# kolinko/effort

Hardware: AMD Instinct MI355X
Metric: effective GB/s + tokens/s vs effort %, Mistral-7B FFN 4096x11008 fp16 (higher is better)
Workload: dtype f16

## Files before the change

effort_amd/_lib.py:

```python
from __future__ import annotations

import ctypes as C
import os
import subprocess

_HERE = os.path.dirname(os.path.abspath(__file__))
LAB_LIB_PATH = os.path.join(_HERE, "libeffort_hip_lab.so")
LIB_PATH = (LAB_LIB_PATH if os.environ.get("EFFORT_HIP_LIB") == "lab" else os.environ.get("EFFORT_HIP_LIB")) or os.path.join(_HERE, "libeffort_hip.so")

ERRORS = {
    -1: "EFFORT_ERR_ARG", -2: "EFFORT_ERR_SHAPE", -3: "EFFORT_ERR_EFFORT", -4: "EFFORT_ERR_HIP",
    -5: "EFFORT_ERR_KIND", -6: "EFFORT_ERR_CONVERT", -7: "EFFORT_ERR_BLAS", -8: "EFFORT_ERR_COMM",
}


class EffortError(RuntimeError):
    def __init__(self, code: int, where: str, detail: str = ""):
        self.code = code
        super().__init__(f"{where}: {ERRORS.get(code, code)} {detail}".strip())


def build(verbose: bool = False) -> str:
    cmd = ["make", "-C", os.path.join(_HERE, "csrc"), "-j8", "all"]
    res = subprocess.run(cmd, capture_output=not verbose, text=True)
    if res.returncode != 0:
        raise RuntimeError("building libeffort_hip.so failed:\n" + (res.stdout or "") + (res.stderr or ""))
    return LIB_PATH


_P = C.c_void_p
_SIGS = {
    "effort_create": (_P, [C.c_int, _P]),
    "effort_destroy": (None, [_P]),
    "effort_set_stream": (C.c_int, [_P, _P]),
    "effort_sync": (C.c_int, [_P]),
    "effort_set_overlap": (C.c_int, [_P, C.c_int]),
    "effort_set_row_reuse": (C.c_int, [_P, C.c_int]),
    "effort_join": (C.c_int, [_P]),
    "effort_last_error": (C.c_char_p, [_P]),
    "effort_version": (C.c_char_p, []),
    "effort_weights_fp16": (_P, [_P, _P, _P, _P, C.c_int, C.c_int, C.c_int, C.c_int]),
    "effort_weights_fp16_pitched": (_P, [_P, _P, C.c_int, _P, _P, C.c_int, C.c_int, C.c_int, C.c_int]),
    "effort_aligned_row_pitch": (C.c_int, [C.c_int]),
    "effort_weights_q4": (_P, [_P, _P, _P, _P, _P, C.c_int64, C.c_int, C.c_int, C.c_int]),
    "effort_weights_free": (None, [_P]),
    "effort_weights_refresh": (C.c_int, [_P]),
    "effort_weights_align_rows": (C.c_int, [_P]),
    "effort_weights_row_pitch": (C.c_int, [_P]),
    "effort_weights_get_bound": (C.c_int, [_P, C.POINTER(C.c_float)]),
    "effort_weights_set_bound": (C.c_int, [_P, C.POINTER(C.c_float)]),
    "effort_weights_column_shard": (_P, [_P, C.c_int, C.c_int]),
    "effort_comm_unique_id": (C.c_int, [_P]),
    "effort_comm_create": (C.c_int, [_P, C.c_int, C.c_int, _P]),
    "effort_comm_destroy": (C.c_int, [_P]),
    "effort_comm_rank": (C.c_int, [_P]),
    "effort_comm_world": (C.c_int, [_P]),
    "effort_allgather_outputs": (C.c_int, [_P, _P, _P, C.c_int]),
    "effort_bucketmul": (C.c_int, [_P, _P, _P, _P, _P, C.c_double]),
    "effort_bucketmul_q4": (C.c_int, [_P, _P, _P, _P, _P, C.c_double]),
    "effort_bucketmul_group": (C.c_int, [_P, C.c_int, _P, _P, _P, _P, _P]),
    "effort_bucketmul_q4_group": (C.c_int, [_P, C.c_int, _P, _P, _P, _P, _P]),
    "effort_bucketmul_group_fused": (C.c_int, [_P, C.c_int, _P, _P, _P, _P, _P, _P, _P, _P]),
    "effort_bucketmul_q4_group_fused": (C.c_int, [_P, C.c_int, _P, _P, _P, _P, _P, _P, _P, _P]),
    "effort_group_dispatch_count": (C.c_int, [_P, C.c_int, C.POINTER(C.c_uint32)]),
    "effort_group_cutoff": (C.c_int, [_P, C.c_int, C.POINTER(C.c_float)]),
    "effort_debug_occupancy": (C.c_int, [_P, C.c_int, C.c_int, C.c_int, C.c_int]),
    "effort_set_persistent": (C.c_int, [_P, C.c_int]),
    "effort_debug_hook_lane": (C.c_int, [_P, C.c_int]),
    "effort_add_rmsnorm_mul": (C.c_int, [_P, _P, _P, _P, _P, C.c_int]),
    "effort_rope_kv": (C.c_int, [_P, _P, _P, _P, _P, _P, _P, _P, C.c_int, C.c_int, C.c_int, C.c_int, C.c_float]),
    "effort_attention": (C.c_int, [_P, _P, _P, _P, _P, _P, C.c_int, C.c_int, C.c_int]),
    "effort_rope_attention": (C.c_int, [_P, _P, _P, _P, _P, _P, _P, _P, C.c_int, C.c_int, C.c_int, C.c_int, C.c_float]),
    "effort_silu_mul": (C.c_int, [_P, _P, _P, _P, C.c_int]),
    "effort_fetch_row": (C.c_int, [_P, _P, _P, _P, C.c_int]),
    "effort_argmax": (C.c_int, [_P, _P, C.c_int, _P, _P, _P, C.c_int]),
    "effort_decode_status": (C.c_int, [_P, C.POINTER(C.c_int)]),
    "effort_sample": (C.c_int, [_P, _P, C.c_int, _P, _P, _P, _P, C.c_int, _P, _P]),
    "effort_topk": (C.c_int, [_P, _P, C.c_int, C.c_int, _P, _P]),
    "effort_sample_bits": (C.c_uint32, [C.c_uint32, C.c_uint32, C.c_uint32, C.c_uint32]),
    "effort_convert_status": (C.c_int, [_P, C.POINTER(C.c_int)]),
    "effort_q4_outlier_count": (C.c_int64, [C.c_int, C.c_int, C.c_double]),
    "effort_convert_q4": (C.c_int, [_P, _P, C.c_int, C.c_int, C.c_double, _P, _P, _P, _P]),
    "effort_top2_softmax": (C.c_int, [_P, _P, C.c_int, _P, _P]),
    "effort_mix2": (C.c_int, [_P, _P, _P, _P, _P, C.c_int]),
    "effort_moe_route": (C.c_int, [_P, _P, _P, _P, C.c_int, C.c_int, _P, _P, _P]),
    "effort_mix2_add": (C.c_int, [_P, _P, _P, _P, _P, C.c_int]),
    "effort_dense_gemv": (C.c_int, [_P, _P, _P, _P, C.c_int, C.c_int]),
    "effort_dense_gemv_expert": (C.c_int, [_P, _P, _P, _P, _P, C.c_int, C.c_int, C.c_int]),
    "effort_dense_gemm_rows": (C.c_int, [_P, _P, _P, _P, C.c_int, C.c_int, C.c_int]),
    "effort_dense_gemm_rows_routed": (C.c_int, [_P, _P, C.c_int, _P, _P, C.c_int, _P, C.c_int, C.c_int, C.c_int]),
    "effort_weights_bucket_dense_ok": (C.c_int, [_P, C.POINTER(C.c_int)]),
    "effort_bucket_gemm_rows": (C.c_int, [_P, _P, C.c_int, _P, _P, C.c_int]),
    "effort_bucket_gemm_rows_routed": (C.c_int, [_P, _P, _P, _P, C.c_int, _P, C.c_int]),
    "effort_moe_route_rows": (C.c_int, [_P, _P, _P, _P, C.c_int, C.c_int, _P, _P, _P, C.c_int]),
    "effort_mix2_add_rows": (C.c_int, [_P, _P, _P, _P, C.c_int, C.c_int]),
    "effort_fetch_rows": (C.c_int, [_P, _P, _P, _P, C.c_int, C.c_int]),
    "effort_add_rmsnorm_mul_rows": (C.c_int, [_P, _P, _P, _P, _P, C.c_int, C.c_int]),
    "effort_rope_kv_rows": (C.c_int, [_P, _P, _P, _P, _P, _P, _P, C.c_int, C.c_int, C.c_int, C.c_int, C.c_int, C.c_int, C.c_float]),
    "effort_attention_rows": (C.c_int, [_P, _P, _P, _P, C.c_int, C.c_int, _P, C.c_int, C.c_int, C.c_int]),
    "effort_attention_block": (C.c_int, [_P, _P, _P, _P, C.c_int, C.c_int, _P, C.c_int, C.c_int, C.c_int]),
    "effort_set_dense_backend": (C.c_int, [_P, C.c_int]),
    "effort_last_dispatch_count": (C.c_int, [_P, C.POINTER(C.c_uint32)]),
    "effort_last_cutoff": (C.c_int, [_P, C.POINTER(C.c_float)]),
    "effort_calc_dispatch": (C.c_int, [_P, _P, _P, _P, C.c_double, _P, _P]),
    "effort_convert_fp16": (C.c_int, [_P, _P, C.c_int, C.c_int, _P, _P, _P]),
    "effort_convert_fp16_pitched": (C.c_int, [_P, _P, C.c_int, C.c_int, _P, C.c_int, _P, _P]),
    "effort_cosine": (C.c_int, [_P, _P, _P, C.c_int, C.POINTER(C.c_float)]),
    "effort_set_split_cutoff": (C.c_int, [_P, C.c_int]),
    "effort_set_tuning": (C.c_int, [_P, C.c_int, C.c_int, C.c_int]),
    "effort_is_lab_build": (C.c_int, []),
    "effort_enable_kernel_timing": (C.c_int, [_P, C.c_int]),
    "effort_debug_stamps": (C.c_int, [_P, C.POINTER(C.c_ulonglong)]),
    "effort_debug_slice_counts": (C.c_int, [_P, C.c_int, C.POINTER(C.c_uint32), C.c_int]),
    "effort_debug_plan": (C.c_int, [C.c_int, C.c_int, C.c_int, C.c_int, _P, _P, _P, _P, _P, _P, C.c_int, C.c_int, C.c_int, C.c_int, _P, _P, _P, _P, _P, _P, _P, _P, _P]),
    "effort_debug_check_bundle": (C.c_int, [C.c_int, C.c_int, C.c_int, C.c_int, C.c_int, C.c_int]),
    "effort_debug_variants": (C.c_int, [C.c_int, _P, C.c_int]),
    "effort_debug_last_variant": (C.c_int, [_P, C.c_int, _P]),
    "effort_debug_lanes": (C.c_int, [C.c_int, C.c_int, _P, C.c_int64, _P]),
    "effort_debug_trace": (C.c_int, [_P, C.POINTER(C.c_ulonglong), C.c_int]),
    "effort_kernel_clock": (C.c_int, [_P, C.POINTER(C.c_double), C.POINTER(C.c_int)]),
    "effort_kernel_timing": (C.c_int, [_P, C.POINTER(C.c_double), C.POINTER(C.c_double), C.POINTER(C.c_double), C.POINTER(C.c_int)]),
}

_lib = None


def lib() -> C.CDLL:
    global _lib
    if _lib is None:
        if not os.path.exists(LIB_PATH):
            raise RuntimeError(
                f"{LIB_PATH} is missing: the HIP extension has not been built "
                "(run `python -c 'import __graft_entry__ as g; g.build()'` or `make -C effort_amd/csrc`). "
                "effort_amd has no CPU fallback.")
        import torch
        l = C.CDLL(LIB_PATH)
        for name, (res, args) in _SIGS.items():
            if (name.startswith("effort_debug_") or name == "effort_is_lab_build") and os.environ.get("EFFORT_HIP_LIB") and not hasattr(l, name):
                continue
            fn = getattr(l, name)
            fn.restype = res
            fn.argtypes = args
        _lib = l
    return _lib


def exported_symbols() -> list[str]:
    return sorted(_SIGS)
```

effort_amd/csrc/bucket_mul.hip:

```cpp
#include <cstring>
#include <type_traits>

#include "cutoff_device.h"

namespace effort {

constexpr int kBatch = 16;
template <int E> __host__ __device__ constexpr int batch_rows() { return E >= 4 ? 8 : kBatch; }
constexpr int kRounds = 16;

#ifndef EFFORT_ABLATE_NOSCATTER
#define EFFORT_ABLATE_NOSCATTER 0
#endif
#ifndef EFFORT_ABLATE_NOLOAD
#define EFFORT_ABLATE_NOLOAD 0
#endif

constexpr int kMinWavesPerEU = 4;

#ifndef EFFORT_ROW_AUX
#define EFFORT_ROW_AUX 2
#endif
constexpr int kRowAux = EFFORT_ROW_AUX;
#define GA_PERSISTENT(ga) (PERSIST ? (ga).persistent : 0u)
#define GA_CUTJOBS(ga) (PERSIST ? (ga).cutJobs : 0u)
#ifndef EFFORT_LAB
#define EFFORT_PRODUCT_ONLY 1
#if defined(EFFORT_CUT_FINE) || defined(EFFORT_LEAN_STAMPS) || EFFORT_ABLATE_NOSCATTER || EFFORT_ABLATE_NOLOAD
#error "lab switches need -DEFFORT_LAB (they belong in libeffort_hip_lab.so / build/variants, never in the shipped library)"
#endif
#endif
#ifdef EFFORT_PRODUCT_ONLY
constexpr bool kProductOnly = true;
#else
constexpr bool kProductOnly = false;
#endif
#ifdef EFFORT_PRODUCT_ONLY
#define GA_TSTAMP(ga) ((unsigned long long*)nullptr)
#define GA_ABLATE(ga) 0u
#define GA_TRACE(ga) 0u
#elif defined(EFFORT_LEAN_STAMPS)
#define GA_TSTAMP(ga) ((ga).tstamp)
#define GA_ABLATE(ga) (PERSIST ? (ga).ablate : 0u)
#define GA_TRACE(ga) 0u
#else
#define GA_TSTAMP(ga) (PERSIST ? (ga).tstamp : nullptr)
#define GA_ABLATE(ga) (PERSIST ? (ga).ablate : 0u)
#define GA_TRACE(ga) (PERSIST ? (ga).trace : 0u)
#endif
#ifdef EFFORT_LEAN_STAMPS
constexpr bool kLeanStamps = true;
#else
constexpr bool kLeanStamps = false;
#endif
constexpr uint32_t kMaxLdsBytes = 160u * 1024u - 1024u;
constexpr int kSc1 = 16;

template <int FMT> struct Fmt;
template <> struct Fmt<kFp16> { static constexpr int kAcc = 16, kSlots = 16; };
template <> struct Fmt<kQ4> { static constexpr int kAcc = 32, kSlots = 64; };

template <int FMT> struct MeanT;
template <> struct MeanT<kFp16> { typedef uint16_t type; };
template <> struct MeanT<kQ4> { typedef float type; };

template <int E> struct Piece;
template <> struct Piece<1> {
    uint32_t w;
    template <int AUX> __device__ __forceinline__ void load(__amdgpu_buffer_rsrc_t r, uint32_t voff, uint32_t soff) { w = __builtin_amdgcn_raw_buffer_load_b16(r, voff, soff, AUX); }
    __device__ __forceinline__ uint32_t word(int) const { return w & 0xFFFFu; }
    __device__ __forceinline__ uint32_t dword(int) const { return w; }
};
template <> struct Piece<2> {
    uint32_t w;
    template <int AUX> __device__ __forceinline__ void load(__amdgpu_buffer_rsrc_t r, uint32_t voff, uint32_t soff) { w = __builtin_amdgcn_raw_buffer_load_b32(r, voff, soff, AUX); }
    __device__ __forceinline__ uint32_t word(int j) const { return (w >> (16 * j)) & 0xFFFFu; }
    __device__ __forceinline__ uint32_t dword(int) const { return w; }
};
template <> struct Piece<4> {
    uint32_t w[2];
    template <int AUX> __device__ __forceinline__ void load(__amdgpu_buffer_rsrc_t r, uint32_t voff, uint32_t soff) {
        auto t = __builtin_amdgcn_raw_buffer_load_b64(r, voff, soff, AUX); w[0] = t[0]; w[1] = t[1];
    }
    __device__ __forceinline__ uint32_t word(int j) const { return (w[j >> 1] >> (16 * (j & 1))) & 0xFFFFu; }
    __device__ __forceinline__ uint32_t dword(int j) const { return w[j >> 1]; }
};
__host__ __device__ inline uint32_t align_up(uint32_t x, uint32_t a) { return (x + a - 1) / a * a; }

constexpr int kOlBatch = 16;
constexpr uint32_t kOlLdsFloats = 16384;
template <int E> __host__ __device__ inline uint32_t ol_outputs_per_item(const MulGeom& g) { return align_up((32u * E * 64u + g.slices - 1u) / g.slices, 64u); }
constexpr uint32_t kOlEarlyFloats = 4096;
constexpr int kOlMerged = 8;
constexpr uint32_t kOlSumFloats = 1024;
template <int E> __host__ __device__ inline uint32_t ol_scratch_bytes(const MulGeom& g) {
    const uint32_t per = ol_outputs_per_item<E>(g);
    return (per > kOlSumFloats ? per : kOlSumFloats) * 4u + (g.inDim <= kOlLdsFloats ? g.inDim * 4u : 0u);
}

template <int FMT, int E, int W>
__host__ __device__ inline LdsPlan plan_lds(const MulGeom* geoms, int nGeoms, bool merge) {
    uint32_t slots = 0, vrows = 0, ol = 0, vEarly = 0;
    for (int i = 0; i < nGeoms; i++) {
        const MulGeom& g = geoms[i];
        if (!g.slices) continue;
        slots = slots > g.slots ? slots : g.slots;
        const uint32_t vr = align_up(g.sliceRows, 64);
        vrows = vrows > vr ? vrows : vr;
        if (FMT != kFp16) {
            const uint32_t x = ol_scratch_bytes<E>(g); ol = ol > x ? ol : x;
            if (merge && W == 8 && g.inDim <= kOlEarlyFloats) vEarly = vEarly > g.inDim * 4u ? vEarly : g.inDim * 4u;
        }
    }
    LdsPlan p;
    uint32_t o = 0;
    p.offM = o; o += align_up(slots, 64) * 4;
    p.offV[0] = o; o += vrows * 4;
    p.offV[1] = FMT == kFp16 ? o : p.offV[0];
    if (FMT == kFp16) o += vrows * 4;
    if (FMT != kFp16 && o < ol) o = align_up(ol, 16);
    p.offA = o; o += (uint32_t)Fmt<FMT>::kSlots * E * 64 * 4;
    p.offL = o; o += align_up(slots * 2, 16);
    const uint32_t tbl = cutoff_table_bytes(64 * W);
    if (o < p.offA + tbl) o = p.offA + tbl;
    p.offC = o; o += 2048;
    p.offO = vEarly ? o : 0u; o += vEarly;
    static_assert(kCutoffLdsBytes <= 1280, "the cutoff scratch must end below the flags of the misc region");
    p.total = o;
    return p;
}
struct ItemRef { uint32_t ci, t, s; };

__device__ __forceinline__ bool locate_item(const GroupKArgs& ga, const uint32_t item, ItemRef& r) {
    uint32_t ci = 0;
    for (uint32_t i = 0; i + 1 < ga.count; i++) if ((item >> 3) >= (uint32_t)ga.wgEnd8[i]) ci = i + 1;
    ci = __builtin_amdgcn_readfirstlane(ci);
    const MulGeom& g = ga.geom[ga.call[ci].geom];
    const uint32_t b = item - (ci ? (uint32_t)ga.wgEnd8[ci - 1] * 8u : 0u), xcd = b & 7u, k = b >> 3;
    r.ci = ci;
    if ((g.slices & 7u) == 0u) {
        r.s = (k / g.tiles) * 8u + ((xcd + ci) & 7u); r.t = k % g.tiles;
        return true;
    }
    const uint32_t per = (uint32_t)ga.wgEnd8[ci] - (ci ? (uint32_t)ga.wgEnd8[ci - 1] : 0u);
    const uint32_t idx = ((xcd + ci) & 7u) * per + k;
    r.s = idx / g.tiles; r.t = idx - r.s * g.tiles;
    return r.s < g.slices;
}

typedef uint32_t u32x4 __attribute__((ext_vector_type(4)));
__device__ __forceinline__ void lds_dma_dword(const u32x4 rsrc, const uint32_t voff, const uint32_t ldsAddr) {
    uint32_t keep;
    asm volatile("s_mov_b32 %0, m0\n\ts_mov_b32 m0, %2\n\ts_nop 0\n\tbuffer_load_dword %1, %3, 0 offen lds\n\ts_mov_b32 m0, %0"
                 : "=&s"(keep) : "v"(voff), "s"(ldsAddr), "s"(rsrc) : "memory");
}
__device__ __forceinline__ u32x4 make_rsrc(const void* base, uint32_t bytes) {
    const uint64_t p = (uint64_t)(size_t)base;
    u32x4 r;
    r[0] = __builtin_amdgcn_readfirstlane((uint32_t)p); r[1] = __builtin_amdgcn_readfirstlane((uint32_t)(p >> 32) & 0xFFFFu);
    r[2] = __builtin_amdgcn_readfirstlane(bytes); r[3] = 0x00020000u;
    return r;
}

template <int FMT, int W, bool COMPACT>
__device__ __forceinline__ void stage_issue(const GroupKArgs& ga, const ItemRef& r, const int tid, char* smem, const LdsPlan& lp, const uint32_t par) {
    constexpr int NT = 64 * W;
    using lds_v = __attribute__((address_space(3))) void;
    const CallDesc& a = ga.call[__builtin_amdgcn_readfirstlane(r.ci)];
    const MulGeom& g = ga.geom[a.geom];
    const uint32_t wave = __builtin_amdgcn_readfirstlane(tid >> 6);
    const uint32_t B = g.sliceRows, j0 = __builtin_amdgcn_readfirstlane(r.s) * B, nb = min(B, g.inDim - j0), lg = g.sliceLog2;
    const uint32_t e = a.expNo ? a.expNo[0] : 0u;
    const uint32_t rowBase = e * g.expertRows;
    const uint32_t rowsPerIn = g.rowsPerIn, inDim = g.inDim, mask = (1u << lg) - 1u;
    const uint32_t nSlots = FMT == kFp16 ? (rowsPerIn << lg) : (nb << 3);
    constexpr bool compact = COMPACT && FMT == kFp16;
    const u32x4 rs = make_rsrc(a.stats, (uint32_t)((size_t)g.numExperts * g.expertRows * (compact ? 2u : 8u)));
    const u32x4 rv = make_rsrc(a.v, inDim * 4u);
    const uint32_t ldsM = __builtin_amdgcn_readfirstlane((uint32_t)(size_t)(lds_v*)(smem + lp.offM));
    const uint32_t ldsV = __builtin_amdgcn_readfirstlane((uint32_t)(size_t)(lds_v*)(smem + ((par & 1u) ? lp.offV[1] : lp.offV[0])));
    if constexpr (compact) {
#pragma unroll
        for (int rr = 0; rr < kRounds / 2; rr++) {
            if (((uint32_t)(rr * NT) + wave * 64u) * 2u >= nSlots) continue;
            const uint32_t c = ((uint32_t)(rr * NT) + (uint32_t)tid) * 2u, rank = c >> lg, jl = c & mask;
            const bool ok = rank < rowsPerIn && jl < nb;
            lds_dma_dword(rs, (rowBase + (ok ? rank * inDim + j0 + jl : j0)) * 2u, ldsM + ((uint32_t)(rr * NT) + wave * 64u) * 4u);
        }
    } else
#pragma unroll
    for (int rr = 0; rr < kRounds; rr++) {
        if ((uint32_t)(rr * NT) + wave * 64u >= nSlots) continue;
        const uint32_t c = rr * NT + tid;
        uint32_t voff;
        if (FMT == kFp16) {
            const uint32_t rank = c >> lg, jl = c & mask;
            const bool ok = rank < rowsPerIn && jl < nb;
            voff = (rowBase + (ok ? rank * inDim + j0 + jl : j0)) * 8u + 4u;
        } else {
            voff = ((rowBase + j0 * 8u + (c < nSlots ? c : 0u)) * 2u + 1u) * 4u;
        }
        lds_dma_dword(rs, voff, ldsM + ((uint32_t)(rr * NT) + wave * 64u) * 4u);
    }
#pragma unroll
    for (int u = 0; u < (FMT == kFp16 ? 1 : 2); u++) {
        if ((uint32_t)(u * NT) + wave * 64u >= nb) continue;
        lds_dma_dword(rv, (j0 + (uint32_t)(u * NT + tid)) * 4u, ldsV + ((uint32_t)(u * NT) + wave * 64u) * 4u);
    }
}

template <int FMT, int E, int W, bool FUSED, bool COMPACT, bool PERSIST, typename Prefetch>
__device__ __forceinline__ void mul_item(const GroupKArgs& ga, const uint32_t item, const ItemRef& ref, char* smem, const LdsPlan& lp, uint32_t& cachedCall,
                                         float& cachedCutoff, const uint32_t par, const bool staged, const bool firstItem, Prefetch prefetch) {
    constexpr int NACC = Fmt<FMT>::kAcc;
    constexpr int TILE_F = NACC * E * 64;
    constexpr int TILE_L = Fmt<FMT>::kSlots * E * 64;
    constexpr int NT = 64 * W;
    constexpr int VPT = 4096 / NT;
    constexpr int KB = batch_rows<E>();

    const uint32_t ci = __builtin_amdgcn_readfirstlane(ref.ci), s = __builtin_amdgcn_readfirstlane(ref.s), t = __builtin_amdgcn_readfirstlane(ref.t);
    const CallDesc& a = ga.call[ci];
    const MulGeom& g = ga.geom[a.geom];
    float* const a_slabs = ga.slabs + (size_t)a.slabOff * 64u;
    uint32_t* const a_counters = ga.counters + a.tileOff;
    uint32_t* const a_sliceCounts = ga.sliceCounts + a.sliceOff;
    float* const a_cutoff = ga.cutoff + ci;
    (void)item;

    int tid0 = threadIdx.x;
    asm volatile("" : "+v"(tid0));
    const int tid = tid0, lane = tid & 63;
#ifdef EFFORT_CUT_FINE
    const bool wstamp = false;
#else
    const bool wstamp = GA_TSTAMP(ga) && tid == 0;
#endif
    unsigned long long ph[6] = {0, 0, 0, 0, 0, 0};
    if (wstamp) ph[0] = wall_clock64();
#ifdef EFFORT_CUT_FINE
    const bool stampCut = GA_TSTAMP(ga) && item == 0 && tid == 0, stamp = false;
#define EFFORT_PSTAMP(i) if (stampCut) GA_TSTAMP(ga)[26 + (i)] = clock64();
#else
#define EFFORT_PSTAMP(i)
    const bool stamp = GA_TSTAMP(ga) && item == 0 && tid == 0;
    const bool stampCut = stamp;
#endif
    if (stamp) GA_TSTAMP(ga)[16] = wall_clock64();
    const int wave = __builtin_amdgcn_readfirstlane(tid >> 6);
    const uint32_t B = g.sliceRows;
    const uint32_t offC = __builtin_amdgcn_readfirstlane(lp.offC), offL = __builtin_amdgcn_readfirstlane(lp.offL), offM = __builtin_amdgcn_readfirstlane(lp.offM);
    const uint32_t offA = __builtin_amdgcn_readfirstlane(lp.offA);
    int* acc = reinterpret_cast<int*>(smem + offA);
    float* vblk = reinterpret_cast<float*>(smem + __builtin_amdgcn_readfirstlane((par & 1u) ? lp.offV[1] : lp.offV[0]));
    uint32_t* flags = reinterpret_cast<uint32_t*>(smem + offC + 1280);
    float* wbound = reinterpret_cast<float*>(smem + offC + 1344);
    uint16_t* list = reinterpret_cast<uint16_t*>(smem + offL);
    const uint32_t* m32 = reinterpret_cast<const uint32_t*>(smem + offM);
    const float* means = reinterpret_cast<const float*>(smem + offM);

    const uint32_t j0 = s * B;
    uint32_t vSlabOff = (s * g.tiles + t) * (uint32_t)(TILE_F * 4), vSlabBytes = (uint32_t)min((size_t)0xFFFFFFFFu, (size_t)g.slices * g.tiles * TILE_F * 4);
    uint32_t vSlices = g.slices, vSliceStride = g.tiles * (uint32_t)(TILE_F * 4);
    if constexpr (!PERSIST) asm volatile("" : "+v"(vSlabOff), "+v"(vSlabBytes), "+v"(vSlices), "+v"(vSliceStride));
    const uint32_t nb = min(B, g.inDim - j0);
    const uint32_t e = a.expNo ? a.expNo[0] : 0u;

    EFFORT_PSTAMP(1)
    if (!staged) stage_issue<FMT, W, COMPACT>(ga, ref, tid, smem, lp, par);
    EFFORT_PSTAMP(2)
    constexpr bool kPreZero = !PERSIST;
    if constexpr (kPreZero) cutoff_table_zero<NT>(reinterpret_cast<uint32_t*>(smem + offA), tid);
    constexpr bool kOlMerge = FMT != kFp16 && W == 8 && (!PERSIST || kProductOnly);
    const uint32_t olPer = ol_outputs_per_item<E>(g);
    bool olAny = false, olEarly = false;
    uint32_t olParts = 1u, olStride = 0u;
    uint32_t olBFirst = 0u, olNB = 0u;
    float olVx[kOlMerge ? 8 : 1]; uint32_t olMeta0 = 0u, olBeg0 = 0u, olEnd0 = 0u;
    auto ol_share = [&]() {
        const uint32_t oBeg = min(t * (uint32_t)TILE_F + s * olPer, g.outDim);
        const uint32_t oEnd = max(oBeg, min(min(t * (uint32_t)TILE_F + (s + 1u) * olPer, (t + 1u) * (uint32_t)TILE_F), g.outDim));
        olBFirst = oBeg >> 6; olNB = ((oEnd + 63u) >> 6) - olBFirst;
        olParts = (olNB && olNB < (uint32_t)W) ? (uint32_t)W / olNB : 1u;
        olStride = olNB * 64u;
    };
    if constexpr (FMT != kFp16) {
        olAny = a.ol.blockPtr != nullptr;
        if (olAny) {
            if constexpr (kOlMerge) {
                ol_share();
                olEarly = g.inDim <= kOlEarlyFloats && lp.offO != 0u;
                if (olEarly) {
                    if constexpr (FUSED) {
                        if (a.pre == (uint16_t)kPreNone) {
#pragma unroll
                            for (int u = 0; u < 8; u++) olVx[u] = a.v[min((uint32_t)(u * NT + tid), g.inDim - 1u)];
                        }
                    } else {
#pragma unroll
                    for (int u = 0; u < 8; u++) olVx[u] = a.v[min((uint32_t)(u * NT + tid), g.inDim - 1u)];
                    }
                    if ((uint32_t)wave < olNB * olParts) {
                        const uint32_t bq = (uint32_t)wave / olParts;
                        olMeta0 = a.ol.meta[(size_t)(olBFirst + bq) * 64u + (uint32_t)lane];
                        olBeg0 = a.ol.blockPtr[olBFirst + bq]; olEnd0 = a.ol.blockPtr[olBFirst + bq + 1u];
                    }
                }
            }
        }
    }
    const float rankBound = a.rankBound[e];
    float vj[VPT]; uint16_t prj[VPT];
    const uint16_t* pr = a.probes + (size_t)e * kProbes;
    const bool fused = (ga.split & 1u) == 0u;
#pragma unroll
    for (int i = 0; i < VPT; i++) { vj[i] = 0.0f; prj[i] = 0; }
    const bool needCut = fused && cachedCall != ci;
    const bool viaJob = needCut && GA_CUTJOBS(ga) != 0u && !firstItem;
    const uint32_t pre = FUSED ? (uint32_t)a.pre : (uint32_t)kPreNone;
    float rawn[VPT]; uint32_t auxc[VPT]; uint32_t auxS = 0u;
    uint32_t auxS1 = 0u;
    const bool preAny = FUSED && pre != (uint32_t)kPreNone;
#pragma unroll
    for (int i = 0; i < VPT; i++) { rawn[i] = 0.0f; auxc[i] = 0u; }
    if (preAny) {
        const bool gate = pre == (uint32_t)kPreSiluGate;
        if (needCut || !gate) {
#pragma unroll
            for (int i = 0; i < VPT; i++) rawn[i] = *(a.v + tid + NT * i);
        }
        if (needCut) {
#pragma unroll
            for (int i = 0; i < VPT; i++) {
                auxc[i] = gate ? __float_as_uint(*(reinterpret_cast<const float*>(a.vAux) + tid + NT * i)) : (uint32_t)reinterpret_cast<const uint16_t*>(a.vAux)[tid + NT * i];
                prj[i] = pr[tid + NT * i];
            }
        }
        const uint32_t js = j0 + min((uint32_t)tid, nb - 1u);
        auxS = gate ? __float_as_uint(*(reinterpret_cast<const float*>(a.vAux) + js)) : (uint32_t)reinterpret_cast<const uint16_t*>(a.vAux)[js];
        if constexpr (FUSED && FMT != kFp16) {
            const uint32_t js1 = j0 + min((uint32_t)(tid + NT), nb - 1u);
            auxS1 = gate ? __float_as_uint(*(reinterpret_cast<const float*>(a.vAux) + js1)) : (uint32_t)reinterpret_cast<const uint16_t*>(a.vAux)[js1];
            if (olEarly && !needCut) {
                if (gate) {
#pragma unroll
                    for (int i = 0; i < VPT; i++) rawn[i] = *(a.v + tid + NT * i);
                }
#pragma unroll
                for (int i = 0; i < VPT; i++)
                    auxc[i] = gate ? __float_as_uint(*(reinterpret_cast<const float*>(a.vAux) + tid + NT * i)) : (uint32_t)reinterpret_cast<const uint16_t*>(a.vAux)[tid + NT * i];
            }
        }
    }
    const uint32_t lg = g.sliceLog2;
    const uint32_t nSlots = FMT == kFp16 ? (g.rowsPerIn << lg) : (nb << 3);
    float normInv = 1.0f;
    if (FUSED && pre == kPreRmsNorm) {
        constexpr int R = 1024 / NT;
        static_assert(R >= 1 && R * NT == 1024 && R * W == 16, "fused rmsNorm: the workgroup must divide add_rmsnorm_mul_kernel's 1024 threads");
        float part[R];
#pragma unroll
        for (int r = 0; r < R; r++) part[r] = 0.0f;
#pragma unroll
        for (int i = 0; i < VPT; i++) part[i % R] += rawn[i] * rawn[i];
        for (uint32_t base = 4096u + (uint32_t)tid; base < g.inDim; base += 1024u) {
#pragma unroll
            for (int r = 0; r < R; r++) {
                const uint32_t j = base + (uint32_t)(r * NT);
                if (j < g.inDim) { const float x = *(a.v + j); part[r] += x * x; }
            }
        }
#pragma unroll
        for (int r = 0; r < R; r++) {
            part[r] = wave_sum_f32(part[r]);
            if (lane == 0) wbound[r * W + wave] = part[r];
        }
        __syncthreads();
        float tot = 0.0f;
#pragma unroll
        for (int w2 = 0; w2 < 16; w2++) tot += wbound[w2];
        normInv = 1.0f / sqrtf(tot / (float)g.inDim + 1e-5f);
        __syncthreads();
    }
    auto xform = [&](float x, uint32_t aux) -> float {
        if (!FUSED) return x;
        if (pre == kPreSiluGate) return __uint_as_float(aux) * x / (1.0f + expf(-x));
        if (pre == kPreRmsNorm) return (x * normInv) * half_bits_to_float((uint16_t)aux);
        return x;
    };
    auto load_cut_inputs = [&]() {
        if (preAny) {
#pragma unroll
            for (int i = 0; i < VPT; i++) vj[i] = xform(rawn[i], auxc[i]);
        } else {
#pragma unroll
            for (int i = 0; i < VPT; i++) { vj[i] = *(a.v + tid + NT * i); prj[i] = pr[tid + NT * i]; }
        }
    };
    if constexpr (kPreZero) {
        asm volatile("s_waitcnt lgkmcnt(0)" ::: "memory");
        __builtin_amdgcn_s_barrier();
    }
    if (needCut && !viaJob) load_cut_inputs();
    EFFORT_PSTAMP(3)
    uint32_t* const cutWords = ga.queue + 9 * 16;
    uint32_t cutWord = 0;
    if (viaJob && tid == 0 && !(GA_ABLATE(ga) & 32u)) cutWord = __hip_atomic_load(&cutWords[ci], __ATOMIC_RELAXED, __HIP_MEMORY_SCOPE_AGENT);
    asm volatile("s_waitcnt vmcnt(0)" ::: "memory");
    EFFORT_PSTAMP(4)
    uint32_t vColOK = 0, voff = 0, vRecords = 0, vBuckLo = 0, vBuckHi = 0, vRowPitch = 0, vInDim = 0, vRow0 = 0;
    auto stream_geom = [&]() {
        const uint32_t col = t * (64u * E) + (uint32_t)lane * E;
        vColOK = col < g.cols ? 1u : 0u;
        voff = (vColOK ? col : (g.cols - 1u) / (uint32_t)E * (uint32_t)E) * 2u;
        vRecords = (uint32_t)min((size_t)0xFFFFFFFFu, (size_t)g.numExperts * g.expertRows * g.rowPitch - (size_t)a.bucketsTrim);
        vBuckLo = (uint32_t)(size_t)a.buckets; vBuckHi = (uint32_t)((size_t)a.buckets >> 32);
        vRowPitch = g.rowPitch; vInDim = g.inDim; vRow0 = e * g.expertRows + (FMT == kFp16 ? j0 : j0 * 8u);
    };
    if constexpr (!PERSIST) {
        stream_geom();
        asm volatile("" : "+v"(vColOK), "+v"(voff), "+v"(vRecords), "+v"(vBuckLo), "+v"(vBuckHi), "+v"(vRowPitch), "+v"(vInDim), "+v"(vRow0));
    }
    if constexpr (kOlMerge) {
        if (olEarly) {
            float* const vf = reinterpret_cast<float*>(smem + __builtin_amdgcn_readfirstlane(lp.offO));
#pragma unroll
            for (int u = 0; u < 8; u++) {
                if constexpr (FUSED) { if ((uint32_t)(u * NT + tid) < g.inDim) vf[u * NT + tid] = preAny ? xform(rawn[u % VPT], auxc[u % VPT]) : olVx[u]; }
                else if ((uint32_t)(u * NT + tid) < g.inDim) vf[u * NT + tid] = olVx[u];
            }
        }
    }
    float bound = 0.0f;
#pragma unroll
    for (int u = 0; u < (FMT == kFp16 ? 1 : 2); u++) {
        const uint32_t jl = tid + u * NT;
        if (jl < nb) {
            float x = vblk[jl];
            if constexpr (FUSED && FMT != kFp16) { if (preAny) { x = xform(x, u ? auxS1 : auxS); vblk[jl] = x; } }
            else
            if (preAny) { x = xform(x, auxS); vblk[jl] = x; }
            bound += fabsf(x);
        }
    }
    bound = wave_sum_f32(bound);
    if (lane == 0) wbound[wave] = bound;
    if (tid == 0) { flags[4] = 0u; flags[5] = (uint32_t)(W * KB); }
    if (stamp) GA_TSTAMP(ga)[17] = wall_clock64();
    if (wstamp) ph[1] = wall_clock64();

    uint32_t* tbl = reinterpret_cast<uint32_t*>(smem + offA);
    float cutoff;
    bool fromJob = false;
    if (viaJob) {
        if (tid == 0) {
            for (int spin = 0; spin < ((GA_ABLATE(ga) & 32u) ? 0 : 20000) && !(cutWord >> 31); spin++) {
                __builtin_amdgcn_s_sleep(8);
                cutWord = __hip_atomic_load(&cutWords[ci], __ATOMIC_RELAXED, __HIP_MEMORY_SCOPE_AGENT);
            }
            flags[2] = cutWord >> 31;
            flags[3] = cutWord & 0x7FFFFFFFu;
        }
        __syncthreads();
        fromJob = flags[2] != 0u;
        if (fromJob) { cutoff = __uint_as_float(flags[3]); cachedCall = ci; cachedCutoff = cutoff; }
        else load_cut_inputs();
    }
    if (fromJob) {
    } else if (needCut) {
        cutoff = block_find_cutoff<NT, kPreZero>(vj, prj, a.q, smem + offC, tbl, []() {}, stampCut ? GA_TSTAMP(ga) + 8 : nullptr);
        cachedCall = ci; cachedCutoff = cutoff;
    } else if (fused) {
        cutoff = cachedCutoff;
        __syncthreads();
    } else {
        cutoff = a_cutoff[0];
        __syncthreads();
    }
    const uint32_t slotCap = __builtin_amdgcn_readfirstlane((lp.offV[0] - lp.offM) / 4u) - 1u;
    const uint16_t* m16 = reinterpret_cast<const uint16_t*>(m32);
    auto load_block = [&](int blk, uint32_t (&mraw)[4], float (&vq)[4]) {
#pragma unroll
        for (int u = 0; u < 4; u++) {
            const uint32_t c = min((uint32_t)((blk * 4 + u) * NT + tid), slotCap);
            if constexpr (COMPACT && FMT == kFp16) { mraw[u] = (uint32_t)m16[c] << 16; vq[u] = 0.0f; }
            else { mraw[u] = m32[c]; vq[u] = FMT != kFp16 ? vblk[min(c >> 3, nb - 1u)] : 0.0f; }
        }
    };
    uint32_t mraw0[4]; float vq0[4];
    load_block(0, mraw0, vq0);
    const uint32_t jlSel = (uint32_t)tid & ((1u << lg) - 1u);
    float axRaw = 0.0f;
    if (FMT == kFp16) axRaw = vblk[min(jlSel, nb - 1u)];
    float wb[W];
#pragma unroll
    for (int w2 = 0; w2 < W; w2++) wb[w2] = wbound[w2];
    __builtin_amdgcn_sched_barrier(0);
    for (int i = tid; i < TILE_L; i += NT) acc[i] = 0;
    float L = 0.0f;
#pragma unroll
    for (int w2 = 0; w2 < W; w2++) L += wb[w2];
    L *= rankBound;
    int kexp = 30 - (int)((__float_as_uint(L) >> 23) & 0xFFu) + 126;
    kexp = L > 0.0f ? max(-100, min(100, kexp)) : 0;
    const float scale = __uint_as_float((uint32_t)(127 + kexp) << 23), unscale = __uint_as_float((uint32_t)(127 - kexp) << 23);
    if (stamp) GA_TSTAMP(ga)[18] = wall_clock64();
    if (wstamp) ph[2] = wall_clock64();

    const float ax = (FMT == kFp16 && jlSel < nb) ? fabsf(axRaw) : 0.0f;
    const bool sel = !(GA_ABLATE(ga) & 8u);
    uint32_t keepMask = 0;
    uint32_t before[kRounds];
    uint32_t wtot = 0;
#pragma unroll
    for (int blk = 0; blk < kRounds / 4; blk++) {
        if (blk > 0 && (uint32_t)(blk * 4 * NT) >= nSlots) {
#pragma unroll
            for (int u = 0; u < 4; u++) before[blk * 4 + u] = wtot;
            continue;
        }
        uint32_t mraw[4]; float vq[4];
        if (blk == 0) {
#pragma unroll
            for (int u = 0; u < 4; u++) { mraw[u] = mraw0[u]; vq[u] = vq0[u]; }
        } else {
            load_block(blk, mraw, vq);
        }
#pragma unroll
        for (int u = 0; u < 4; u++) {
            const int rr = blk * 4 + u;
            before[rr] = wtot;
            const uint32_t c = rr * NT + tid;
            bool k;
            if (FMT == kFp16) k = (cutoff < (kCutoffScale * half_bits_to_float((uint16_t)(mraw[u] >> 16))) * ax) & ((c >> lg) < g.rowsPerIn) & sel;
            else k = (cutoff < (kCutoffScale * __uint_as_float(mraw[u])) * fabsf(vq[u])) & (c < nSlots) & sel;
            keepMask |= k ? (1u << rr) : 0u;
            wtot += (uint32_t)__popcll(__ballot(k));
        }
    }
    uint32_t wbase = 0;
    if (lane == 0) wbase = atomicAdd(&flags[4], wtot);
    wbase = __builtin_amdgcn_readfirstlane(wbase);
#pragma unroll
    for (int rr = 0; rr < kRounds; rr++) {
        if ((uint32_t)(rr * NT) >= nSlots) break;
        const uint32_t c = rr * NT + tid;
        const bool k = (keepMask >> rr) & 1u;
        const unsigned long long m = __ballot(k);
        const uint32_t pos = wbase + before[rr] + __builtin_amdgcn_mbcnt_hi((uint32_t)(m >> 32), __builtin_amdgcn_mbcnt_lo((uint32_t)m, 0u));
        if (k) list[pos] = (uint16_t)(FMT == kFp16 ? (((c >> lg) << 12) | (c & ((1u << lg) - 1u))) : c);
    }
    __syncthreads();
    const uint32_t n = flags[4];
    const uint32_t code0 = list[(uint32_t)(wave * KB) + ((uint32_t)lane & (uint32_t)(KB - 1))];
    if (t == 0 && tid == 0) a_sliceCounts[s] = n;
    if (stamp) GA_TSTAMP(ga)[19] = wall_clock64();
    if (wstamp) ph[3] = wall_clock64();

    if constexpr (PERSIST) stream_geom();
    const bool colOK = vColOK != 0u;
    const __amdgpu_buffer_rsrc_t rsrc = __builtin_amdgcn_make_buffer_rsrc(
        reinterpret_cast<uint16_t*>((size_t)(uint32_t)__builtin_amdgcn_readfirstlane(vBuckLo) | ((size_t)(uint32_t)__builtin_amdgcn_readfirstlane(vBuckHi) << 32)), 0,
        (int)__builtin_amdgcn_readfirstlane(vRecords), 0x00020000);
    const uint32_t nU = (GA_ABLATE(ga) & 4u) ? 0u : __builtin_amdgcn_readfirstlane(n);
    uint32_t* const cursor = flags + 5;
    auto grab = [&]() -> uint32_t {
        uint32_t bq = 0;
        if (lane == 0) bq = atomicAdd(cursor, (uint32_t)KB);
        return __builtin_amdgcn_readfirstlane(bq);
    };

    auto decode_code = [&](uint32_t code, uint32_t& boff, float& dv) {
        {
            uint32_t rowIdx;
            if (FMT == kFp16) { const uint32_t rank = code >> 12, jl = code & 4095u; rowIdx = rank * vInDim + jl; dv = vblk[jl] * scale; }
            else {
                rowIdx = code;
                dv = __int_as_float(__float2int_rn((vblk[code >> 3] * means[code]) * scale));
            }
            boff = (vRow0 + rowIdx) * vRowPitch;
        }
    };
    auto decode = [&](uint32_t i0, uint32_t& boff, float& dv) {
        boff = 0; dv = 0.0f;
        if (lane < KB && nU) decode_code(list[min(i0 + (uint32_t)lane, nU - 1u)], boff, dv);
    };
    auto decode_first = [&](uint32_t i0, uint32_t& boff, float& dv) {
        boff = 0; dv = 0.0f;
        if (lane < KB && nU) decode_code(i0 + (uint32_t)lane < nU ? code0 : (uint32_t)__builtin_amdgcn_readfirstlane((int)code0), boff, dv);
    };
    auto issue = [&](auto aux, Piece<E> (&piece)[KB], uint32_t boff) {
#pragma unroll
        for (int u = 0; u < KB; u++) piece[u].template load<decltype(aux)::value>(rsrc, voff, EFFORT_ABLATE_NOLOAD ? 0u : __builtin_amdgcn_readlane(boff, u));
    };
    using lds_i = __attribute__((address_space(3))) int;
    const uint32_t accB = (uint32_t)(size_t)(lds_i*)(acc + lane);
    constexpr int kShift = (E == 1 ? 8 : E == 2 ? 9 : 10);
    auto row = [&](const Piece<E>& pc, float dd) {
        if (FMT == kFp16) {
#pragma unroll
            for (int j = 0; j < E; j++) {
                const uint32_t dw = pc.dword(j);
                uint32_t a2; int qv;
                asm("v_bfe_u32 %0, %1, %2, 4\n\tv_lshl_add_u32 %0, %0, %3, %4" : "=&v"(a2) : "v"(dw), "n"(16 * (j & 1)), "n"(kShift), "v"(accB));
                if (j & 1) asm("v_fma_mix_f32 %0, %1, %2, 0 op_sel:[0,1,0] op_sel_hi:[0,1,0]\n\tv_cvt_rpi_i32_f32 %0, %0" : "=v"(qv) : "v"(dd), "v"(dw));
                else asm("v_fma_mix_f32 %0, %1, %2, 0 op_sel_hi:[0,1,0]\n\tv_cvt_rpi_i32_f32 %0, %0" : "=v"(qv) : "v"(dd), "v"(dw));
                __hip_atomic_fetch_add((lds_i*)(size_t)a2 + j * 64, qv, __ATOMIC_RELAXED, __HIP_MEMORY_SCOPE_WORKGROUP);
            }
        } else {
            const int di = __float_as_int(dd);
#pragma unroll
            for (int j = 0; j < E; j++) {
                const uint32_t x = pc.word(j);
#pragma unroll
                for (int q = 0; q < 4; q++) {
                    uint32_t a2;
                    asm("v_bfe_u32 %0, %1, %2, 4\n\tv_lshl_add_u32 %0, %0, %3, %4" : "=&v"(a2) : "v"(x), "n"(4 * q), "n"(kShift), "v"(accB));
                    __hip_atomic_fetch_add((lds_i*)(size_t)a2 + ((3 - q) * 16 * E + j) * 64, di, __ATOMIC_RELAXED, __HIP_MEMORY_SCOPE_WORKGROUP);
                }
            }
        }
    };
    auto accumulate = [&](const Piece<E> (&piece)[KB], float dv, uint32_t nv) {
        if (EFFORT_ABLATE_NOSCATTER) {
#pragma unroll
            for (int u = 0; u < KB; u++) asm volatile("" ::"v"(piece[u].word(E - 1)), "v"(dv));
            return;
        }
        if (!colOK) return;
        if (nv == (uint32_t)KB) {
#pragma unroll
            for (int u = 0; u < KB; u++) row(piece[u], __uint_as_float(__builtin_amdgcn_readlane(__float_as_uint(dv), u)));
        } else {
#pragma unroll
            for (int u = 0; u < KB; u++)
                if ((uint32_t)u < nv) row(piece[u], __uint_as_float(__builtin_amdgcn_readlane(__float_as_uint(dv), u)));
        }
    };

    bool asked = false;
    using lds_f = __attribute__((address_space(3))) float;
    uint32_t olLen = 0u, olOut = 0u, olKa = 0u, olKf = 0u, olK1 = 0u, olCur = 0u, olSlot = 0xFFFFFFFFu;
    float olAcc = 0.0f;
    const lds_f* olV = nullptr;
    if constexpr (kOlMerge) {
        if (olEarly) {
            olV = (const lds_f*)(size_t)(uint32_t)(size_t)(__attribute__((address_space(3))) void*)(smem + __builtin_amdgcn_readfirstlane(lp.offO));
            if ((uint32_t)wave < olNB * olParts) {
                const uint32_t bq = (uint32_t)wave / olParts, part = (uint32_t)wave % olParts;
                olLen = olMeta0 >> 8; olOut = olMeta0 & 63u;
                const uint32_t olLenAll = olLen;
                const uint32_t maxLen = (uint32_t)__builtin_amdgcn_readfirstlane((int)olLen);
                const uint32_t chunk = (maxLen + olParts - 1u) / olParts, k0 = min(maxLen, part * chunk);
                const uint32_t bBeg = __builtin_amdgcn_readfirstlane(olBeg0), bEnd = __builtin_amdgcn_readfirstlane(olEnd0);
                olK1 = bEnd > bBeg ? min(maxLen, k0 + chunk) : k0;
                olKa = olKf = k0;
                olCur = bBeg + wave_sum_u32(min(olLenAll, k0));
                olLen = min(olLenAll, olK1);
                olSlot = part * olStride + bq * 64u + olOut;
            }
        }
    }
    auto ol_fma = [](float x, uint32_t ent, float acc) -> float {
        float r;
        asm("v_fma_mix_f32 %0, %1, %2, %3 op_sel:[0,1,0] op_sel_hi:[0,1,0]" : "=v"(r) : "v"(x), "v"(ent), "v"(acc));
        return r;
    };
    auto ol_fetch = [&](uint32_t (&ent)[kOlMerged]) {
#pragma unroll
        for (int u = 0; u < kOlMerged; u++) {
            ent[u] = *((a.ol.entry + olCur) + lane);
            olCur += (uint32_t)__popcll(__ballot(olLen > olKf + (uint32_t)u));
        }
        olKf += (uint32_t)kOlMerged;
    };
    auto ol_add = [&](const uint32_t (&ent)[kOlMerged]) {
        float x[kOlMerged];
#pragma unroll
        for (int u = 0; u < kOlMerged; u++) x[u] = olV[ent[u] & 0xFFFFu];
#pragma unroll
        for (int u = 0; u < kOlMerged; u++)
            { const float r = ol_fma(x[u], ent[u], olAcc); olAcc = olLen > olKa + (uint32_t)u ? r : olAcc; }
        olKa += (uint32_t)kOlMerged;
    };
    auto stream_rows = [&](auto withOl, auto aux) {
        constexpr bool OL = decltype(withOl)::value;
        Piece<E> pa[KB], pb[KB];
        uint32_t entA[OL ? kOlMerged : 1], entB[OL ? kOlMerged : 1];
        uint32_t boffA, boffB; float dvA, dvB;
        uint32_t baseA = (uint32_t)(wave * KB), baseB;
        if (baseA < nU) { decode_first(baseA, boffA, dvA); issue(aux, pa, boffA); }
        if constexpr (OL) ol_fetch(entA);
        while (baseA < nU) {
            if (!asked && nU - baseA <= 4u * KB * W) asked = prefetch();
            if (wstamp && GA_TRACE(ga) && item + GA_CUTJOBS(ga) < (uint32_t)kTraceItems) {
                const uint32_t q0 = (4u * baseA) / nU, q1 = min(4u, (4u * (baseA + 2u * KB * W)) / nU);
                for (uint32_t q = q0 + 1u; q <= q1 && q < 4u; q++) GA_TSTAMP(ga)[kTraceOff + (size_t)kTraceItems * 8u + (size_t)(item + GA_CUTJOBS(ga)) * 4u + q - 1u] = wall_clock64();
            }
            baseB = grab();
            decode(baseB, boffB, dvB);
            issue(aux, pb, boffB);
            if constexpr (OL) ol_fetch(entB);
            accumulate(pa, dvA, __builtin_amdgcn_readfirstlane(min((uint32_t)KB, nU - baseA)));
            if constexpr (OL) ol_add(entA);
            baseA = grab();
            decode(baseA, boffA, dvA);
            issue(aux, pa, boffA);
            if constexpr (OL) ol_fetch(entA);
            accumulate(pb, dvB, __builtin_amdgcn_readfirstlane(baseB < nU ? min((uint32_t)KB, nU - baseB) : 0u));
            if constexpr (OL) ol_add(entB);
        }
        if constexpr (OL) {
            while (olKa < olK1) {
                ol_fetch(entB); ol_add(entA);
                if (olKa >= olK1) break;
                ol_fetch(entA); ol_add(entB);
            }
        }
    };
    constexpr bool kRowSwitch = kRowAux != 0 && (PERSIST || E == 4);
    const bool rowsReused = kRowSwitch && (ga.split & 8u) != 0u;
    auto stream = [&](auto withOl) {
        if constexpr (kRowSwitch) { if (rowsReused) { stream_rows(withOl, std::integral_constant<int, 0>{}); return; } }
        stream_rows(withOl, std::integral_constant<int, kRowAux>{});
    };
    if constexpr (kOlMerge) { if (olEarly) stream(std::true_type{}); else stream(std::false_type{}); }
    else stream(std::false_type{});
    if (!asked) asked = prefetch();
    __syncthreads();
    if (stamp) GA_TSTAMP(ga)[20] = wall_clock64();
    if (wstamp) ph[4] = wall_clock64();

    float* const olsum = reinterpret_cast<float*>(smem + offM);
    if constexpr (FMT != kFp16) {
        if (olAny) {
            const OutlierIndex& ol = a.ol;
            float* const vfull = olEarly ? reinterpret_cast<float*>(smem + __builtin_amdgcn_readfirstlane(lp.offO)) : olsum + (olPer > kOlSumFloats ? olPer : kOlSumFloats);
            const bool vLds = g.inDim <= kOlLdsFloats;
            if constexpr (!kOlMerge) ol_share();
            const uint32_t bFirst = olBFirst, nB = olNB, parts = olParts;
            if (vLds && !olEarly) {
                for (uint32_t i0 = 0; i0 < g.inDim; i0 += NT * 8u) {
                    float x[8];
#pragma unroll
                    for (int u = 0; u < 8; u++) x[u] = a.v[min(i0 + u * NT + tid, g.inDim - 1u)];
                    if constexpr (FUSED) {
                        uint32_t xa[8];
#pragma unroll
                        for (int u = 0; u < 8; u++) xa[u] = 0u;
                        if (preAny) {
#pragma unroll
                            for (int u = 0; u < 8; u++) {
                                const uint32_t i = min(i0 + u * NT + tid, g.inDim - 1u);
                                xa[u] = pre == (uint32_t)kPreSiluGate ? __float_as_uint(*(reinterpret_cast<const float*>(a.vAux) + i)) : (uint32_t)reinterpret_cast<const uint16_t*>(a.vAux)[i];
                            }
                        }
#pragma unroll
                        for (int u = 0; u < 8; u++) {
                            const uint32_t i = i0 + u * NT + tid;
                            if (i < g.inDim) vfull[i] = preAny ? xform(x[u], xa[u]) : x[u];
                        }
                    } else
#pragma unroll
                    for (int u = 0; u < 8; u++) {
                        const uint32_t i = i0 + u * NT + tid;
                        if (i < g.inDim) vfull[i] = x[u];
                    }
                }
                __syncthreads();
            }
            if (olSlot != 0xFFFFFFFFu) olsum[olSlot] = olAcc;
            const lds_f* const vfullL = (const lds_f*)(size_t)(uint32_t)(size_t)(__attribute__((address_space(3))) void*)vfull;
            auto run_blocks = [&](auto fromLds) {
                for (uint32_t q = (uint32_t)wave + (olEarly ? (uint32_t)W : 0u); q < nB * parts; q += (uint32_t)W) {
                    const uint32_t bq = q / parts, part = q % parts;
                    const uint32_t meta = ol.meta[(size_t)(bFirst + bq) * 64u + (uint32_t)lane];
                    const uint32_t lenAll = meta >> 8, myOut = meta & 63u;
                    const uint32_t maxLen = (uint32_t)__builtin_amdgcn_readfirstlane((int)lenAll);
                    const uint32_t chunk = (maxLen + parts - 1u) / parts, k0 = min(maxLen, part * chunk), k1 = min(maxLen, k0 + chunk);
                    const uint32_t myLen = min(lenAll, k1);
                    const uint32_t bBeg = __builtin_amdgcn_readfirstlane(ol.blockPtr[bFirst + bq]), bEnd = __builtin_amdgcn_readfirstlane(ol.blockPtr[bFirst + bq + 1u]);
                    uint32_t cur = bBeg + wave_sum_u32(min(lenAll, k0));
                    float acc = 0.0f;
                    auto fetch = [&](uint32_t (&ent)[kOlBatch], uint32_t kk) {
#pragma unroll
                        for (int u = 0; u < kOlBatch; u++) {
                            ent[u] = *((ol.entry + cur) + lane);
                            cur += (uint32_t)__popcll(__ballot(myLen > kk + (uint32_t)u));
                        }
                    };
                    auto add = [&](const uint32_t (&ent)[kOlBatch], uint32_t kk) {
                        float x[kOlBatch];
#pragma unroll
                        for (int u = 0; u < kOlBatch; u++) {
                            const uint32_t in = ent[u] & 0xFFFFu;
                            if constexpr (decltype(fromLds)::value) x[u] = vfullL[in]; else x[u] = a.v[in];
                        }
#pragma unroll
                        for (int u = 0; u < kOlBatch; u++)
                            { const float r = ol_fma(x[u], ent[u], acc); acc = myLen > kk + (uint32_t)u ? r : acc; }
                    };
                    if (k0 < k1 && bEnd > bBeg) {
                        uint32_t entA[kOlBatch], entB[kOlBatch];
                        uint32_t kk = k0;
                        fetch(entA, kk);
                        for (;;) {
                            const bool more = kk + (uint32_t)kOlBatch < k1;
                            if (more) fetch(entB, kk + (uint32_t)kOlBatch);
                            add(entA, kk);
                            if (!more) break;
                            kk += (uint32_t)kOlBatch;
                            const bool more2 = kk + (uint32_t)kOlBatch < k1;
                            if (more2) fetch(entA, kk + (uint32_t)kOlBatch);
                            add(entB, kk);
                            if (!more2) break;
                            kk += (uint32_t)kOlBatch;
                        }
                    }
                    olsum[part * olStride + bq * 64u + myOut] = acc;
                }
            };
            if (vLds) run_blocks(std::true_type{}); else run_blocks(std::false_type{});
            __syncthreads();
        }
    }

    const __amdgpu_buffer_rsrc_t srs = __builtin_amdgcn_make_buffer_rsrc(a_slabs, 0, (int)__builtin_amdgcn_readfirstlane(vSlabBytes), 0x00020000);
    const uint32_t slabOff = __builtin_amdgcn_readfirstlane(vSlabOff);
    const uint32_t nSlices = __builtin_amdgcn_readfirstlane(vSlices);
    auto tile_out = [&](int o) -> float {
        if (FMT == kFp16) return (float)acc[o] * unscale;
        const int slot = o / (E * 64), rem = o % (E * 64);
        const int p = (((slot >> 3) * 16 + (slot & 7)) * E * 64) + rem;
        float r = (float)(acc[p] - acc[p + 8 * E * 64]) * unscale;
        if (olAny) {
            const uint32_t ol_o = (uint32_t)((rem & 63) * E + (rem >> 6)) * 32u + (uint32_t)slot - s * olPer;
            if (ol_o < olPer && (uint32_t)(t * TILE_F) + s * olPer + ol_o < g.outDim) {
                float so = olsum[ol_o];
                for (uint32_t pp = 1; pp < olParts; pp++) so += olsum[pp * olStride + ol_o];
                r += so;
            }
        }
        return r;
    };
    if (fused && t == 0 && s == 0 && tid == 0 && !GA_CUTJOBS(ga)) a_cutoff[0] = cutoff;
    {
        constexpr int kIt = (TILE_F + NT * 2 - 1) / (NT * 2);
        float s0[kIt], s1[kIt];
#pragma unroll
        for (int it = 0; it < kIt; it++) {
            const int o = min(tid * 2 + it * NT * 2, TILE_F - 2);
            s0[it] = tile_out(o); s1[it] = tile_out(o + 1);
        }
#pragma unroll
        for (int it = 0; it < kIt; it++) {
            const int o = tid * 2 + it * NT * 2;
            if (TILE_F % (NT * 2) != 0 && o >= TILE_F) continue;
            typedef uint32_t u2 __attribute__((ext_vector_type(2)));
            u2 pk; pk[0] = __float_as_uint(s0[it]); pk[1] = __float_as_uint(s1[it]);
            __builtin_amdgcn_raw_buffer_store_b64(pk, srs, (uint32_t)o * 4u, slabOff, kSc1);
        }
    }
    asm volatile("s_waitcnt vmcnt(0)" ::: "memory");
    if (stamp) { GA_TSTAMP(ga)[21] = wall_clock64(); GA_TSTAMP(ga)[22] = n; }
    if (wstamp) ph[5] = wall_clock64();
    auto flush_stamps = [&]() {
#ifndef EFFORT_PRODUCT_ONLY
        if (!wstamp) return;
        if (GA_TRACE(ga) && item + GA_CUTJOBS(ga) < (uint32_t)kTraceItems) {
            unsigned long long* rec = GA_TSTAMP(ga) + kTraceOff + (size_t)(item + GA_CUTJOBS(ga)) * 8u;
            rec[0] = (unsigned long long)(item + GA_CUTJOBS(ga)) | ((unsigned long long)blockIdx.x << 32);
            rec[1] = (unsigned long long)(__builtin_amdgcn_s_getreg((31 << 11) | 20) & 0xFu) | ((unsigned long long)(ci & 0xFu) << 4) | ((unsigned long long)(n & 0xFFFFu) << 8) | ((unsigned long long)(t & 0xFFu) << 24) |
                     ((unsigned long long)__builtin_amdgcn_s_getreg((31 << 11) | 4) << 32);
#pragma unroll
            for (int i = 0; i < 6; i++) rec[2 + i] = ph[i];
        }
        unsigned long long* line = GA_TSTAMP(ga) + 64 + (item & 31u) * 8u;
#pragma unroll
        for (int i = 0; i < 5; i++) atomicAdd(&line[i], ph[i + 1] - ph[i]);
        atomicAdd(&line[5], 1ull);
        atomicMin(&GA_TSTAMP(ga)[0], ph[0]);
        atomicMax(&GA_TSTAMP(ga)[26], ph[0]);
        atomicMax(&GA_TSTAMP(ga)[28], ph[5] - ph[0]);
        atomicMax(&GA_TSTAMP(ga)[29], ph[4] - ph[3]);
        atomicMax(&GA_TSTAMP(ga)[1], (unsigned long long)wall_clock64());
#endif
    };
    {
        __syncthreads();
        if (tid == 0) {
            const uint32_t ticket = __hip_atomic_fetch_add(&a_counters[t], 1u, __ATOMIC_RELAXED, __HIP_MEMORY_SCOPE_AGENT);
            flags[0] = (ticket == nSlices - 1u) ? 1u : 0u;
        }
        __syncthreads();
        if (flags[0] == 0u) { flush_stamps(); return; }
    }
    if (GA_ABLATE(ga) & 2u) { if (tid == 0) __hip_atomic_store(&a_counters[t], 0u, __ATOMIC_RELAXED, __HIP_MEMORY_SCOPE_AGENT); return; }

    const bool rstamp = GA_TSTAMP(ga) && ci == 0 && t == 0 && tid == 0;
    if (rstamp) GA_TSTAMP(ga)[23] = wall_clock64();
    typedef uint32_t u4v __attribute__((ext_vector_type(4)));
    const uint32_t sliceStride = __builtin_amdgcn_readfirstlane(vSliceStride);
    constexpr int kCols4 = TILE_F / 4;
    constexpr int G = NT / kCols4 >= 2 ? NT / kCols4 : 1;
    float* const gpart = reinterpret_cast<float*>(smem + offA + (uint32_t)TILE_L * 4u);
    static_assert(G == 1 || (uint32_t)TILE_L * 4u + (uint32_t)G * TILE_F * 4u <= (cutoff_table_bytes(NT) > (uint32_t)TILE_L * 4u ? cutoff_table_bytes(NT) : (uint32_t)TILE_L * 4u),
                  "the thread groups' partial sums must fit behind the tile");
    auto reduce_tile = [&](auto kc) {
        constexpr int kRed = decltype(kc)::value;
        const int grp = G > 1 ? tid / kCols4 : 0;
        const uint32_t per = G > 1 ? ((nSlices + G - 1) / G + 3u) / 4u * 4u : nSlices;
        const uint32_t sl0 = (uint32_t)grp * per, sl1 = min(nSlices, sl0 + per);
        for (int o = (G > 1 ? tid % kCols4 : tid) * 4; o < TILE_F; o += (G > 1 ? kCols4 : NT) * 4) {
            const uint32_t vo = t * (uint32_t)(TILE_F * 4) + (uint32_t)o * 4u;
            float res[4] = {0.0f, 0.0f, 0.0f, 0.0f};
            if (FUSED && a.resid && (G == 1 || grp == 0)) {
#pragma unroll
                for (int h = 0; h < 4; h++) {
                    const uint32_t oo = (uint32_t)o + h, lane2 = oo & 63u, sj = oo >> 6, j = sj % E, slot = sj / E;
                    const uint32_t c2 = t * (64u * E) + lane2 * E + j;
                    if (c2 < g.cols) res[h] = *(a.resid + c2 * NACC + slot);
                }
            }
            float sm[4][4];
#pragma unroll
            for (int h = 0; h < 4; h++) { sm[h][0] = 0.0f; sm[h][1] = 0.0f; sm[h][2] = 0.0f; sm[h][3] = 0.0f; }
            for (uint32_t sl = sl0; sl < sl1; sl += kRed) {
                u4v r[kRed];
#pragma unroll
                for (int i = 0; i < kRed; i++)
                    r[i] = __builtin_amdgcn_raw_buffer_load_b128(srs, vo, min(sl + i, nSlices - 1u) * sliceStride, kSc1);
#pragma unroll
                for (int i = 0; i < kRed; i++) {
                    if (sl + i < sl1) {
#pragma unroll
                        for (int h = 0; h < 4; h++) sm[h][i & 3] += __uint_as_float(r[i][h]);
                    }
                }
            }
            float tot[4];
#pragma unroll
            for (int h = 0; h < 4; h++) tot[h] = (sm[h][0] + sm[h][1]) + (sm[h][2] + sm[h][3]);
            if (G > 1) {
#pragma unroll
                for (int h = 0; h < 4; h++) gpart[grp * TILE_F + o + h] = tot[h];
                __syncthreads();
                if (grp != 0) continue;
#pragma unroll
                for (int h = 0; h < 4; h++) {
                    tot[h] = gpart[o + h];
                    for (int g2 = 1; g2 < G; g2++) tot[h] += gpart[g2 * TILE_F + o + h];
                }
            }
#pragma unroll
            for (int h = 0; h < 4; h++) {
                const uint32_t oo = (uint32_t)o + h;
                const uint32_t lane2 = oo & 63u, sj = oo >> 6, j = sj % E, slot = sj / E;
                const uint32_t c2 = t * (64u * E) + lane2 * E + j;
                if (c2 < g.cols) {
                    const uint32_t oi = c2 * NACC + slot;
                    const float val = (FUSED && a.resid) ? res[h] + tot[h] : tot[h];
                    a.out[oi] = val;
                }
            }
        }
    };
    if (nSlices <= 8u * G) reduce_tile(std::integral_constant<int, 8>{});
    else reduce_tile(std::integral_constant<int, 16>{});
    if (PERSIST && G > 1) __syncthreads();
    if (rstamp) GA_TSTAMP(ga)[24] = wall_clock64();
    if (tid == 0) {
        __hip_atomic_store(&a_counters[t], 0u, __ATOMIC_RELAXED, __HIP_MEMORY_SCOPE_AGENT);
#if !defined(EFFORT_CUT_FINE) && !defined(EFFORT_PRODUCT_ONLY)
        if (GA_TSTAMP(ga)) {
            flush_stamps();
            const uint32_t done = __hip_atomic_fetch_add(ga.groupDone, 1u, __ATOMIC_RELAXED, __HIP_MEMORY_SCOPE_AGENT);
            if (done == ga.totalTiles - 1u) {
                const unsigned long long t0 = __hip_atomic_load(&GA_TSTAMP(ga)[0], __ATOMIC_RELAXED, __HIP_MEMORY_SCOPE_AGENT);
                const unsigned long long t1 = __hip_atomic_load(&GA_TSTAMP(ga)[1], __ATOMIC_RELAXED, __HIP_MEMORY_SCOPE_AGENT);
                GA_TSTAMP(ga)[2] += t1 - t0; GA_TSTAMP(ga)[3] += 1;
                GA_TSTAMP(ga)[27] += __hip_atomic_load(&GA_TSTAMP(ga)[26], __ATOMIC_RELAXED, __HIP_MEMORY_SCOPE_AGENT) - t0;
                __hip_atomic_store(&GA_TSTAMP(ga)[26], 0ull, __ATOMIC_RELAXED, __HIP_MEMORY_SCOPE_AGENT);
                __hip_atomic_store(&GA_TSTAMP(ga)[0], ~0ull, __ATOMIC_RELAXED, __HIP_MEMORY_SCOPE_AGENT);
                __hip_atomic_store(&GA_TSTAMP(ga)[1], 0ull, __ATOMIC_RELAXED, __HIP_MEMORY_SCOPE_AGENT);
                __hip_atomic_store(ga.groupDone, 0u, __ATOMIC_RELAXED, __HIP_MEMORY_SCOPE_AGENT);
            }
        }
#endif
    }
}

template <int NT>
__device__ __forceinline__ void cutoff_job(const GroupKArgs& ga, uint32_t ci, char* smem) {
    constexpr int VPT = 4096 / NT;
    const CallDesc& a = ga.call[ci];
    int tid0 = threadIdx.x;
    asm volatile("" : "+v"(tid0));
    const int tid = tid0;
    const uint32_t e = a.expNo ? a.expNo[0] : 0u;
    const uint16_t* pr = a.probes + (size_t)e * kProbes;
    float vj[VPT]; uint16_t prj[VPT];
#pragma unroll
    for (int i = 0; i < VPT; i++) { vj[i] = a.v[tid + NT * i]; prj[i] = pr[tid + NT * i]; }
    [[maybe_unused]] constexpr bool PERSIST = true;
    const unsigned long long tj0 = (GA_TSTAMP(ga) && GA_TRACE(ga)) ? wall_clock64() : 0ull;
    const float cutoff = block_find_cutoff<NT>(vj, prj, a.q, smem + cutoff_table_bytes(NT), reinterpret_cast<uint32_t*>(smem), []() {}, nullptr);
    if (tid == 0 && GA_TSTAMP(ga) && GA_TRACE(ga)) {
        unsigned long long* rec = GA_TSTAMP(ga) + kTraceOff + (size_t)ci * 8u;
        rec[0] = (unsigned long long)ci | ((unsigned long long)blockIdx.x << 32) | (1ull << 63);
        rec[1] = (unsigned long long)__builtin_amdgcn_s_getreg((31 << 11) | 20) | ((unsigned long long)__builtin_amdgcn_s_getreg((31 << 11) | 4) << 32);
        rec[2] = tj0; rec[3] = wall_clock64();
    }
    if (tid == 0) {
        __hip_atomic_store(&ga.queue[9 * 16 + ci], __float_as_uint(cutoff) | 0x80000000u, __ATOMIC_RELAXED, __HIP_MEMORY_SCOPE_AGENT);
        __hip_atomic_store(reinterpret_cast<uint32_t*>(ga.cutoff + ci), __float_as_uint(cutoff), __ATOMIC_RELAXED, __HIP_MEMORY_SCOPE_AGENT);
    }
    __syncthreads();
}

template <int FMT, int E, int W, bool FUSED, bool COMPACT = false, bool PERSIST = true>
__global__ __launch_bounds__(64 * W, (FUSED && FMT != kFp16 && W == 2 ? 2 : W <= 8 ? kMinWavesPerEU : 4)) void bucket_mul_kernel(const GroupKArgs ga) {
    extern __shared__ __attribute__((aligned(16))) char smem[];
    __shared__ uint32_t s_item;
    __shared__ unsigned long long s_next;
#ifdef EFFORT_CUT_FINE
    if (GA_TSTAMP(ga) && blockIdx.x == 0 && threadIdx.x == 0) GA_TSTAMP(ga)[26] = clock64();
#endif
    if constexpr (!PERSIST) {
        const uint32_t* const kw = reinterpret_cast<const uint32_t*>(&ga);
        uint32_t touch[12];
#pragma unroll
        for (int i = 0; i < 12; i++) touch[i] = kw[i * 16];
#pragma unroll
        for (int i = 0; i < 12; i++) asm volatile("" :: "s"(touch[i]));
    }
#ifdef EFFORT_CUT_FINE
#define EFFORT_ESTAMP(i) if (GA_TSTAMP(ga) && blockIdx.x == 0 && threadIdx.x == 0) GA_TSTAMP(ga)[16 + (i)] = clock64();
#else
#define EFFORT_ESTAMP(i)
#endif
    EFFORT_ESTAMP(0)
    const uint32_t staggerSleeps = ga.staggerSleeps;
    if constexpr (PERSIST) {
        if (GA_PERSISTENT(ga) && staggerSleeps && blockIdx.x >= ga.numCU)
            for (uint32_t i = 0; i < staggerSleeps; i++) __builtin_amdgcn_s_sleep(32);
    }
    const uint32_t total = ga.totalItems + GA_CUTJOBS(ga);
    uint32_t cachedCall = 0xFFFFFFFFu; float cachedCutoff = 0.0f;
    const uint32_t x = blockIdx.x & 7u;
    uint32_t dry = 0;
    auto pull = [&]() -> uint32_t {
        uint32_t got = total;
        for (uint32_t tries = 0; tries < 8u && got >= total; tries++) {
            const uint32_t q = (x + tries) & 7u;
            if ((dry >> q) & 1u) continue;
            const uint32_t cand = __hip_atomic_fetch_add(&ga.queue[q * 16u], 1u, __ATOMIC_RELAXED, __HIP_MEMORY_SCOPE_AGENT) * 8u + q;
            if (cand < total) got = cand; else dry |= 1u << q;
            if (GA_ABLATE(ga) & 64u) break;
        }
        return got;
    };
    auto pull_sync = [&]() -> uint32_t {
        if (threadIdx.x == 0) s_item = pull();
        __syncthreads();
        const uint32_t it = __builtin_amdgcn_readfirstlane(s_item);
        __syncthreads();
        return it;
    };
    constexpr bool kPipe = !FUSED && FMT == kFp16;
    const LdsPlan lp = ga.lp;
    uint32_t par = 0;
    bool staged = false;
    uint32_t gen = 0;
    if (threadIdx.x == 0) __hip_atomic_store(&s_next, 0ull, __ATOMIC_RELAXED, __HIP_MEMORY_SCOPE_WORKGROUP);
    uint32_t item = GA_PERSISTENT(ga) ? pull_sync() : blockIdx.x;
    while (item < total) {
        if (item < GA_CUTJOBS(ga)) {
            if (item < ga.count) cutoff_job<64 * W>(ga, item, smem);
            item = GA_PERSISTENT(ga) ? pull_sync() : total;
            continue;
        }
        ItemRef ref;
        EFFORT_ESTAMP(1)
        if (!locate_item(ga, item - GA_CUTJOBS(ga), ref)) {
            item = GA_PERSISTENT(ga) ? pull_sync() : total;
            continue;
        }
        EFFORT_ESTAMP(2)
        gen++;
        bool stagedNext = false;
        auto prefetch = [&]() -> bool {
            if (!GA_PERSISTENT(ga)) return true;
            if (threadIdx.x == 0)
                __hip_atomic_store(&s_next, ((unsigned long long)gen << 32) | (unsigned long long)pull(), __ATOMIC_RELAXED, __HIP_MEMORY_SCOPE_WORKGROUP);
            const unsigned long long nx = __hip_atomic_load(&s_next, __ATOMIC_RELAXED, __HIP_MEMORY_SCOPE_WORKGROUP);
            if (__builtin_amdgcn_readfirstlane((uint32_t)(nx >> 32)) != gen) return false;
            const uint32_t next = __builtin_amdgcn_readfirstlane((uint32_t)nx);
            ItemRef nref;
            if (kPipe && !(GA_ABLATE(ga) & 128u) && next >= GA_CUTJOBS(ga) && next < total && locate_item(ga, next - GA_CUTJOBS(ga), nref)) {
                int tid0 = threadIdx.x;
                asm volatile("" : "+v"(tid0));
                stage_issue<FMT, W, COMPACT>(ga, nref, tid0, smem, lp, par ^ 1u);
                stagedNext = true;
            }
            return true;
        };
        const bool firstOwn = gen == 1u && (GA_ABLATE(ga) & 512u) != 0u;
        mul_item<FMT, E, W, FUSED, COMPACT, PERSIST>(ga, item - GA_CUTJOBS(ga), ref, smem, lp, cachedCall, cachedCutoff, par, staged, firstOwn, prefetch);
        item = GA_PERSISTENT(ga) ? __builtin_amdgcn_readfirstlane((uint32_t)__hip_atomic_load(&s_next, __ATOMIC_RELAXED, __HIP_MEMORY_SCOPE_WORKGROUP)) : total;
        staged = stagedNext;
        par ^= 1u;
    }
    if (GA_PERSISTENT(ga) && threadIdx.x == 0) {
        const uint32_t gone = __hip_atomic_fetch_add(&ga.queue[8 * 16], 1u, __ATOMIC_RELAXED, __HIP_MEMORY_SCOPE_AGENT);
        if (gone == gridDim.x - 1u) {
            for (int i = 0; i <= 8; i++) __hip_atomic_store(&ga.queue[i * 16], 0u, __ATOMIC_RELAXED, __HIP_MEMORY_SCOPE_AGENT);
            for (int i = 0; i < kMaxGroup; i++) __hip_atomic_store(&ga.queue[9 * 16 + i], 0u, __ATOMIC_RELAXED, __HIP_MEMORY_SCOPE_AGENT);
        }
    }
}

template <int FMT, int E, int W, typename F>
static hipError_t each_variant(F&& f) {
    hipError_t err = hipSuccess;
    auto one = [&](auto fu, auto co, auto pe) {
        constexpr bool FU = decltype(fu)::value, CO = decltype(co)::value, PE = decltype(pe)::value;
        if (err == hipSuccess) err = f(&bucket_mul_kernel<FMT, E, W, FU, CO, PE>, FU, CO, PE);
    };
    constexpr std::true_type T{}; constexpr std::false_type N{};
    one(N, N, T); one(T, N, T);
    if constexpr (FMT == kFp16) one(N, T, T);
    if constexpr (W == 8) {
        one(N, N, N); one(T, N, N);
        if constexpr (FMT == kFp16) { one(N, T, N); one(T, T, N); }
    }
    return err;
}

template <int FMT, int E, int W>
static hipError_t launch_mul_t(const GroupKArgs& gaIn, hipStream_t st, LaunchedVariant* ran) {
    GroupKArgs ga = gaIn;
    constexpr bool kLean = W == 8;
    const bool lean = kLean && !ga.persistent && (kLeanStamps || !ga.tstamp) && !ga.ablate;
    const LdsPlan lp = ga.lp = plan_lds<FMT, E, W>(ga.geom, kMaxGeoms, lean || (kLean && kProductOnly));
    uint32_t lds = lp.total;
    if (lp.offA > 65536u && FMT == kFp16) return hipErrorInvalidValue;
    for (uint32_t i = 0; i < ga.count; i++) {
        const MulGeom& g = ga.geom[ga.call[i].geom];
        if (g.slots > (uint32_t)kRounds * 64 * W || g.slots != (FMT == kFp16 ? (g.rowsPerIn << g.sliceLog2) : g.sliceRows * 8u)) return hipErrorInvalidValue;
        if (FMT == kFp16 ? (1u << g.sliceLog2) > 64u * W : g.sliceRows > 128u * W) return hipErrorInvalidValue;
        if (((uint32_t)ga.wgEnd8[i] - (i ? (uint32_t)ga.wgEnd8[i - 1] : 0u)) * 8u != align_up(g.tiles * g.slices, 8)) return hipErrorInvalidValue;
    }
    if (ga.totalItems != (uint32_t)ga.wgEnd8[ga.count - 1] * 8u) return hipErrorInvalidValue;
    uint32_t grid = ga.totalItems;
    if (ga.persistent) {
        const uint32_t R = ga.persistent;
        grid = ga.numCU * R;
        const uint32_t force = (160u * 1024u) / (R + 1u) + 512u;
        if (lds < force && force <= (160u * 1024u) / R) lds = force;
    }
    bool fusedAny = false;
    for (uint32_t i = 0; i < ga.count; i++) fusedAny = fusedAny || ga.call[i].pre || ga.call[i].resid;
    for (uint32_t i = 0; FMT != kFp16 && i < ga.count; i++)
        if (ga.call[i].pre && ga.call[i].ol.blockPtr && ga.geom[ga.call[i].geom].inDim > kOlLdsFloats) return hipErrorInvalidValue;
    if (lds > kMaxLdsBytes) return hipErrorInvalidValue;
    const bool compact = (ga.split & 4u) != 0u;
    if (compact && (FMT != kFp16 || (fusedAny && !lean))) return hipErrorInvalidValue;
    const dim3 gd(grid), bd(64 * W);
    bool launched = false;
    const hipError_t err = each_variant<FMT, E, W>([&](auto kernel, bool fu, bool co, bool pe) -> hipError_t {
        if (launched || fu != fusedAny || co != compact || pe == lean) return hipSuccess;
        launched = true;
        if (ran) *ran = LaunchedVariant{(uint32_t)W, (uint32_t)E, fu, co, !pe, ga.persistent, grid, ga.totalItems};
        hipLaunchKernelGGL(kernel, gd, bd, lds, st, ga);
        return hipGetLastError();
    });
    return err != hipSuccess ? err : launched ? hipSuccess : hipErrorInvalidValue;
}

hipError_t bucket_mul_prepare_device() {
    auto set = [](auto kernel, bool, bool, bool) -> hipError_t {
        const void* f = reinterpret_cast<const void*>(kernel);
        hipFuncAttributes fa;
        hipError_t e = hipFuncGetAttributes(&fa, f);
        if (e != hipSuccess) return e;
        if (fa.sharedSizeBytes > 1024u) return hipErrorInvalidValue;
        return hipFuncSetAttribute(f, hipFuncAttributeMaxDynamicSharedMemorySize, (int)(160u * 1024u - (uint32_t)fa.sharedSizeBytes));
    };
    hipError_t err = hipSuccess;
#define EFFORT_CASE(w, e) if (err == hipSuccess) err = each_variant<kFp16, e, w>(set); if (err == hipSuccess) err = each_variant<kQ4, e, w>(set);
    EFFORT_GEOMS(EFFORT_CASE)
#undef EFFORT_CASE
    return err;
}

template <typename F>
static bool with_geom(int W, int E, F&& f) {
#define EFFORT_CASE(w, e) if (W == w && E == e) { f(std::integral_constant<int, w>{}, std::integral_constant<int, e>{}); return true; }
    EFFORT_GEOMS(EFFORT_CASE)
#undef EFFORT_CASE
    return false;
}

hipError_t launch_bucket_mul(Format fmt, int W, int E, const GroupKArgs& a, hipStream_t st, LaunchedVariant* ran) {
    hipError_t err = hipErrorInvalidValue;
    with_geom(W, E, [&](auto w, auto e) { err = fmt == kFp16 ? launch_mul_t<kFp16, decltype(e)::value, decltype(w)::value>(a, st, ran) : launch_mul_t<kQ4, decltype(e)::value, decltype(w)::value>(a, st, ran); });
    return err;
}

int bucket_mul_variants(Format fmt, int* rows, int maxRows) {
    int n = 0;
    auto note = [&](int w, int e) {
        return [&n, rows, maxRows, w, e](auto, bool fu, bool co, bool pe) -> hipError_t {
            if (rows && n < maxRows) { int* r = rows + 5 * n; r[0] = w; r[1] = e; r[2] = fu; r[3] = co; r[4] = !pe; }
            n++;
            return hipSuccess;
        };
    };
#define EFFORT_CASE(w, e) if (fmt == kFp16) each_variant<kFp16, e, w>(note(w, e)); else each_variant<kQ4, e, w>(note(w, e));
    EFFORT_GEOMS(EFFORT_CASE)
#undef EFFORT_CASE
    return n;
}

size_t bucket_mul_lds_bytes(Format fmt, int W, int E, const MulGeom& g, bool lean) {
    size_t n = 0;
    with_geom(W, E, [&](auto w, auto e) { n = fmt == kFp16 ? plan_lds<kFp16, decltype(e)::value, decltype(w)::value>(&g, 1, lean).total : plan_lds<kQ4, decltype(e)::value, decltype(w)::value>(&g, 1, lean).total; });
    return n;
}

int bucket_mul_occupancy(Format fmt, int W, int E, size_t ldsBytes) {
    int n = 0;
    with_geom(W, E, [&](auto w, auto e) {
        const void* f = fmt == kFp16 ? reinterpret_cast<const void*>(&bucket_mul_kernel<kFp16, decltype(e)::value, decltype(w)::value, false>)
                                     : reinterpret_cast<const void*>(&bucket_mul_kernel<kQ4, decltype(e)::value, decltype(w)::value, false>);
        if (hipOccupancyMaxActiveBlocksPerMultiprocessor(&n, f, 64 * decltype(w)::value, ldsBytes) != hipSuccess) n = 0;
    });
    return n;
}

uint32_t bucket_mul_ol_lds_floats() { return kOlLdsFloats; }

uint32_t bucket_mul_max_candidates(int W) { return (uint32_t)kRounds * 64u * (uint32_t)W; }

}
```

effort_amd/csrc/ctx.hip:

```cpp
#include <map>
#include <mutex>
#include <vector>

#include "host.h"

using namespace effort;

static constexpr size_t kStampBytes = (size_t)(kTraceOff + kTraceItems * 12) * 8;

extern "C" const char* effort_version(void) { return "effort-hip 0.1 (gfx950)"; }
static char g_createErr[256] = "null context";
extern "C" const char* effort_last_error(effort_ctx* c) { return c ? c->err : g_createErr; }

static bool lane_alloc(effort_ctx* c, Lane& L) {
    bool ok = hipMalloc(&L.d_cutoff, 512) == hipSuccess && hipMalloc(&L.d_count, 16) == hipSuccess &&
              hipMalloc(&L.d_slabs, c->env.slabBytes) == hipSuccess && hipMalloc(&L.d_counters, effort_ctx::kMaxTiles * 4) == hipSuccess &&
              hipMalloc(&L.d_sliceCounts, effort_ctx::kMaxSlices * 4) == hipSuccess && hipMalloc(&L.d_queue, kQueueWords * 4) == hipSuccess;
    if (!ok) return false;
    hipMemset(L.d_counters, 0, effort_ctx::kMaxTiles * 4);
    hipMemset(L.d_sliceCounts, 0, effort_ctx::kMaxSlices * 4);
    hipMemset(L.d_queue, 0, kQueueWords * 4);
    hipMemset(L.d_cutoff, 0, 512);
    hipMemset(L.d_count, 0, 16);
    return true;
}
static std::mutex g_poolMutex;
static std::map<int, std::vector<hipStream_t>> g_streamPool;
static std::map<int, std::vector<hipEvent_t>> g_eventPool;
static hipStream_t pool_stream(int device) {
    std::lock_guard<std::mutex> lk(g_poolMutex);
    auto& pool = g_streamPool[device];
    if (!pool.empty()) { hipStream_t s = pool.back(); pool.pop_back(); return s; }
    hipStream_t s = nullptr;
    return hipStreamCreateWithFlags(&s, hipStreamNonBlocking) == hipSuccess ? s : nullptr;
}
static hipEvent_t pool_event(int device) {
    std::lock_guard<std::mutex> lk(g_poolMutex);
    auto& pool = g_eventPool[device];
    if (!pool.empty()) { hipEvent_t e = pool.back(); pool.pop_back(); return e; }
    hipEvent_t e = nullptr;
    return hipEventCreateWithFlags(&e, hipEventDisableTiming) == hipSuccess ? e : nullptr;
}
static void pool_put(int device, hipStream_t s) { if (s) { std::lock_guard<std::mutex> lk(g_poolMutex); g_streamPool[device].push_back(s); } }
static void pool_put(int device, hipEvent_t e) { if (e) { std::lock_guard<std::mutex> lk(g_poolMutex); g_eventPool[device].push_back(e); } }

static void lane_free(int device, Lane& L) {
    pool_put(device, L.own);
    pool_put(device, L.done);
    hipFree(L.d_cutoff); hipFree(L.d_count); hipFree(L.d_slabs); hipFree(L.d_counters); hipFree(L.d_sliceCounts); hipFree(L.d_queue);
    L = Lane();
}

extern "C" effort_ctx* effort_create(int device, void* stream) {
    if (hipSetDevice(device) != hipSuccess) return nullptr;
    effort_ctx* c = new (std::nothrow) effort_ctx();
    if (!c) return nullptr;
    c->device = device;
    c->stream = reinterpret_cast<hipStream_t>(stream);
    hipDeviceProp_t prop;
    if (hipGetDeviceProperties(&prop, device) == hipSuccess) c->env.numCU = prop.multiProcessorCount;
    {
        static std::mutex m; static std::map<int, bool> prepared;
        std::lock_guard<std::mutex> lk(m);
        if (!prepared[device]) {
            const hipError_t pe = bucket_mul_prepare_device();
            if (pe != hipSuccess) { snprintf(g_createErr, sizeof(g_createErr), "effort_create: kernel attributes: %s", hipGetErrorString(pe)); delete c; return nullptr; }
            prepared[device] = true;
        }
    }
    bool ok = lane_alloc(c, c->lane[0]) && hipMalloc(&c->d_blockScratch, 4096 * 4) == hipSuccess &&
              hipMalloc(&c->d_cos, 16) == hipSuccess && hipMalloc(&c->d_status, 16) == hipSuccess &&
              hipMalloc(&c->d_tstamp, kStampBytes) == hipSuccess;
    if (!ok) { snprintf(g_createErr, sizeof(g_createErr), "effort_create: out of device memory for the context scratch"); effort_destroy(c); return nullptr; }
    int khz = 0;
    if (hipDeviceGetAttribute(&khz, hipDeviceAttributeWallClockRate, device) == hipSuccess && khz > 0) c->wallClockKHz = khz;
    hipMemset(c->d_tstamp, 0, kStampBytes);
    { unsigned long long init[2] = {~0ull, 0ull}; hipMemcpy(c->d_tstamp, init, 16, hipMemcpyHostToDevice); }
    hipMemset(c->d_status, 0, 16);
    return c;
}

static hipError_t lane_mark(Lane& L) {
    if (!L.dirty) return hipSuccess;
    const hipError_t e = hipEventRecord(L.done, L.own);
    if (e == hipSuccess) L.dirty = false;
    return e;
}
static hipError_t wait_for_lanes(effort_ctx* c, hipStream_t st, uint32_t set) {
    for (int i = 0; i < kMaxLanes; i++) if (set >> i & 1u) {
        hipError_t e = lane_mark(c->lane[i]);
        if (e == hipSuccess) e = hipStreamWaitEvent(st, c->lane[i].done, 0);
        if (e != hipSuccess) return e;
    }
    return hipSuccess;
}
static unsigned long long capture_of(hipStream_t st) {
    hipStreamCaptureStatus cap = hipStreamCaptureStatusNone;
    unsigned long long id = 0;
    if (hipStreamGetCaptureInfo(st, &cap, &id) != hipSuccess) { (void)hipGetLastError(); return 0; }
    return cap == hipStreamCaptureStatusActive ? (id ? id : ~0ull) : 0ull;
}
static bool lanes_match_capture(effort_ctx* c, unsigned long long now) {
    uint32_t dropped = 0;
    if (!c->book.match_capture(now, &dropped)) { snprintf(c->err, sizeof(c->err), "%s", kLanesPendingBeforeCapture); return false; }
    for (int i = 0; i < kMaxLanes; i++) if (dropped >> i & 1u) c->lane[i].dirty = false;
    return true;
}
int join_lanes(effort_ctx* c) {
    if (c->book.pending_lanes()) {
        if (!lanes_match_capture(c, capture_of(c->stream))) return EFFORT_ERR_ARG;
        const hipError_t e = wait_for_lanes(c, c->stream, c->book.pending_lanes());
        if (e != hipSuccess) { snprintf(c->err, sizeof(c->err), "join: %s", hipGetErrorString(e)); return EFFORT_ERR_HIP; }
    }
    c->book.join();
    return EFFORT_OK;
}
int choose_lane(effort_ctx* c, LaneChoice& lc, int n, const effort_w* const* ws, const float* const* vs, const uint32_t* const* expNos,
                float* const* outs, const void* const* vAux, const float* const* resids) {
    if (lc.laned) {
        lc.capNow = capture_of(c->stream);
        if (!lanes_match_capture(c, lc.capNow)) return EFFORT_ERR_ARG;
        if (c->book.full()) JOIN_TRY(c);
        for (int i = 0; i < n; i++)
            lc.ranges.call(vs[i], expNos ? expNos[i] : nullptr, vAux ? vAux[i] : nullptr, resids ? resids[i] : nullptr, outs[i], ws[i]->inDim, ws[i]->outDim);
        lc.pick = c->book.pick(lc.ranges);
    } else if (c->book.nLanes > 1) {
        JOIN_TRY(c);
    }
    return EFFORT_OK;
}
int fork_lane(effort_ctx* c, LaneChoice& lc) {
    if (!lc.laned || lc.forked) return EFFORT_OK;
    Lane& L = c->lane[lc.pick.lane];
    bool wait = true;
    if (lc.capNow == 0) {
        const hipError_t q = hipStreamQuery(c->stream);
        if (q == hipSuccess) wait = false;
        else {
            (void)hipGetLastError();
            if (q != hipErrorNotReady) return fail(c, EFFORT_ERR_HIP, "hipStreamQuery", q);
        }
    }
    if (wait) {
        HIP_TRY(c, hipEventRecord(c->forkEv, c->stream));
        HIP_TRY(c, hipStreamWaitEvent(L.own, c->forkEv, 0));
    }
    lc.forked = true;
    L.dirty = true;
    const uint32_t waits = c->book.commit(lc.pick, lc.ranges, lc.capNow, wait);
    const hipError_t e = wait_for_lanes(c, L.own, waits);
    if (e != hipSuccess) { c->book.keep_pending(waits, lc.capNow); return fail(c, EFFORT_ERR_HIP, "lane wait", e); }
    return EFFORT_OK;
}

extern "C" int effort_set_overlap(effort_ctx* c, int lanes) {
    if (!c || lanes < 1 || lanes > kMaxLanes) return EFFORT_ERR_ARG;
    hipSetDevice(c->device);
    JOIN_TRY(c);
    if (lanes > 1) {
        if (!c->forkEv && !(c->forkEv = pool_event(c->device))) return fail(c, EFFORT_ERR_HIP, "set_overlap: event");
        for (int i = 0; i < lanes; i++) {
            Lane& L = c->lane[i];
            if (!L.d_slabs && !lane_alloc(c, L)) return fail(c, EFFORT_ERR_HIP, "set_overlap: out of device memory for a lane's scratch");
            if (!L.own && !(L.own = pool_stream(c->device))) return fail(c, EFFORT_ERR_HIP, "set_overlap: stream");
            if (!L.done && !(L.done = pool_event(c->device))) return fail(c, EFFORT_ERR_HIP, "set_overlap: event");
        }
    }
    c->book.reset(lanes); c->lastLane = 0;
    c->env.nLanes = c->book.nLanes;
    return EFFORT_OK;
}
extern "C" int effort_join(effort_ctx* c) { return c ? join_lanes(c) : EFFORT_ERR_ARG; }

extern "C" void effort_destroy(effort_ctx* c) {
    if (!c) return;
    hipSetDevice(c->device);
    for (int i = 0; i < kMaxLanes; i++) if (c->lane[i].own) hipStreamSynchronize(c->lane[i].own);
    hipStreamSynchronize(c->stream);
    comm_release(c);
    dense_release(c);
    if (c->ev) { for (int i = 0; i < effort_ctx::kMaxSamples * 2; i++) if (c->ev[i]) hipEventDestroy(c->ev[i]); delete[] c->ev; }
    for (int i = 0; i < kMaxLanes; i++) lane_free(c->device, c->lane[i]);
    pool_put(c->device, c->forkEv);
#define EFFORT_X(T, name) c->name.release();
    EFFORT_CTX_SCRATCH(EFFORT_X)
#undef EFFORT_X
    hipFree(c->d_blockScratch); hipFree(c->d_cos); hipFree(c->d_status); hipFree(c->d_tstamp);
    delete c;
}

extern "C" int effort_set_stream(effort_ctx* c, void* stream) {
    if (!c) return EFFORT_ERR_ARG;
    if (reinterpret_cast<hipStream_t>(stream) != c->stream && join_lanes(c) != EFFORT_OK) return EFFORT_ERR_HIP;
    c->stream = reinterpret_cast<hipStream_t>(stream);
    dense_set_stream(c);
    return EFFORT_OK;
}

extern "C" int effort_sync(effort_ctx* c) {
    if (!c) return EFFORT_ERR_ARG;
    JOIN_TRY(c);
    return HIP_RC(c, hipStreamSynchronize(c->stream));
}

extern "C" int effort_set_tuning(effort_ctx* c, int W, int E, int S) {
    if (!c) return EFFORT_ERR_ARG;
    if ((W || E) && !supported(W ? W : 16, E ? E : 1)) return fail(c, EFFORT_ERR_ARG, "set_tuning: unsupported (waves, elems)");
    if (S < 0) return EFFORT_ERR_ARG;
    c->env.tuneW = W; c->env.tuneE = E; c->env.tuneS = S;
    return EFFORT_OK;
}
extern "C" int effort_set_persistent(effort_ctx* c, int wgPerCU) {
    if (!c || wgPerCU < -1 || wgPerCU > 8) return EFFORT_ERR_ARG;
    c->env.persistent = wgPerCU;
    return EFFORT_OK;
}
extern "C" int effort_set_row_reuse(effort_ctx* c, int reuse) {
    if (!c) return EFFORT_ERR_ARG;
    c->rowReuse = reuse != 0;
    return EFFORT_OK;
}
extern "C" int effort_set_split_cutoff(effort_ctx* c, int split) {
    if (!c) return EFFORT_ERR_ARG;
    c->env.splitCutoff = split != 0;
    return EFFORT_OK;
}
extern "C" int effort_debug_hook_lane(effort_ctx* c, int lane) {
    if (!c || lane < 0 || lane >= c->book.nLanes) return EFFORT_ERR_ARG;
    c->lastLane = lane;
    return EFFORT_OK;
}
```

effort_amd/csrc/effort_internal.h:

```cpp
#pragma once
#include <hip/hip_runtime.h>
#include <hip/hip_fp16.h>
#include <stdint.h>

#include <map>
#include <mutex>
#include <utility>

namespace effort {

constexpr int kWave = 64;
constexpr int kProbes = 4096;
constexpr float kCutoffScale = 100000.0f;

enum Format : int { kFp16 = 0, kQ4 = 1 };

struct MulGeom {
    uint32_t inDim;
    uint32_t outDim;
    uint32_t cols;
    uint32_t rowsPerIn;
    uint32_t expertRows;
    uint32_t tiles;
    uint32_t slices;
    uint32_t sliceRows;
    uint32_t sliceLog2;
    uint32_t slots;
    uint32_t rowPitch;
    uint32_t numExperts;
    uint32_t elems;
};

struct OutlierIndex {
    const uint32_t* blockPtr;
    const uint32_t* entry;
    const uint32_t* meta;
};

#ifndef EFFORT_MAX_GROUP
#define EFFORT_MAX_GROUP 32
#endif
constexpr int kMaxGroup = EFFORT_MAX_GROUP;
constexpr int kMaxGeoms = 4;
#define EFFORT_GEOMS(X) X(16, 1) X(16, 2) X(16, 4) X(8, 1) X(8, 2) X(8, 4) X(4, 1) X(4, 2) X(4, 4) X(2, 4)
constexpr int kQueueWords = 11 * 16;
constexpr int kTraceOff = 512, kTraceItems = 4096;
enum Prologue : uint16_t { kPreNone = 0, kPreSiluGate = 1, kPreRmsNorm = 2 };
struct CallDesc {
    const uint16_t* buckets;
    const void* stats;
    const float* rankBound;
    const uint16_t* probes;
    const float* v;
    const uint32_t* expNo;
    float* out;
    OutlierIndex ol;
    uint16_t q;
    uint16_t bucketsTrim;
    uint32_t slabOff;
    uint16_t tileOff;
    uint16_t sliceOff;
    uint16_t geom;
    uint16_t pre;
    const void* vAux;
    const float* resid;
};
struct LdsPlan { uint32_t offM, offV[2], offA, offL, offC, offO, total; };
struct GroupKArgs {
    uint32_t count;
    uint32_t totalTiles;
    uint32_t persistent;
    uint32_t numCU;
    uint32_t ablate;
    uint32_t split;
    uint32_t cutJobs;
    uint32_t trace;
    LdsPlan lp;
    uint32_t totalItems;
    uint32_t staggerSleeps;
    uint32_t* groupDone;
    uint32_t* queue;
    float* slabs;
    uint32_t* counters;
    uint32_t* sliceCounts;
    float* cutoff;
    unsigned long long* tstamp;
    uint16_t wgEnd8[kMaxGroup];
    MulGeom geom[kMaxGeoms];
    CallDesc call[kMaxGroup];
};
static_assert(sizeof(CallDesc) == 112 && sizeof(GroupKArgs) <= 4000, "the launch descriptor must fit the kernel-argument segment");

__device__ __forceinline__ float half_bits_to_float(uint16_t h) { return __half2float(__ushort_as_half(h)); }

__device__ __forceinline__ float bf16_round(float f) {
    uint32_t u = __float_as_uint(f);
    if ((u & 0x7FFFFFFFu) > 0x7F800000u) u |= 0x00400000u;
    else u += 0x7FFFu + ((u >> 16) & 1u);
    return __uint_as_float(u & 0xFFFF0000u);
}

typedef __bf16 effort_bf16x2 __attribute__((ext_vector_type(2)));
typedef float effort_f32x2 __attribute__((ext_vector_type(2)));
__device__ __forceinline__ uint32_t bf16_pack2(float x, float y) {
    effort_f32x2 v; v[0] = x; v[1] = y;
    const effort_bf16x2 r = __builtin_convertvector(v, effort_bf16x2);
    uint32_t u; __builtin_memcpy(&u, &r, 4); return u;
}

#define EFFORT_DPP_SCAN(v, OP, IDENT)                                                                 \
    v = OP(v, __builtin_amdgcn_update_dpp(IDENT, v, 0x111, 0xf, 0xf, false));          \
    v = OP(v, __builtin_amdgcn_update_dpp(IDENT, v, 0x112, 0xf, 0xf, false));          \
    v = OP(v, __builtin_amdgcn_update_dpp(IDENT, v, 0x114, 0xf, 0xf, false));          \
    v = OP(v, __builtin_amdgcn_update_dpp(IDENT, v, 0x118, 0xf, 0xf, false));          \
    v = OP(v, __builtin_amdgcn_update_dpp(IDENT, v, 0x142, 0xa, 0xf, false));       \
    v = OP(v, __builtin_amdgcn_update_dpp(IDENT, v, 0x143, 0xc, 0xf, false));
__device__ __forceinline__ int dpp_op_add(int a, int b) { return a + b; }
__device__ __forceinline__ int dpp_op_umin(int a, int b) { return (int)min((uint32_t)a, (uint32_t)b); }
__device__ __forceinline__ int dpp_op_umax(int a, int b) { return (int)max((uint32_t)a, (uint32_t)b); }
__device__ __forceinline__ uint32_t wave_prefix_sum_u32(uint32_t x) { int v = (int)x; EFFORT_DPP_SCAN(v, dpp_op_add, 0) return (uint32_t)v; }
__device__ __forceinline__ uint32_t wave_sum_u32(uint32_t x) { int v = (int)x; EFFORT_DPP_SCAN(v, dpp_op_add, 0) return (uint32_t)__builtin_amdgcn_readlane(v, 63); }
__device__ __forceinline__ uint32_t wave_min_u32(uint32_t x) { int v = (int)x; EFFORT_DPP_SCAN(v, dpp_op_umin, -1) return (uint32_t)__builtin_amdgcn_readlane(v, 63); }
__device__ __forceinline__ uint32_t wave_max_u32(uint32_t x) { int v = (int)x; EFFORT_DPP_SCAN(v, dpp_op_umax, 0) return (uint32_t)__builtin_amdgcn_readlane(v, 63); }
__device__ __forceinline__ float wave_sum_f32(float x) {
    int v = __float_as_int(x);
#define EFFORT_FADD_(a, b) __float_as_int(__int_as_float(a) + __int_as_float(b))
    EFFORT_DPP_SCAN(v, EFFORT_FADD_, 0)
#undef EFFORT_FADD_
    return __int_as_float(__builtin_amdgcn_readlane(v, 63));
}

__device__ __forceinline__ float wave_max_f32(float x) {
    int v = __float_as_int(x);
#define EFFORT_FMAX_(a, b) __float_as_int(fmaxf(__int_as_float(a), __int_as_float(b)))
    EFFORT_DPP_SCAN(v, EFFORT_FMAX_, (int)0xFF800000)
#undef EFFORT_FMAX_
    return __int_as_float(__builtin_amdgcn_readlane(v, 63));
}
__device__ __forceinline__ float row16_sum_f32(float x) {
    int v = __float_as_int(x);
#define EFFORT_FADD_(a, b) __float_as_int(__int_as_float(a) + __int_as_float(b))
    v = EFFORT_FADD_(v, __builtin_amdgcn_update_dpp(0, v, 0x111, 0xf, 0xf, false));
    v = EFFORT_FADD_(v, __builtin_amdgcn_update_dpp(0, v, 0x112, 0xf, 0xf, false));
    v = EFFORT_FADD_(v, __builtin_amdgcn_update_dpp(0, v, 0x114, 0xf, 0xf, false));
    v = EFFORT_FADD_(v, __builtin_amdgcn_update_dpp(0, v, 0x118, 0xf, 0xf, false));
#undef EFFORT_FADD_
    return __int_as_float(v);
}

inline hipError_t allow_full_lds(const void* fn) {
    static std::mutex m;
    static std::map<std::pair<const void*, int>, bool> done;
    int dev = 0;
    hipError_t e = hipGetDevice(&dev);
    if (e != hipSuccess) return e;
    std::lock_guard<std::mutex> lk(m);
    bool& d = done[std::make_pair(fn, dev)];
    if (d) return hipSuccess;
    hipFuncAttributes fa;
    e = hipFuncGetAttributes(&fa, fn);
    if (e == hipSuccess) e = hipFuncSetAttribute(fn, hipFuncAttributeMaxDynamicSharedMemorySize, (int)(160u * 1024u - (uint32_t)fa.sharedSizeBytes));
    if (e == hipSuccess) d = true;
    return e;
}

bool dense_gemv_supported(uint32_t inDim, uint32_t outDim);
hipError_t launch_dense_gemv(const uint16_t* W_f16, const float* v, float* out, uint32_t inDim, uint32_t outDim, hipStream_t st);
hipError_t launch_dense_gemv_expert(const uint16_t* W_f16, const uint32_t* expNo, const float* v, float* out, uint32_t inDim, uint32_t outDim,
                                    uint32_t numExperts, hipStream_t st);
hipError_t launch_find_cutoff(const float* v, const uint16_t* probes, const uint32_t* expNo, uint32_t q,
                              float* cutoff, uint32_t* dispatchCount, unsigned long long* tstamp, hipStream_t st);

struct LaunchedVariant { uint32_t W, E, fused, compact, lean, persistent, grid, totalItems; };
hipError_t launch_bucket_mul(Format fmt, int wavesPerGroup, int elemsPerLane, const GroupKArgs& ga, hipStream_t st, LaunchedVariant* ran = nullptr);
int bucket_mul_variants(Format fmt, int* rows, int maxRows);
hipError_t bucket_mul_prepare_device();
hipError_t launch_find_cutoff_group(const GroupKArgs& ga, hipStream_t st);
size_t bucket_mul_lds_bytes(Format fmt, int wavesPerGroup, int elemsPerLane, const MulGeom& g, bool lean);
uint32_t bucket_mul_max_candidates(int wavesPerGroup);
uint32_t bucket_mul_ol_lds_floats();
int bucket_mul_occupancy(Format fmt, int wavesPerGroup, int elemsPerLane, size_t ldsBytes);

hipError_t launch_calc_dispatch(Format fmt, const void* stats, const float* v, const uint32_t* expNo,
                                const float* cutoff, const MulGeom& g, float* dispatch, uint32_t* count,
                                uint32_t* ctxCount, uint32_t* blockScratch, hipStream_t st);

hipError_t launch_convert_fp16(const uint16_t* W, uint32_t outDim, uint32_t inDim, uint16_t* buckets, uint32_t pitchCols,
                               uint16_t* stats, uint16_t* probes, uint16_t* scratchVals, int* status, hipStream_t st);

hipError_t launch_convert_q4(const uint16_t* core2, uint32_t inDim, uint32_t outDim, uint32_t cnt, uint16_t* buckets, float* stats, uint16_t* probes,
                             float* outliers, int numCU, hipStream_t st);

hipError_t launch_compact_means(const void* stats_f16x4, uint16_t* means, uint32_t rows, hipStream_t st);
hipError_t launch_rank_bound(Format fmt, const uint16_t* buckets, uint32_t pitchCols, const void* stats, uint32_t numExperts, uint32_t rowsPerIn,
                             uint32_t inDim, uint32_t cols, float* rowScratch, float* rankBound, hipStream_t st);
hipError_t launch_add_rmsnorm_mul(float* h, const float* delta, const uint16_t* w, float* out, uint32_t n, hipStream_t st);
hipError_t launch_rope_kv(const float* xq, const float* xk, const float* xv, float* qOut, float* kCache, float* vCache,
                          const uint32_t* pos, uint32_t numHeads, uint32_t numHeadsKV, uint32_t headDim, float ropeBase, uint32_t maxTokens,
                          int* status, hipStream_t st);
hipError_t launch_attention(const float* q, const float* kCache, const float* vCache, const uint32_t* pos, float* out,
                            uint32_t numHeads, uint32_t headDim, uint32_t maxTokens, hipStream_t st);
hipError_t launch_rope_attention(const float* xq, const float* xk, const float* xv, float* kCache, float* vCache, const uint32_t* pos,
                                 float* out, uint32_t numHeads, uint32_t numHeadsKV, uint32_t headDim, uint32_t maxTokens, float ropeBase,
                                 int* status, hipStream_t st);
hipError_t launch_silu_mul(const float* x1, const float* x3, float* out, uint32_t n, hipStream_t st);
hipError_t launch_fetch_row(const uint16_t* emb, const uint32_t* id, float* out, uint32_t n, hipStream_t st);
hipError_t launch_top2_softmax(const float* gate, uint32_t n, uint32_t* idx, float* val, hipStream_t st);
hipError_t launch_mix2(const float* f0, const float* f1, const float* val, float* out, uint32_t n, hipStream_t st);
hipError_t launch_mix2_add(float* h, const float* f0, const float* f1, const float* val, uint32_t n, hipStream_t st);
bool moe_route_supported(uint32_t n, uint32_t numExperts);
hipError_t launch_moe_route(const float* h, const uint16_t* w, const uint16_t* gateW, uint32_t n, uint32_t numExperts, float* gateOut,
                            uint32_t* idx, float* val, hipStream_t st);
hipError_t launch_argmax(const float* logits, uint32_t n, uint32_t* idOut, uint32_t* pos, uint32_t* history, uint32_t historyLen,
                         int* status, hipStream_t st);
hipError_t launch_fetch_rows(const uint16_t* emb, const uint32_t* ids, float* out, uint32_t n, uint32_t rows, hipStream_t st);
hipError_t launch_add_rmsnorm_mul_rows(float* h, const float* delta, const uint16_t* w, float* out, uint32_t n, uint32_t rows, hipStream_t st);
hipError_t launch_rope_kv_rows(const float* xq, const float* xk, const float* xv, float* qOut, float* kCache, float* vCache, uint32_t pos0,
                               uint32_t rows, uint32_t numHeads, uint32_t numHeadsKV, uint32_t headDim, float ropeBase, hipStream_t st);
hipError_t launch_attention_rows(const float* q, const float* kCache, const float* vCache, uint32_t pos0, uint32_t rows, float* out,
                                 uint32_t numHeads, uint32_t headDim, hipStream_t st);
hipError_t launch_moe_route_rows(const float* h, const uint16_t* w, const uint16_t* gateW, uint32_t n, uint32_t numExperts, float* gateOut,
                                 uint32_t* idx, float* val, uint32_t rows, hipStream_t st);
hipError_t launch_mix2_add_rows(float* h, const float* f, const float* val, uint32_t n, uint32_t rows, hipStream_t st);

bool dense_gemm_rows_supported(uint32_t inDim, uint32_t outDim);
size_t dense_gemm_rows_partial_floats(uint32_t inDim, uint32_t outDim, uint32_t rows);
hipError_t launch_dense_gemm_rows(const uint16_t* W_f16, const float* x, uint16_t* xhScratch , float* partScratch, float* out,
                                  uint32_t inDim, uint32_t outDim, uint32_t rows, hipStream_t st);
size_t dense_gemm_rows_routed_partial_floats(uint32_t inDim, uint32_t outDim, uint32_t rows);
size_t dense_gemm_rows_routed_group_words();
hipError_t launch_dense_gemm_rows_routed(const uint16_t* W_f16, uint32_t numExperts, const uint32_t* idx2, const float* x, uint32_t xPerSlot,
                                         uint16_t* xhScratch , float* partScratch, uint32_t* groupScratch,
                                         float* out, uint32_t inDim, uint32_t outDim, uint32_t rows, hipStream_t st);
hipError_t launch_attention_block(const float* q, const float* kCache, const float* vCache, uint32_t pos0, uint32_t rows, float* out,
                                  uint32_t numHeads, uint32_t headDim, hipStream_t st);

hipError_t launch_sample(const float* logits, uint32_t n, const void* params, uint32_t* idOut, uint32_t* pos, uint32_t* history, uint32_t historyLen,
                         int* status, uint32_t* topkIdx, float* topkVal, hipStream_t st);
hipError_t launch_topk(const float* logits, uint32_t n, uint32_t k, uint32_t* idx, float* val, hipStream_t st);

hipError_t launch_f32_to_f16(const float* in, uint16_t* out, uint32_t n, hipStream_t st);
hipError_t launch_cosine(const float* a, const float* b, uint32_t n, float* out3, hipStream_t st);
hipError_t launch_validate_outliers(const float* outliers, uint64_t n, uint32_t inDim, uint32_t outDim, int* bad, hipStream_t st);
hipError_t launch_build_outlier_index(const float* outliers, uint64_t n, uint32_t inDim, uint32_t outDim, uint32_t* rowPtr,
                                      uint32_t* blockPtr, uint32_t* entry, uint32_t* meta, uint32_t* tmp, hipStream_t st);
hipError_t launch_sort_pairs_u32(const uint32_t* keysIn, uint32_t* keysOut, const uint32_t* valsIn, uint32_t* valsOut, uint64_t n, hipStream_t st);

}
```

effort_amd/csrc/mul.hip:

```cpp
#include <cstdlib>

#include "host.h"

using namespace effort;

static PlanEnv call_env(PlanEnv env, bool laned, bool thinEffort) {
    env.laned = laned; env.thinEffort = thinEffort;
#ifdef EFFORT_LAB
    static const uint32_t ablate = getenv("EFFORT_ABLATE") ? (uint32_t)atoi(getenv("EFFORT_ABLATE")) : 0u;
    static const bool noJobs = getenv("EFFORT_NO_CUTJOBS") != nullptr, noCompact = getenv("EFFORT_NO_COMPACT_MEANS") != nullptr;
    env.ablate = ablate; env.noJobs = noJobs; env.noCompact = noCompact;
    if (getenv("EFFORT_TAIL_CALLS")) {
        env.tailCalls = atoi(getenv("EFFORT_TAIL_CALLS"));
        env.tailMult = getenv("EFFORT_TAIL_MULT") ? atoi(getenv("EFFORT_TAIL_MULT")) : 2;
    }
#endif
    return env;
}
static PlanCall plan_call(const effort_w* w, int pre, bool resid) {
    return PlanCall{w->inDim, w->outDim, w->cols, w->rowsPerIn, w->rowPitch, w->numExperts, w->means16 != nullptr, (uint16_t)pre, resid};
}
static bool thin_effort(int n, const double* efforts) {
    double sum = 0.0;
    for (int i = 0; i < n; i++) sum += efforts[i];
    return sum < 0.08 * n;
}

static int do_group(effort_ctx* c, Format fmt, int n, const effort_w* const* ws, const float* const* vs,
                    const uint32_t* const* expNos, float* const* outs, const double* efforts,
                    const int* prologues = nullptr, const void* const* vAux = nullptr, const float* const* resids = nullptr) {
    if (!c || !ws || !vs || !outs || !efforts) return fail(c, EFFORT_ERR_ARG, "bucketmul: null argument");
    if (n < 1 || n > kMaxGroup) return fail(c, EFFORT_ERR_ARG, "bucketmul: group size outside 1..32");
    PlanCall pc[kMaxGroup];
    for (int i = 0; i < n; i++) {
        if (!ws[i] || !vs[i] || !outs[i]) return fail(c, EFFORT_ERR_ARG, "bucketmul: null argument");
        if (ws[i]->dead) return fail(c, EFFORT_ERR_ARG, "bucketmul: the handle was freed (its buffers live on only for its column shards)");
        if (ws[i]->fmt != fmt) return fail(c, EFFORT_ERR_KIND, "bucketmul: weight handle of the wrong kind");
        if (!(efforts[i] >= 0.0 && efforts[i] <= 1.0)) return fail(c, EFFORT_ERR_EFFORT, "bucketmul: effort outside [0,1]");
        const int pre = prologues ? prologues[i] : 0;
        if (pre < 0 || pre > 2 || (pre && (!vAux || !vAux[i]))) return fail(c, EFFORT_ERR_ARG, "bucketmul: bad input prologue");
        if (pre && c->env.splitCutoff) return fail(c, EFFORT_ERR_KIND, "bucketmul: input prologues need the fused cutoff");
        if (pre && fmt == kQ4 && ws[i]->olBlockPtr && (uint32_t)ws[i]->inDim > bucket_mul_ol_lds_floats())
            return fail(c, EFFORT_ERR_SHAPE, "bucketmul: an input prologue on a Q4 handle with outliers needs inDim <= 16384 (materialise the input, or register without outliers)");
        pc[i] = plan_call(ws[i], pre, resids && resids[i]);
    }
    LaneChoice lc;
    lc.laned = c->book.nLanes > 1 && !c->timing && !c->env.clock;
    const PlanEnv env = call_env(c->env, lc.laned, thin_effort(n, efforts));
    GroupPlan plan;
    if (plan_group(fmt, env, n, pc, &plan) != EFFORT_OK) return fail(c, plan.err, plan.msg);
    const bool tm = c->timing && c->nSamples < effort_ctx::kMaxSamples;
    hipEvent_t* ev = tm ? c->ev + 2 * c->nSamples : nullptr;
    OK_TRY(choose_lane(c, lc, n, ws, vs, expNos, outs, vAux, resids));
    Lane& L = c->lane[lc.pick.lane];
    const hipStream_t st = lc.laned ? L.own : c->stream;
    c->lastLane = lc.pick.lane;
    if (tm) HIP_TRY(c, hipEventRecord(ev[0], st));
    L.lastLaunches = 0;
    for (uint32_t l = 0; l < plan.nLaunches; l++) {
        const LaunchPlan& lp = plan.launch[l];
        GroupKArgs ga;
        memset(&ga, 0, sizeof(ga));
        ga.groupDone = L.d_counters + effort_ctx::kMaxTiles - 1;
        ga.slabs = L.d_slabs; ga.counters = L.d_counters; ga.sliceCounts = L.d_sliceCounts; ga.cutoff = L.d_cutoff + lp.first;
        ga.tstamp = env.clock ? c->d_tstamp : nullptr;
        ga.ablate = env.ablate; ga.trace = (env.clock && c->trace) ? 1u : 0u;
        ga.split = (env.splitCutoff ? 1u : 0u) | (lp.compact ? 4u : 0u) | (c->rowReuse ? 8u : 0u);
        ga.numCU = (uint32_t)env.numCU; ga.queue = L.d_queue;
        ga.count = lp.count; ga.totalTiles = lp.totalTiles; ga.totalItems = lp.totalItems;
        ga.persistent = lp.persistent; ga.cutJobs = lp.cutJobs; ga.staggerSleeps = lp.staggerSleeps;
        for (uint32_t k = 0; k < lp.count; k++) {
            const int i = (int)(lp.first + k);
            const effort_w* w = ws[i];
            const CallPlan& p = plan.call[i];
            CallDesc& a = ga.call[k];
            a.buckets = w->buckets; a.stats = lp.compact ? (const void*)w->means16 : w->stats; a.rankBound = w->rankBound; a.probes = w->probes; a.v = vs[i];
            a.expNo = expNos ? expNos[i] : nullptr; a.out = outs[i];
            a.ol = OutlierIndex{fmt == kQ4 ? w->olBlockPtr : nullptr, w->olEntry, w->olMeta};
            a.q = (uint16_t)(int)((double)(kProbes - 1) * (1.0 - efforts[i]));
            a.bucketsTrim = (uint16_t)w->viewTrim;
            a.pre = pc[i].pre; a.vAux = a.pre ? vAux[i] : nullptr; a.resid = resids ? resids[i] : nullptr;
            a.slabOff = p.slabOff; a.tileOff = (uint16_t)p.tileOff; a.sliceOff = (uint16_t)p.sliceOff; a.geom = (uint16_t)p.geom;
            ga.geom[p.geom] = p.g;
            ga.wgEnd8[k] = (uint16_t)p.itemEnd8;
            L.lastSliceOff[i] = p.sliceOff; L.lastSlices[i] = p.g.slices;
        }
        OK_TRY(fork_lane(c, lc));
        if (env.splitCutoff && !(env.ablate & 1u)) HIP_TRY(c, launch_find_cutoff_group(ga, st));
        HIP_TRY(c, launch_bucket_mul(fmt, plan.W, plan.E, ga, st, &L.lastVariant[l]));
        L.lastLaunches = l + 1u;
    }
    L.lastCalls = (uint32_t)n;
    if (tm) { HIP_TRY(c, hipEventRecord(ev[1], st)); c->nSamples++; }
    return EFFORT_OK;
}

extern "C" int effort_bucketmul(effort_ctx* c, const effort_w* w, const float* v, const uint32_t* expNo, float* out, double effort) {
    return do_group(c, kFp16, 1, &w, &v, &expNo, &out, &effort);
}
extern "C" int effort_bucketmul_q4(effort_ctx* c, const effort_w* w, const float* v, const uint32_t* expNo, float* out, double effort) {
    return do_group(c, kQ4, 1, &w, &v, &expNo, &out, &effort);
}
extern "C" int effort_bucketmul_group(effort_ctx* c, int n, const effort_w* const* ws, const float* const* vs,
                                      const uint32_t* const* expNos, float* const* outs, const double* efforts) {
    return do_group(c, kFp16, n, ws, vs, expNos, outs, efforts);
}
extern "C" int effort_bucketmul_group_fused(effort_ctx* c, int n, const effort_w* const* ws, const float* const* vs,
                                            const uint32_t* const* expNos, float* const* outs, const double* efforts,
                                            const int* prologues, const void* const* vAux, const float* const* resids) {
    return do_group(c, kFp16, n, ws, vs, expNos, outs, efforts, prologues, vAux, resids);
}
extern "C" int effort_bucketmul_q4_group_fused(effort_ctx* c, int n, const effort_w* const* ws, const float* const* vs,
                                               const uint32_t* const* expNos, float* const* outs, const double* efforts,
                                               const int* prologues, const void* const* vAux, const float* const* resids) {
    return do_group(c, kQ4, n, ws, vs, expNos, outs, efforts, prologues, vAux, resids);
}
extern "C" int effort_bucketmul_q4_group(effort_ctx* c, int n, const effort_w* const* ws, const float* const* vs,
                                         const uint32_t* const* expNos, float* const* outs, const double* efforts) {
    return do_group(c, kQ4, n, ws, vs, expNos, outs, efforts);
}

extern "C" int effort_calc_dispatch(effort_ctx* c, const effort_w* w, const float* v, const uint32_t* expNo, double effort,
                                    float* dispatch, uint32_t* count) {
    if (!c || !w || !v || !dispatch || w->dead) return fail(c, EFFORT_ERR_ARG, "calc_dispatch: null argument (or a freed handle)");
    if (!(effort >= 0.0 && effort <= 1.0)) return fail(c, EFFORT_ERR_EFFORT, "calc_dispatch: effort outside [0,1]");
    JOIN_TRY(c);
    Lane& L = c->lane[0];
    c->lastLane = 0;
    const PlanCall pc = plan_call(w, 0, false);
    GroupPlan plan;
    if (plan_group(w->fmt, call_env(c->env, false, false), 1, &pc, &plan) != EFFORT_OK) return fail(c, plan.err, "calc_dispatch: geometry");
    const MulGeom& g = plan.call[0].g;
    const uint32_t q = (uint32_t)(int)((double)(kProbes - 1) * (1.0 - effort));
    HIP_TRY(c, launch_find_cutoff(v, w->probes, expNo, q, L.d_cutoff, L.d_count, nullptr, c->stream));
    HIP_TRY(c, launch_calc_dispatch(w->fmt, w->stats, v, expNo, L.d_cutoff, g, dispatch, count, L.d_count, c->d_blockScratch, c->stream));
    L.lastCalls = 1; L.lastSlices[0] = 0;
    L.lastLaunches = 0;
    return EFFORT_OK;
}

extern "C" int effort_group_dispatch_count(effort_ctx* c, int idx, uint32_t* host_out) {
    if (!c || !host_out || idx < 0 || (uint32_t)idx >= c->lane[c->lastLane].lastCalls) return EFFORT_ERR_ARG;
    JOIN_TRY(c);
    Lane& L = c->lane[c->lastLane];
    if (L.lastSlices[idx] == 0) {
        HIP_TRY(c, hipMemcpyAsync(host_out, L.d_count, 4, hipMemcpyDeviceToHost, c->stream));
        HIP_TRY(c, hipStreamSynchronize(c->stream));
        return EFFORT_OK;
    }
    static thread_local uint32_t h[effort_ctx::kMaxSlices];
    HIP_TRY(c, hipMemcpyAsync(h, L.d_sliceCounts + L.lastSliceOff[idx], (size_t)L.lastSlices[idx] * 4, hipMemcpyDeviceToHost, c->stream));
    HIP_TRY(c, hipStreamSynchronize(c->stream));
    uint32_t n = 0;
    for (uint32_t i = 0; i < L.lastSlices[idx]; i++) n += h[i];
    *host_out = n;
    return EFFORT_OK;
}
extern "C" int effort_debug_slice_counts(effort_ctx* c, int idx, uint32_t* host, int maxSlices) {
    if (!c || !host || idx < 0 || (uint32_t)idx >= c->lane[c->lastLane].lastCalls || maxSlices < 1) return EFFORT_ERR_ARG;
    JOIN_TRY(c);
    Lane& L = c->lane[c->lastLane];
    const uint32_t n = L.lastSlices[idx] < (uint32_t)maxSlices ? L.lastSlices[idx] : (uint32_t)maxSlices;
    if (n) HIP_TRY(c, hipMemcpyAsync(host, L.d_sliceCounts + L.lastSliceOff[idx], (size_t)n * 4, hipMemcpyDeviceToHost, c->stream));
    HIP_TRY(c, hipStreamSynchronize(c->stream));
    return (int)n;
}
extern "C" int effort_debug_plan(int q4, int numCU, int lanes, int n, const int* inDim, const int* outDim, const int* percentLoad,
                                 const int* prologue, const int* hasResid, const double* effort, int persistent, int tuneW, int tuneE, int tuneS,
                                 int* we, int* slices, int* tiles, int* sliceRows, int* launchOf,
                                 int* launchPersistent, int* launchCutJobs, int* launchCompact, int* launchStagger) {
    if (numCU < 1 || lanes < 1 || lanes > kMaxLanes || n < 1 || n > kMaxGroup || !inDim || !outDim || !effort || !we || !slices || !tiles ||
        !sliceRows || !launchOf || !launchPersistent || !launchCutJobs || !launchCompact || !launchStagger) return EFFORT_ERR_ARG;
    const Format fmt = q4 ? kQ4 : kFp16;
    PlanEnv env = effort_ctx::scratch_env();
    env.numCU = numCU; env.nLanes = lanes; env.persistent = persistent; env.tuneW = tuneW; env.tuneE = tuneE; env.tuneS = tuneS;
    PlanCall pc[kMaxGroup];
    for (int i = 0; i < n; i++) {
        const int load = q4 ? 8 : (percentLoad ? percentLoad[i] : 16);
        if (inDim[i] <= 0 || outDim[i] <= 0 || check_shape((uint32_t)inDim[i], (uint32_t)outDim[i]) != EFFORT_OK || load < 1 || load > 16) return EFFORT_ERR_SHAPE;
        if (!(effort[i] >= 0.0 && effort[i] <= 1.0)) return EFFORT_ERR_EFFORT;
        const uint32_t cols = (uint32_t)outDim[i] / (q4 ? 32u : 16u);
        pc[i] = PlanCall{(uint32_t)inDim[i], (uint32_t)outDim[i], cols, (uint32_t)load, cols * 2u, 1u, !q4, (uint16_t)(prologue ? prologue[i] : 0), hasResid && hasResid[i]};
    }
    GroupPlan plan;
    const int rc = plan_group(fmt, call_env(env, lanes > 1, thin_effort(n, effort)), n, pc, &plan);
    if (rc != EFFORT_OK) return rc;
    we[0] = plan.W; we[1] = plan.E;
    for (int i = 0; i < n; i++) {
        const CallPlan& p = plan.call[i];
        slices[i] = (int)p.g.slices; tiles[i] = (int)p.g.tiles; sliceRows[i] = (int)p.g.sliceRows; launchOf[i] = (int)p.launch;
    }
    for (uint32_t l = 0; l < plan.nLaunches; l++) {
        const LaunchPlan& lp = plan.launch[l];
        launchPersistent[l] = (int)lp.persistent; launchCutJobs[l] = (int)lp.cutJobs; launchCompact[l] = lp.compact ? 1 : 0; launchStagger[l] = (int)lp.staggerSleeps;
    }
    return (int)plan.nLaunches;
}
extern "C" int effort_debug_variants(int q4, int* rows, int maxRows) {
    if (maxRows < 0 || (maxRows > 0 && !rows)) return EFFORT_ERR_ARG;
    return bucket_mul_variants(q4 ? kQ4 : kFp16, rows, maxRows);
}
extern "C" int effort_debug_occupancy(effort_ctx* c, int q4, int W, int E, int ldsBytes) {
    if (!c || !supported(W, E)) return EFFORT_ERR_ARG;
    return bucket_mul_occupancy(q4 ? kQ4 : kFp16, W, E, (size_t)ldsBytes);
}
extern "C" int effort_debug_last_variant(effort_ctx* c, int launch, int* out8) {
    if (!c || !out8 || launch < 0) return EFFORT_ERR_ARG;
    const Lane& L = c->lane[c->lastLane];
    if ((uint32_t)launch >= L.lastLaunches) return EFFORT_ERR_ARG;
    const LaunchedVariant& v = L.lastVariant[launch];
    const uint32_t w[8] = {v.W, v.E, v.fused, v.compact, v.lean, v.persistent, v.grid, v.totalItems};
    for (int i = 0; i < 8; i++) out8[i] = (int)w[i];
    return EFFORT_OK;
}
extern "C" int effort_group_cutoff(effort_ctx* c, int idx, float* host_out) {
    if (!c || !host_out || idx < 0 || (uint32_t)idx >= c->lane[c->lastLane].lastCalls) return EFFORT_ERR_ARG;
    JOIN_TRY(c);
    Lane& L = c->lane[c->lastLane];
    HIP_TRY(c, hipMemcpyAsync(host_out, L.d_cutoff + idx, 4, hipMemcpyDeviceToHost, c->stream));
    return HIP_RC(c, hipStreamSynchronize(c->stream));
}
extern "C" int effort_last_dispatch_count(effort_ctx* c, uint32_t* host_out) { return effort_group_dispatch_count(c, 0, host_out); }
extern "C" int effort_last_cutoff(effort_ctx* c, float* host_out) { return effort_group_cutoff(c, 0, host_out); }

#ifdef EFFORT_LAB
static constexpr bool kLabBuild = true;
#else
static constexpr bool kLabBuild = false;
#endif
static int lab_only(effort_ctx* c) { return fail(c, EFFORT_ERR_KIND, "device-clock stamps / traces are compiled into libeffort_hip_lab.so only (EFFORT_HIP_LIB=lab)"); }
extern "C" int effort_is_lab_build(void) { return kLabBuild ? 1 : 0; }

static int ensure_timing(effort_ctx* c) {
    if (c->ev) return EFFORT_OK;
    c->ev = new (std::nothrow) hipEvent_t[effort_ctx::kMaxSamples * 2]();
    if (!c->ev) return EFFORT_ERR_HIP;
    for (int i = 0; i < effort_ctx::kMaxSamples * 2; i++) HIP_TRY(c, hipEventCreate(&c->ev[i]));
    return EFFORT_OK;
}
extern "C" int effort_enable_kernel_timing(effort_ctx* c, int enable) {
    if (!c) return EFFORT_ERR_ARG;
    if (!kLabBuild && enable >= 2) return lab_only(c);
    if (enable == 1) OK_TRY(ensure_timing(c));
    c->timing = enable == 1;
    c->env.clock = kLabBuild && enable != 0;
    c->trace = kLabBuild && enable == 3;
    if (c->trace) HIP_TRY(c, hipMemsetAsync(c->d_tstamp + kTraceOff, 0, (size_t)kTraceItems * 96, c->stream));
    c->nSamples = 0;
    HIP_TRY(c, hipMemsetAsync(c->d_tstamp, 0, 4096, c->stream));
    return HIP_RC(c, hipMemsetAsync(c->d_tstamp, 0xFF, 8, c->stream));
}

extern "C" int effort_debug_stamps(effort_ctx* c, unsigned long long* host32) {
    if (!c || !host32) return EFFORT_ERR_ARG;
    if (!kLabBuild) return lab_only(c);
    HIP_TRY(c, hipMemcpyAsync(host32, c->d_tstamp + 8, 192, hipMemcpyDeviceToHost, c->stream));
    unsigned long long lines[32 * 8];
    HIP_TRY(c, hipMemcpyAsync(lines, c->d_tstamp + 64, sizeof(lines), hipMemcpyDeviceToHost, c->stream));
    HIP_TRY(c, hipStreamSynchronize(c->stream));
    for (int i = 0; i < 8; i++) { host32[24 + i] = 0; for (int l = 0; l < 32; l++) host32[24 + i] += lines[l * 8 + i]; }
    return EFFORT_OK;
}

extern "C" int effort_debug_trace(effort_ctx* c, unsigned long long* host, int maxRecords) {
    if (!c || !host || maxRecords < 1 || maxRecords > kTraceItems) return EFFORT_ERR_ARG;
    if (!kLabBuild) return lab_only(c);
    HIP_TRY(c, hipMemcpyAsync(host, c->d_tstamp + kTraceOff, (size_t)maxRecords * 64, hipMemcpyDeviceToHost, c->stream));
    HIP_TRY(c, hipMemcpyAsync(host + (size_t)maxRecords * 8, c->d_tstamp + kTraceOff + (size_t)kTraceItems * 8, (size_t)maxRecords * 32, hipMemcpyDeviceToHost, c->stream));
    return HIP_RC(c, hipStreamSynchronize(c->stream));
}

extern "C" int effort_kernel_clock(effort_ctx* c, double* mul_us_avg, int* n_launches) {
    if (!c) return EFFORT_ERR_ARG;
    if (!kLabBuild) return lab_only(c);
    unsigned long long h[4] = {0, 0, 0, 0};
    HIP_TRY(c, hipMemcpyAsync(h, c->d_tstamp, 32, hipMemcpyDeviceToHost, c->stream));
    HIP_TRY(c, hipStreamSynchronize(c->stream));
    if (mul_us_avg) *mul_us_avg = h[3] ? (double)h[2] / (double)h[3] * 1000.0 / c->wallClockKHz : 0.0;
    if (n_launches) *n_launches = (int)h[3];
    return HIP_RC(c, hipMemsetAsync(c->d_tstamp + 2, 0, 16, c->stream));
}

extern "C" int effort_kernel_timing(effort_ctx* c, double* mul_us, double* cutoff_us, double* integrate_us, int* n) {
    if (!c) return EFFORT_ERR_ARG;
    HIP_TRY(c, hipStreamSynchronize(c->stream));
    double b = 0;
    float ms;
    for (int i = 0; i < c->nSamples; i++) { HIP_TRY(c, hipEventElapsedTime(&ms, c->ev[2 * i], c->ev[2 * i + 1])); b += ms; }
    const int ns = c->nSamples ? c->nSamples : 1;
    if (cutoff_us) *cutoff_us = 0.0;
    if (mul_us) *mul_us = b * 1000.0 / ns;
    if (integrate_us) *integrate_us = 0.0;
    if (n) *n = c->nSamples;
    c->nSamples = 0;
    return EFFORT_OK;
}
```

effort_amd/csrc/plan.h:

```cpp
#pragma once
#include "effort_internal.h"

namespace effort {

constexpr int kMaxLaunches = kMaxGroup / kMaxGeoms + 1;

struct PlanEnv {
    int numCU = 256, nLanes = 1;
    bool laned = false;
    int persistent = -1;
    int tuneW = 0, tuneE = 0, tuneS = 0;
    bool splitCutoff = false, clock = false;
    uint32_t ablate = 0;
    bool noJobs = false, noCompact = false;
    size_t slabBytes = 0;
    uint32_t maxTiles = 0, maxSlices = 0;
    bool thinEffort = false;
    int tailCalls = 0, tailMult = 0;
};
struct PlanCall {
    uint32_t inDim, outDim, cols, rowsPerIn, rowPitch, numExperts;
    bool hasMeans16;
    uint16_t pre;
    bool hasResid;
};
struct CallPlan {
    MulGeom g;
    uint32_t mult;
    uint32_t launch, geom;
    uint32_t slabOff, tileOff, sliceOff;
    uint32_t itemEnd8;
};
struct LaunchPlan {
    uint32_t first, count;
    uint32_t persistent, cutJobs, staggerSleeps;
    bool compact;
    uint32_t totalItems, totalTiles, realItems;
};
struct GroupPlan {
    int W = 0, E = 0;
    int err = 0;
    const char* msg = "";
    uint32_t nLaunches = 0;
    CallPlan call[kMaxGroup];
    LaunchPlan launch[kMaxLaunches];
};

bool supported(int W, int E);
int plan_group(Format fmt, const PlanEnv& env, int n, const PlanCall* calls, GroupPlan* plan);

}
```

effort_amd/csrc/plan.hip:

```cpp
#include <cstring>

#include "../../include/effort_hip.h"
#include "plan.h"

namespace effort {

static uint32_t round8(uint32_t x) { return (x + 7u) / 8u * 8u; }
static uint32_t min_slices(uint32_t inDim) { return round8((inDim + 511u) / 512u); }
static uint32_t max_slices(uint32_t inDim) { return round8((inDim + 127u) / 128u); }
static uint32_t tiles_at(const PlanCall& w, int E) { return (w.cols + 64 * E - 1) / (64 * E); }
static uint32_t group_tiles(int n, const PlanCall* ws, int E) {
    uint32_t t = 0;
    for (int i = 0; i < n; i++) t += tiles_at(ws[i], E);
    return t;
}
static uint32_t padded_items(uint32_t tiles, uint32_t slices) { return round8(tiles * slices); }
static uint32_t padded_min_items(int n, const PlanCall* ws, int E) {
    uint32_t t = 0;
    for (int i = 0; i < n; i++) t += padded_items(tiles_at(ws[i], E), min_slices(ws[i].inDim));
    return t;
}
static bool fits_one_round(const PlanEnv& env, int n, uint32_t tiles, uint32_t allTiles, uint32_t s) {
    const bool same = allTiles == (uint32_t)n * tiles;
    return (same ? (uint32_t)n * padded_items(tiles, s) : allTiles * s + 7u * (uint32_t)n) <= (uint32_t)env.numCU;
}

bool supported(int W, int E) {
#define EFFORT_CASE(w, e) if (W == w && E == e) return true;
    EFFORT_GEOMS(EFFORT_CASE)
#undef EFFORT_CASE
    return false;
}

static uint32_t q4_one_round(const PlanEnv& env, uint32_t inDim, uint32_t groupTiles1) {
    if (env.nLanes > 1 || env.tuneS || !groupTiles1) return 0;
    const uint32_t sMin = (inDim + 831u) / 832u;
    const uint32_t S = (uint32_t)env.numCU * 15u / 8u / groupTiles1;
    return S >= sMin && S >= 2u ? S : 0u;
}
static uint32_t q4_one_per_cu(const PlanEnv& env, uint32_t inDim, uint32_t tiles1, int n, uint32_t groupTiles1) {
    if (env.nLanes > 1 || env.tuneS || n < 3 || n > 9) return 0;
    const uint32_t sMin = (inDim + 831u) / 832u, hi = max_slices(inDim);
    auto fits = [&](uint32_t s) { return fits_one_round(env, n, tiles1, groupTiles1 ? groupTiles1 : (uint32_t)n * tiles1, s); };
    uint32_t S = sMin > 2u ? sMin : 2u;
    if (!fits(S)) return 0;
    const uint32_t top = env.thinEffort ? min_slices(inDim) : hi;
    while (S < top && S < hi && fits(S + 1u)) S++;
    return S;
}
static uint32_t pick_slices(const PlanEnv& env, Format fmt, const PlanCall& w, int groupSize, int E, uint32_t groupTiles = 0, bool fill = true) {
    const uint32_t tiles = tiles_at(w, E);
    const uint32_t lo = min_slices(w.inDim), hi = max_slices(w.inDim);
    if (fmt != kFp16 && (E == 1 || groupSize >= 8) && fill) {
        const uint32_t S = q4_one_per_cu(env, w.inDim, tiles, groupSize, groupTiles);
        if (S) return S;
    }
    if (fmt != kFp16 && E == 1 && groupSize >= 8 && groupTiles) {
        const uint32_t S = q4_one_round(env, w.inDim, groupTiles);
        if (S) return S;
    }
    if (groupSize >= 8 && (fmt != kFp16 || !fill || env.nLanes > 1 || env.thinEffort)) return lo;
    const uint32_t target = (E == 1 && fmt == kFp16) ? (uint32_t)env.numCU : (uint32_t)env.numCU * 3u / 4u;
    const uint32_t allTiles = groupTiles ? groupTiles : (uint32_t)groupSize * tiles;
    uint32_t S = (target / allTiles + 4u) / 8u * 8u;
    if (S < lo) S = lo;
    if (S > hi) S = hi;
    if ((w.inDim & (w.inDim - 1u)) == 0u && (S & (S - 1u)) != 0u) {
        uint32_t up = 8u;
        while (up < S) up <<= 1;
        S = up <= hi ? up : up >> 1;
    }
    if (fmt == kFp16 && fill && groupSize >= 3 && env.nLanes <= 1) {
        auto fits = [&](uint32_t s) { return fits_one_round(env, groupSize, tiles, allTiles, s); };
        if (fits(S)) { if (!env.thinEffort) while (S < hi && fits(S + 1u)) S++; }
        else {
            uint32_t s2 = S;
            while (s2 > lo && !fits(s2)) s2--;
            if (fits(s2)) S = s2;
        }
    }
    return S;
}

static int pick_elems(const PlanEnv& env, Format fmt, int n, const PlanCall* ws) {
    if (env.tuneE) return env.tuneE;
    if (fmt != kFp16) {
        if (n < 8) return 1;
        uint32_t inMax = 0;
        for (int i = 0; i < n; i++) inMax = inMax > ws[i].inDim ? inMax : ws[i].inDim;
        if (n < 10) {
            uint32_t tMax = 0;
            bool same = true;
            for (int i = 0; i < n; i++) {
                const uint32_t t = tiles_at(ws[i], 1);
                same = same && (tMax == 0 || t == tMax); tMax = tMax > t ? tMax : t;
            }
            if (q4_one_per_cu(env, inMax, tMax, n, same ? 0u : group_tiles(n, ws, 1))) return 1;
        }
        if (n >= 10) {
            if (q4_one_round(env, inMax, group_tiles(n, ws, 1))) return 1;
        }
        return 2;
    }
    if (env.tuneS) return 2;
    auto items = [&](int E) {
        uint32_t t = 0;
        const uint32_t gt = group_tiles(n, ws, E);
        for (int i = 0; i < n; i++) t += tiles_at(ws[i], E) * pick_slices(env, fmt, ws[i], n, E, gt, false);
        return t;
    };
    const uint32_t numCU = (uint32_t)env.numCU;
    auto only_wide_tiles_fit = [&] { return padded_min_items(n, ws, 1) > numCU && padded_min_items(n, ws, 2) <= numCU; };
    auto fill = [&](int E) {
        double used = 0, have = 0;
        for (int i = 0; i < n; i++) { used += ws[i].cols; have += (double)tiles_at(ws[i], E) * 64 * E; }
        return have > 0 ? used / have : 1.0;
    };
    const double f1 = fill(1), f2 = fill(2), f4 = fill(4), best = f1 > f2 ? (f1 > f4 ? f1 : f4) : (f2 > f4 ? f2 : f4);
    if (n >= 8) {
        const uint32_t i4 = items(4);
        if (((i4 > numCU / 2 && i4 <= numCU) || i4 >= 3u * numCU) && f4 >= 0.8 * best) return 4;
        if (f2 >= 0.8 * best) return 2;
        if (env.nLanes <= 1 && f2 >= 0.7 * best && only_wide_tiles_fit()) return 2;
        return 1;
    }
    const uint32_t i2 = items(2);
    if (f2 < 0.8 * best) return 1;
    if (n >= 3 && f4 >= 0.8 * best && env.nLanes <= 1) {
        uint32_t lo2 = 0, lo4 = 0;
        for (int i = 0; i < n; i++) {
            const uint32_t lo = min_slices(ws[i].inDim);
            lo2 += tiles_at(ws[i], 2) * lo; lo4 += tiles_at(ws[i], 4) * lo;
        }
        if (lo2 > numCU && lo4 <= numCU * 15u / 16u) return 4;
    }
    bool narrow = true;
    for (int i = 0; i < n; i++) narrow = narrow && ws[i].cols <= 256u;
    if (narrow && f1 >= 0.8 * best && n >= 3 && env.nLanes <= 1 && f2 >= 0.8 * best && only_wide_tiles_fit()) return 2;
    if (narrow && f1 >= 0.8 * best && !(env.nLanes > 1 && n >= 3)) return 1;
    return (i2 * 10u < numCU * 3u / 4u * 6u && items(1) > i2) ? 1 : 2;
}

static uint32_t tile_floats(Format fmt, int E) { return (fmt == kFp16 ? 16u : 32u) * (uint32_t)E * 64u; }
static int choose_geom(const PlanEnv& env, Format fmt, const PlanCall& w, int groupSize, int W, int E, uint32_t groupTiles, uint32_t sliceMult, MulGeom* g) {
    memset(g, 0, sizeof(*g));
    g->inDim = w.inDim; g->outDim = w.outDim; g->cols = w.cols; g->rowsPerIn = w.rowsPerIn;
    g->expertRows = w.rowsPerIn * w.inDim; g->numExperts = w.numExperts;
    g->tiles = tiles_at(w, E);
    g->elems = (uint32_t)E;
    g->rowPitch = w.rowPitch;
    const uint32_t tileFloats = tile_floats(fmt, E);
    const size_t ldsMax = 160 * 1024;
    uint32_t S;
    if (env.tuneS) S = env.tuneS;
    else {
        const uint32_t want = pick_slices(env, fmt, w, groupSize, E, groupTiles) * sliceMult;
        const uint32_t cap = (env.numCU * 2u) / g->tiles / 8 * 8;
        S = cap < want ? cap : want;
    }
    if (S > w.inDim) S = w.inDim / 8 * 8;
    if (S < 1) S = 1;
    const uint32_t maxCand = bucket_mul_max_candidates(W);
    for (;;) {
        g->sliceRows = (w.inDim + S - 1) / S;
        g->slices = (w.inDim + g->sliceRows - 1) / g->sliceRows;
        g->sliceLog2 = 0; while ((1u << g->sliceLog2) < g->sliceRows) g->sliceLog2++;
        g->slots = fmt == kFp16 ? (g->rowsPerIn << g->sliceLog2) : g->sliceRows * 8u;
        const size_t lds = bucket_mul_lds_bytes(fmt, W, E, *g, true);
        const bool fits = lds <= ldsMax && g->slots <= maxCand && (size_t)g->slots * 4 + (size_t)g->sliceRows * 8 + 1024 <= 65536 &&
                          (fmt == kFp16 ? (1u << g->sliceLog2) <= 64u * (uint32_t)W : g->sliceRows <= 128u * (uint32_t)W);
        const size_t slab = (size_t)g->slices * g->tiles * tileFloats * 4;
        if (fits && slab <= env.slabBytes) break;
        if (!fits) { S += 1; if (S > w.inDim + 8) return EFFORT_ERR_SHAPE; }
        else return EFFORT_ERR_SHAPE;
    }
    return EFFORT_OK;
}
static int plan_fail(GroupPlan* P, int code, const char* msg) { P->err = code; P->msg = msg; return code; }

static uint32_t geom_index(MulGeom* geoms, uint32_t& n, const MulGeom& g) {
    uint32_t k = 0;
    while (k < n && memcmp(&geoms[k], &g, sizeof(g)) != 0) k++;
    if (k == n && n < (uint32_t)kMaxGeoms) geoms[n++] = g;
    return k;
}

static void finish_launch(Format fmt, const PlanEnv& env, int W, const PlanCall* ws, const GroupPlan* P, LaunchPlan* lp) {
    const uint32_t R = env.persistent < 0 ? 2u : (uint32_t)env.persistent;
    const uint32_t perCU = (env.persistent < 0 && fmt == kFp16 && !env.laned) ? 6u : R;
    lp->persistent = (R && lp->realItems > (uint32_t)env.numCU * perCU) ? R : 0u;
    bool plain = true;
    for (uint32_t i = 0; i < lp->count; i++) plain = plain && !ws[lp->first + i].pre;
    lp->cutJobs = (lp->persistent && !env.splitCutoff && plain && !env.noJobs) ? (lp->count + 7u) / 8u * 8u : 0u;
    const bool leanGrid = lp->persistent == 0u && W == 8 && !env.clock && !env.ablate;
    bool compact = fmt == kFp16 && !env.noCompact && (leanGrid || (lp->persistent != 0u && plain));
    for (uint32_t i = 0; compact && !leanGrid && i < lp->count; i++) compact = !ws[lp->first + i].hasResid;
    for (uint32_t i = 0; compact && i < lp->count; i++) {
        const MulGeom& g = P->call[lp->first + i].g;
        compact = ws[lp->first + i].hasMeans16 && g.inDim % 2u == 0u && g.sliceRows % 2u == 0u;
    }
    lp->compact = compact;
    lp->staggerSleeps = (lp->persistent && fmt == kQ4 && !env.laned) ? 11u : 0u;
}

int plan_group(Format fmt, const PlanEnv& env, int n, const PlanCall* ws, GroupPlan* P) {
    P->err = EFFORT_OK; P->msg = ""; P->nLaunches = 0;
    const bool laned = env.laned;
    const int W = env.tuneW ? env.tuneW : 8;
    const int E = pick_elems(env, fmt, n, ws);
    P->W = W; P->E = E;
    const char* const noGeometry = "bucketmul: no launch geometry for this shape/tuning";
    if (!supported(W, E)) return plan_fail(P, EFFORT_ERR_ARG, noGeometry);
    const uint32_t groupTiles = group_tiles(n, ws, E);
    MulGeom g1[kMaxGroup], g2[kMaxGroup];
    uint32_t it1[kMaxGroup], base = 0;
    for (int i = 0; i < n; i++) {
        const int rc = choose_geom(env, fmt, ws[i], n, W, E, groupTiles, 1, &g1[i]);
        if (rc != EFFORT_OK) return plan_fail(P, rc, noGeometry);
        it1[i] = padded_items(g1[i].tiles, g1[i].slices);
        base += it1[i];
    }
    int thinFrom = n;
    if (E == 2 && n >= 8 && !laned && !env.tuneS && env.persistent < 0 && !env.thinEffort) {
        const uint32_t round = 2u * (uint32_t)env.numCU, over = base % round;
        if (base > round && over != 0u && over * 32u <= round * 7u && (fmt != kFp16 || base <= 6u * (uint32_t)env.numCU)) {
            int tc = 0;
            uint32_t thin = 0;
            while (tc < n && tc < 4 && (tc < 2 || thin < over)) thin += it1[n - 1 - tc++];
            MulGeom seen[kMaxGeoms];
            uint32_t nSeen = 0, extra = 0;
            bool ok = thin >= over;
            for (int i = 0; ok && i < n; i++) {
                const bool t = i >= n - tc;
                if (t) {
                    ok = choose_geom(env, fmt, ws[i], n, W, E, groupTiles, 2, &g2[i]) == EFFORT_OK;
                    const uint32_t it2 = padded_items(g2[i].tiles, g2[i].slices);
                    ok = ok && it2 > it1[i];
                    extra += it2 - it1[i];
                }
                ok = ok && geom_index(seen, nSeen, t ? g2[i] : g1[i]) < (uint32_t)kMaxGeoms;
            }
            if (ok && (fmt != kFp16 || base + extra <= 6u * (uint32_t)env.numCU)) thinFrom = n - tc;
        }
    }
    uint32_t nGeoms = 0, wg = 0;
    MulGeom geoms[kMaxGeoms];
    size_t slabOff = 0; uint32_t tileOff = 0, sliceOff = 0;
    LaunchPlan* lp = nullptr;
    auto begin = [&](uint32_t firstCall) {
        lp = &P->launch[P->nLaunches++];
        memset(lp, 0, sizeof(*lp));
        lp->first = firstCall;
        nGeoms = 0; wg = 0;
    };
    begin(0);
    for (int i = 0; i < n; i++) {
        uint32_t mult = i >= thinFrom ? 2u : 1u;
        MulGeom g = mult == 2u ? g2[i] : g1[i];
        if (n >= 8 && !env.tuneS && env.tailMult) {
            mult = 1;
            if (i >= n - env.tailCalls) mult = (uint32_t)env.tailMult;
            if (env.tailMult >= 4 && i >= n - env.tailCalls && i < n - env.tailCalls / 2) mult = (uint32_t)env.tailMult / 2;
            const int rc = choose_geom(env, fmt, ws[i], n, W, E, groupTiles, mult, &g);
            if (rc != EFFORT_OK) return plan_fail(P, rc, noGeometry);
        }
        uint32_t gi = geom_index(geoms, nGeoms, g);
        if (gi == (uint32_t)kMaxGeoms) {
            finish_launch(fmt, env, W, ws, P, lp);
            begin((uint32_t)i);
            gi = geom_index(geoms, nGeoms, g);
        }
        CallPlan& a = P->call[i];
        const size_t slab = (size_t)g.slices * g.tiles * tile_floats(fmt, E) * 4;
        if (tileOff + g.tiles + 1 > env.maxTiles || sliceOff + g.slices > env.maxSlices || slabOff + slab > env.slabBytes)
            return plan_fail(P, EFFORT_ERR_SHAPE, "bucketmul: group exceeds the context scratch");
        a.g = g; a.mult = mult; a.launch = P->nLaunches - 1u; a.geom = gi;
        a.slabOff = (uint32_t)(slabOff / 256); a.tileOff = tileOff; a.sliceOff = sliceOff;
        wg += padded_items(g.tiles, g.slices);
        if (wg / 8u > 0xFFFFu) return plan_fail(P, EFFORT_ERR_SHAPE, "bucketmul: group exceeds the launch descriptor's item range");
        a.itemEnd8 = wg / 8u;
        lp->count = (uint32_t)i - lp->first + 1u;
        lp->totalItems = wg; lp->totalTiles += g.tiles; lp->realItems += g.tiles * g.slices;
        slabOff += (slab + 255) / 256 * 256; tileOff += g.tiles; sliceOff += g.slices;
    }
    finish_launch(fmt, env, W, ws, P, lp);
    return EFFORT_OK;
}

}
```

effort_amd/runtime.py:

```python
from __future__ import annotations

import ctypes as C

import torch

from . import _lib


class Gpu:
    def __init__(self, device: int | None = None):
        if not torch.cuda.is_available():
            raise RuntimeError("effort_amd needs an AMD GPU (torch.cuda.is_available() is False); there is no CPU fallback")
        self.device = torch.cuda.current_device() if device is None else int(device)
        self._lib = _lib.lib()
        with torch.cuda.device(self.device):
            stream = torch.cuda.current_stream(self.device).cuda_stream
            self.ctx = self._lib.effort_create(self.device, C.c_void_p(stream))
        self.has_comm = False
        self.dense_rocblas = False
        if not self.ctx:
            raise RuntimeError("effort_create failed: " + (self._lib.effort_last_error(None) or b"").decode())
        self._stream = stream

    def _bind_stream(self):
        cur = torch.cuda.current_stream(self.device)
        stream = cur.cuda_stream
        if stream != self._stream:
            old = getattr(self, "_stream_obj", None)
            if old is not None and not torch.cuda.is_current_stream_capturing():
                try:
                    cur.wait_stream(old)
                except RuntimeError:
                    pass
            self._lib.effort_set_stream(self.ctx, C.c_void_p(stream))
            self._stream = stream
        self._stream_obj = cur

    def check(self, rc: int, where: str):
        if rc != 0:
            detail = self._lib.effort_last_error(self.ctx)
            raise _lib.EffortError(rc, where, detail.decode() if detail else "")

    def eval(self):
        self.check(self._lib.effort_sync(self.ctx), "gpu.eval")

    def set_overlap(self, lanes: int = 4):
        self._bind_stream()
        self.check(self._lib.effort_set_overlap(self.ctx, int(lanes)), "set_overlap")

    def join(self):
        self.check(self._lib.effort_join(self.ctx), "join")

    def set_row_reuse(self, reuse: bool = True):
        self.check(self._lib.effort_set_row_reuse(self.ctx, int(bool(reuse))), "set_row_reuse")

    @staticmethod
    def comm_unique_id() -> bytes:
        buf = (C.c_char * 128)()
        rc = _lib.lib().effort_comm_unique_id(buf)
        if rc != 0:
            raise _lib.EffortError(rc, "comm_unique_id")
        return bytes(buf)

    def comm_create(self, rank: int, world: int, uid: bytes):
        if len(uid) != 128:
            raise ValueError("the communicator id is 128 bytes")
        self._bind_stream()
        self.check(self._lib.effort_comm_create(self.ctx, int(rank), int(world), C.c_char_p(uid)), "comm_create")
        self.has_comm = True

    def comm_destroy(self):
        self.check(self._lib.effort_comm_destroy(self.ctx), "comm_destroy")
        self.has_comm = False

    @property
    def comm_world(self) -> int:
        return int(self._lib.effort_comm_world(self.ctx))

    @property
    def comm_rank(self) -> int:
        return int(self._lib.effort_comm_rank(self.ctx))

    def allgather_outputs(self, send: torch.Tensor, recv: torch.Tensor, count: int | None = None):
        n = int(send.numel() if count is None else count)
        if not (send.is_cuda and recv.is_cuda and send.dtype == torch.float32 and recv.dtype == torch.float32 and send.is_contiguous()
                and recv.is_contiguous() and send.numel() >= n and recv.numel() >= n * self.comm_world):
            raise ValueError("allgather_outputs: contiguous f32 CUDA tensors, recv holding world * count elements")
        self._bind_stream()
        self.check(self._lib.effort_allgather_outputs(self.ctx, C.c_void_p(send.data_ptr()), C.c_void_p(recv.data_ptr()), n), "allgather_outputs")

    def hook_lane(self, lane: int):
        self.check(self._lib.effort_debug_hook_lane(self.ctx, int(lane)), "hook_lane")

    def set_tuning(self, waves: int = 0, elems: int = 0, slices: int = 0):
        self.check(self._lib.effort_set_tuning(self.ctx, waves, elems, slices), "set_tuning")

    def set_split_cutoff(self, split: bool = True):
        self.check(self._lib.effort_set_split_cutoff(self.ctx, int(split)), "set_split_cutoff")

    def enable_kernel_timing(self, mode: int = 1):
        self._bind_stream()
        self.check(self._lib.effort_enable_kernel_timing(self.ctx, int(mode)), "enable_kernel_timing")

    def kernel_clock(self):
        us, n = C.c_double(), C.c_int()
        self.check(self._lib.effort_kernel_clock(self.ctx, C.byref(us), C.byref(n)), "kernel_clock")
        return {"mul_us": us.value, "launches": n.value}

    def set_persistent(self, wg_per_cu: int = -1):
        self.check(self._lib.effort_set_persistent(self.ctx, int(wg_per_cu)), "set_persistent")

    def set_dense_backend(self, rocblas: bool = False):
        self.check(self._lib.effort_set_dense_backend(self.ctx, int(bool(rocblas))), "set_dense_backend")
        self.dense_rocblas = bool(rocblas)

    def convert_status(self) -> int:
        n = C.c_int(0)
        self.check(self._lib.effort_convert_status(self.ctx, C.byref(n)), "convert_status")
        return int(n.value)

    def debug_stamps(self):
        buf = (C.c_ulonglong * 32)()
        self.check(self._lib.effort_debug_stamps(self.ctx, buf), "debug_stamps")
        return list(buf)

    def slice_counts(self, idx: int = 0, n: int = 4096):
        buf = (C.c_uint32 * n)()
        k = self._lib.effort_debug_slice_counts(self.ctx, int(idx), buf, n)
        if k < 0:
            self.check(k, "slice_counts")
        return list(buf[:k])

    def debug_trace(self, n: int = 4096):
        buf = (C.c_ulonglong * (12 * n))()
        self.check(self._lib.effort_debug_trace(self.ctx, buf, n), "debug_trace")
        return [tuple(buf[8 * i:8 * i + 8]) + tuple(buf[8 * n + 4 * i:8 * n + 4 * i + 4]) for i in range(n)]

    def kernel_timing(self):
        mul, cut, integ, n = C.c_double(), C.c_double(), C.c_double(), C.c_int()
        self.check(self._lib.effort_kernel_timing(self.ctx, C.byref(mul), C.byref(cut), C.byref(integ), C.byref(n)), "kernel_timing")
        return {"mul_us": mul.value, "cutoff_us": cut.value, "integrate_us": integ.value, "samples": n.value}

    def last_dispatch_count(self, idx: int = 0) -> int:
        n = C.c_uint32()
        self.check(self._lib.effort_group_dispatch_count(self.ctx, int(idx), C.byref(n)), "last_dispatch_count")
        return int(n.value)

    def last_cutoff(self, idx: int = 0) -> float:
        x = C.c_float()
        self.check(self._lib.effort_group_cutoff(self.ctx, int(idx), C.byref(x)), "last_cutoff")
        return float(x.value)

    def last_variant(self, launch: int = 0) -> dict:
        buf = (C.c_int * 8)()
        self.check(self._lib.effort_debug_last_variant(self.ctx, int(launch), buf), "last_variant")
        return {"variant": (buf[0], buf[1], bool(buf[2]), bool(buf[3]), bool(buf[4])), "persistent": buf[5], "grid": buf[6], "totalItems": buf[7]}

    def close(self):
        if getattr(self, "ctx", None):
            self._lib.effort_destroy(self.ctx)
            self.ctx = None

    def __del__(self):
        try:
            self.close()
        except Exception:
            pass


def plan(calls, *, q4: bool = False, numCU: int = 256, lanes: int = 1, persistent: int = -1, waves: int = 0, elems: int = 0, slices: int = 0) -> dict:
    n = len(calls)
    rows = [tuple(c) + (16, 0, 0)[len(c) - 3:] for c in calls]
    ints = lambda k: (C.c_int * n)(*[int(r[k]) for r in rows])
    out = [(C.c_int * max(n, 2))() for _ in range(9)]
    k = _lib.lib().effort_debug_plan(int(q4), numCU, lanes, n, ints(0), ints(1), ints(3), ints(4), ints(5), (C.c_double * n)(*[float(r[2]) for r in rows]),
                                     persistent, waves, elems, slices, *out)
    if k < 0:
        raise _lib.EffortError(k, "plan")
    we, per_call, per_launch = out[0], out[1:5], out[5:]
    res = {"W": we[0], "E": we[1]}
    res.update({name: list(a[:n]) for name, a in zip(("slices", "tiles", "sliceRows", "launch"), per_call)})
    res.update({name: list(a[:k]) for name, a in zip(("persistent", "cutJobs", "compact", "stagger"), per_launch)})
    return res


def variants(q4: bool = False) -> list[tuple]:
    n = _lib.lib().effort_debug_variants(int(q4), None, 0)
    if n < 0:
        raise _lib.EffortError(n, "variants")
    buf = (C.c_int * (5 * n))()
    k = _lib.lib().effort_debug_variants(int(q4), buf, n)
    if k != n:
        raise _lib.EffortError(min(k, -1), "variants")
    return [(buf[5 * i], buf[5 * i + 1], bool(buf[5 * i + 2]), bool(buf[5 * i + 3]), bool(buf[5 * i + 4])) for i in range(n)]


def lanes(ops, *, lanes: int = 4) -> list[dict]:
    kinds = {"launch": 0, "timed": 1, "join": 2}
    words = []
    for op in ops:
        kind, cap, busy, rd, wr = tuple(op) + (0, (), ())[len(op) - 2:]
        words += [kinds[kind], int(cap), int(bool(busy)), len(rd), len(wr)]
        for lo, hi in list(rd) + list(wr):
            words += [int(lo), int(hi)]
    n, W = len(ops), 18
    out = (C.c_int64 * max(n * W, 1))()
    k = _lib.lib().effort_debug_lanes(lanes, n, (C.c_int64 * max(len(words), 1))(*words), len(words), out)
    if k < 0:
        raise _lib.EffortError(k, "lanes")
    members = lambda mask: tuple(i for i in range(lanes) if mask >> i & 1)
    res = []
    for i in range(n):
        r = out[i * W:(i + 1) * W]
        res.append({"rc": r[0], "joined_first": bool(r[1]), "joined": members(r[2]), "lane": r[3], "fork_waited": bool(r[4]), "waits": members(r[5]),
                    "pending": members(r[6]), "nextLane": r[7], "busyStreak": r[8], "migrated": bool(r[9]),
                    "reads": list(r[10:10 + lanes]), "writes": list(r[14:14 + lanes])})
    return res


_gpus: dict[int, Gpu] = {}


def gpu(device: int | None = None) -> Gpu:
    if not torch.cuda.is_available():
        raise RuntimeError("effort_amd needs an AMD GPU (torch.cuda.is_available() is False); there is no CPU fallback")
    d = torch.cuda.current_device() if device is None else int(device)
    g = _gpus.get(d)
    if g is None:
        g = _gpus[d] = Gpu(d)
    return g
```

include/effort_hip_debug.h:

```cpp
#ifndef EFFORT_HIP_DEBUG_H
#define EFFORT_HIP_DEBUG_H

#include "effort_hip.h"

#ifdef __cplusplus
extern "C" {
#endif

EFFORT_API int effort_set_tuning(effort_ctx* ctx, int wavesPerGroup, int elemsPerLane, int rowSlices);
EFFORT_API int effort_set_split_cutoff(effort_ctx* ctx, int split);

EFFORT_API int effort_set_persistent(effort_ctx* ctx, int wgPerCU);

EFFORT_API int effort_debug_hook_lane(effort_ctx* ctx, int lane);

EFFORT_API int effort_is_lab_build(void);
EFFORT_API int effort_enable_kernel_timing(effort_ctx* ctx, int enable);
EFFORT_API int effort_kernel_clock(effort_ctx* ctx, double* mul_us_avg, int* n_launches);
EFFORT_API int effort_kernel_timing(effort_ctx* ctx, double* mul_us_avg, double* cutoff_us_avg,
                         double* integrate_us_avg, int* n_samples);
EFFORT_API int effort_debug_occupancy(effort_ctx* ctx, int q4, int waves, int elems, int ldsBytes);
EFFORT_API int effort_debug_stamps(effort_ctx* ctx, unsigned long long* host32);
EFFORT_API int effort_debug_slice_counts(effort_ctx* ctx, int idx, uint32_t* host, int maxSlices);
EFFORT_API int effort_debug_plan(int q4, int numCU, int lanes, int n, const int* inDim, const int* outDim, const int* percentLoad,
                      const int* prologue, const int* hasResid, const double* effort, int persistent, int tuneW, int tuneE, int tuneS,
                      int* we, int* slices, int* tiles, int* sliceRows, int* launchOf,
                      int* launchPersistent, int* launchCutJobs, int* launchCompact, int* launchStagger);
EFFORT_API int effort_debug_check_bundle(int q4, int inDim, int outDim, int percentLoad, int numExperts, int rowPitchBytes);
EFFORT_API int effort_debug_variants(int q4, int* rows, int maxRows);
EFFORT_API int effort_debug_last_variant(effort_ctx* ctx, int launch, int* out8);
#define EFFORT_LANES_LAUNCH 0
#define EFFORT_LANES_TIMED 1
#define EFFORT_LANES_JOIN 2
#define EFFORT_LANES_OUT_WORDS 18
EFFORT_API int effort_debug_lanes(int lanes, int nOps, const int64_t* ops, int64_t nWords, int64_t* out);
EFFORT_API int effort_debug_trace(effort_ctx* ctx, unsigned long long* host, int maxRecords);

#ifdef __cplusplus
}
#endif
#endif
```

Before: 21510.

## Pair row slices per workgroup with LDS carry in persistent fp16 bucket mul

Adds a chained mode where one persistent workgroup processes slice s and then slice s+4 of the same tile back-to-back. The first pass keeps its partial sums in LDS and the second adds them before writing, so only four slab slices are written instead of eight. This is meant to cut slab traffic and the reduction work, and to shorten queue pulls by prefetching the paired item directly. It adds a new item-mapping scheme and grid sizing, and is gated to fp16 compact persistent launches with eight slices, enabled by default only for laned plans.

```diff
diff --git a/effort_amd/_lib.py b/effort_amd/_lib.py
--- a/effort_amd/_lib.py
+++ b/effort_amd/_lib.py
@@ -66,6 +66,10 @@
     "effort_group_cutoff": (C.c_int, [_P, C.c_int, C.POINTER(C.c_float)]),
     "effort_debug_occupancy": (C.c_int, [_P, C.c_int, C.c_int, C.c_int, C.c_int]),
     "effort_set_persistent": (C.c_int, [_P, C.c_int]),
+    "effort_set_slice_pairs": (C.c_int, [_P, C.c_int]),
+    "effort_debug_plan_pairs": (C.c_int, [C.c_int, C.c_int, C.c_int, C.c_int, _P, _P, _P, _P, _P, _P, C.c_int, C.c_int, C.c_int, C.c_int, C.c_int, _P, _P, _P]),
+    "effort_debug_pair_items": (C.c_int, [C.c_int, _P, _P, C.c_int]),
+    "effort_debug_last_pairs": (C.c_int, [_P, C.c_int, _P]),
     "effort_debug_hook_lane": (C.c_int, [_P, C.c_int]),
     "effort_add_rmsnorm_mul": (C.c_int, [_P, _P, _P, _P, _P, C.c_int]),
     "effort_rope_kv": (C.c_int, [_P, _P, _P, _P, _P, _P, _P, _P, C.c_int, C.c_int, C.c_int, C.c_int, C.c_float]),
@@ -136,7 +140,7 @@
         import torch
         l = C.CDLL(LIB_PATH)
         for name, (res, args) in _SIGS.items():
-            if (name.startswith("effort_debug_") or name == "effort_is_lab_build") and os.environ.get("EFFORT_HIP_LIB") and not hasattr(l, name):
+            if (name.startswith("effort_debug_") or name in ("effort_is_lab_build", "effort_set_slice_pairs")) and os.environ.get("EFFORT_HIP_LIB") and not hasattr(l, name):
                 continue
             fn = getattr(l, name)
             fn.restype = res
diff --git a/effort_amd/csrc/bucket_mul.hip b/effort_amd/csrc/bucket_mul.hip
--- a/effort_amd/csrc/bucket_mul.hip
+++ b/effort_amd/csrc/bucket_mul.hip
@@ -131,7 +131,17 @@
 }
 struct ItemRef { uint32_t ci, t, s; };
 
+template <bool CHAIN>
 __device__ __forceinline__ bool locate_item(const GroupKArgs& ga, const uint32_t item, ItemRef& r) {
+    if constexpr (CHAIN) {
+        if (ga.split & 16u) {
+            const ChainSlot cs = chain_locate(ga.wgEnd8, ga.count, item);
+            const uint32_t cc = __builtin_amdgcn_readfirstlane(cs.ci);
+            if (cc >= ga.count) return false;
+            r.ci = cc; r.s = cs.pair; r.t = cs.k;
+            return cs.k < ga.geom[ga.call[cc].geom].tiles;
+        }
+    }
     uint32_t ci = 0;
     for (uint32_t i = 0; i + 1 < ga.count; i++) if ((item >> 3) >= (uint32_t)ga.wgEnd8[i]) ci = i + 1;
     ci = __builtin_amdgcn_readfirstlane(ci);
@@ -211,7 +221,9 @@
 
 template <int FMT, int E, int W, bool FUSED, bool COMPACT, bool PERSIST, typename Prefetch>
 __device__ __forceinline__ void mul_item(const GroupKArgs& ga, const uint32_t item, const ItemRef& ref, char* smem, const LdsPlan& lp, uint32_t& cachedCall,
-                                         float& cachedCutoff, const uint32_t par, const bool staged, const bool firstItem, Prefetch prefetch) {
+                                         float& cachedCutoff, const uint32_t par, const bool staged, const bool firstItem, const uint32_t chainIn, Prefetch prefetch) {
+    constexpr bool kChain = PERSIST && COMPACT && !FUSED && FMT == kFp16;
+    const uint32_t chain = kChain ? chainIn : 0u;
     constexpr int NACC = Fmt<FMT>::kAcc;
     constexpr int TILE_F = NACC * E * 64;
     constexpr int TILE_L = Fmt<FMT>::kSlots * E * 64;
@@ -260,8 +272,8 @@
     const float* means = reinterpret_cast<const float*>(smem + offM);
 
     const uint32_t j0 = s * B;
-    uint32_t vSlabOff = (s * g.tiles + t) * (uint32_t)(TILE_F * 4), vSlabBytes = (uint32_t)min((size_t)0xFFFFFFFFu, (size_t)g.slices * g.tiles * TILE_F * 4);
-    uint32_t vSlices = g.slices, vSliceStride = g.tiles * (uint32_t)(TILE_F * 4);
+    uint32_t vSlabOff = ((chain ? (s & 3u) : s) * g.tiles + t) * (uint32_t)(TILE_F * 4), vSlabBytes = (uint32_t)min((size_t)0xFFFFFFFFu, (size_t)g.slices * g.tiles * TILE_F * 4);
+    uint32_t vSlices = chain ? 4u : g.slices, vSliceStride = g.tiles * (uint32_t)(TILE_F * 4);
     if constexpr (!PERSIST) asm volatile("" : "+v"(vSlabOff), "+v"(vSlabBytes), "+v"(vSlices), "+v"(vSliceStride));
     const uint32_t nb = min(B, g.inDim - j0);
     const uint32_t e = a.expNo ? a.expNo[0] : 0u;
@@ -852,6 +864,21 @@
             const int o = min(tid * 2 + it * NT * 2, TILE_F - 2);
             s0[it] = tile_out(o); s1[it] = tile_out(o + 1);
         }
+        if constexpr (kChain) {
+            float2* const carry = reinterpret_cast<float2*>(smem + offM + __builtin_amdgcn_readfirstlane((lp.offV[0] - lp.offM) / 2u));
+            if (chain == 1u) {
+#pragma unroll
+                for (int it = 0; it < kIt; it++) carry[min(tid + it * NT, TILE_F / 2 - 1)] = make_float2(s0[it], s1[it]);
+                return;
+            }
+            if (chain == 2u) {
+#pragma unroll
+                for (int it = 0; it < kIt; it++) {
+                    const float2 cv = carry[min(tid + it * NT, TILE_F / 2 - 1)];
+                    s0[it] = cv.x + s0[it]; s1[it] = cv.y + s1[it];
+                }
+            }
+        }
 #pragma unroll
         for (int it = 0; it < kIt; it++) {
             const int o = tid * 2 + it * NT * 2;
@@ -1073,31 +1100,47 @@
     bool staged = false;
     uint32_t gen = 0;
     if (threadIdx.x == 0) __hip_atomic_store(&s_next, 0ull, __ATOMIC_RELAXED, __HIP_MEMORY_SCOPE_WORKGROUP);
+    constexpr bool kChain = PERSIST && COMPACT && !FUSED && FMT == kFp16;
+    const bool chained = kChain && (ga.split & 16u) != 0u;
+    uint32_t mode = 0;
+    ItemRef ref;
     uint32_t item = GA_PERSISTENT(ga) ? pull_sync() : blockIdx.x;
     while (item < total) {
-        if (item < GA_CUTJOBS(ga)) {
-            if (item < ga.count) cutoff_job<64 * W>(ga, item, smem);
-            item = GA_PERSISTENT(ga) ? pull_sync() : total;
-            continue;
-        }
-        ItemRef ref;
-        EFFORT_ESTAMP(1)
-        if (!locate_item(ga, item - GA_CUTJOBS(ga), ref)) {
-            item = GA_PERSISTENT(ga) ? pull_sync() : total;
-            continue;
-        }
-        EFFORT_ESTAMP(2)
-        gen++;
+        if (mode == 1u) {
+            mode = 2u;
+            ref.s += 4u;
+        } else {
+            if (item < GA_CUTJOBS(ga)) {
+                if (item < ga.count) cutoff_job<64 * W>(ga, item, smem);
+                item = GA_PERSISTENT(ga) ? pull_sync() : total;
+                continue;
+            }
+            EFFORT_ESTAMP(1)
+            if (!locate_item<kChain>(ga, item - GA_CUTJOBS(ga), ref)) {
+                item = GA_PERSISTENT(ga) ? pull_sync() : total;
+                continue;
+            }
+            EFFORT_ESTAMP(2)
+            gen++;
+            mode = chained ? 1u : 0u;
+        }
         bool stagedNext = false;
         auto prefetch = [&]() -> bool {
             if (!GA_PERSISTENT(ga)) return true;
-            if (threadIdx.x == 0)
-                __hip_atomic_store(&s_next, ((unsigned long long)gen << 32) | (unsigned long long)pull(), __ATOMIC_RELAXED, __HIP_MEMORY_SCOPE_WORKGROUP);
-            const unsigned long long nx = __hip_atomic_load(&s_next, __ATOMIC_RELAXED, __HIP_MEMORY_SCOPE_WORKGROUP);
-            if (__builtin_amdgcn_readfirstlane((uint32_t)(nx >> 32)) != gen) return false;
-            const uint32_t next = __builtin_amdgcn_readfirstlane((uint32_t)nx);
             ItemRef nref;
-            if (kPipe && !(GA_ABLATE(ga) & 128u) && next >= GA_CUTJOBS(ga) && next < total && locate_item(ga, next - GA_CUTJOBS(ga), nref)) {
+            bool stage;
+            if (kChain && mode == 1u) {
+                nref.ci = ref.ci; nref.t = ref.t; nref.s = ref.s + 4u;
+                stage = kPipe && !(GA_ABLATE(ga) & 128u);
+            } else {
+                if (threadIdx.x == 0)
+                    __hip_atomic_store(&s_next, ((unsigned long long)gen << 32) | (unsigned long long)pull(), __ATOMIC_RELAXED, __HIP_MEMORY_SCOPE_WORKGROUP);
+                const unsigned long long nx = __hip_atomic_load(&s_next, __ATOMIC_RELAXED, __HIP_MEMORY_SCOPE_WORKGROUP);
+                if (__builtin_amdgcn_readfirstlane((uint32_t)(nx >> 32)) != gen) return false;
+                const uint32_t next = __builtin_amdgcn_readfirstlane((uint32_t)nx);
+                stage = kPipe && !(GA_ABLATE(ga) & 128u) && next >= GA_CUTJOBS(ga) && next < total && locate_item<kChain>(ga, next - GA_CUTJOBS(ga), nref);
+            }
+            if (stage) {
                 int tid0 = threadIdx.x;
                 asm volatile("" : "+v"(tid0));
                 stage_issue<FMT, W, COMPACT>(ga, nref, tid0, smem, lp, par ^ 1u);
@@ -1106,8 +1149,8 @@
             return true;
         };
         const bool firstOwn = gen == 1u && (GA_ABLATE(ga) & 512u) != 0u;
-        mul_item<FMT, E, W, FUSED, COMPACT, PERSIST>(ga, item - GA_CUTJOBS(ga), ref, smem, lp, cachedCall, cachedCutoff, par, staged, firstOwn, prefetch);
-        item = GA_PERSISTENT(ga) ? __builtin_amdgcn_readfirstlane((uint32_t)__hip_atomic_load(&s_next, __ATOMIC_RELAXED, __HIP_MEMORY_SCOPE_WORKGROUP)) : total;
+        mul_item<FMT, E, W, FUSED, COMPACT, PERSIST>(ga, item - GA_CUTJOBS(ga), ref, smem, lp, cachedCall, cachedCutoff, par, staged, firstOwn, mode, prefetch);
+        if (mode != 1u) item = GA_PERSISTENT(ga) ? __builtin_amdgcn_readfirstlane((uint32_t)__hip_atomic_load(&s_next, __ATOMIC_RELAXED, __HIP_MEMORY_SCOPE_WORKGROUP)) : total;
         staged = stagedNext;
         par ^= 1u;
     }
@@ -1145,22 +1188,30 @@
     const LdsPlan lp = ga.lp = plan_lds<FMT, E, W>(ga.geom, kMaxGeoms, lean || (kLean && kProductOnly));
     uint32_t lds = lp.total;
     if (lp.offA > 65536u && FMT == kFp16) return hipErrorInvalidValue;
+    bool fusedAny = false;
+    for (uint32_t i = 0; i < ga.count; i++) fusedAny = fusedAny || ga.call[i].pre || ga.call[i].resid;
+    const bool chain = (ga.split & 16u) != 0u;
+    if (chain && (FMT != kFp16 || !ga.persistent || !(ga.split & 4u) || fusedAny)) return hipErrorInvalidValue;
     for (uint32_t i = 0; i < ga.count; i++) {
         const MulGeom& g = ga.geom[ga.call[i].geom];
         if (g.slots > (uint32_t)kRounds * 64 * W || g.slots != (FMT == kFp16 ? (g.rowsPerIn << g.sliceLog2) : g.sliceRows * 8u)) return hipErrorInvalidValue;
         if (FMT == kFp16 ? (1u << g.sliceLog2) > 64u * W : g.sliceRows > 128u * W) return hipErrorInvalidValue;
-        if (((uint32_t)ga.wgEnd8[i] - (i ? (uint32_t)ga.wgEnd8[i - 1] : 0u)) * 8u != align_up(g.tiles * g.slices, 8)) return hipErrorInvalidValue;
+        if (!chain && ((uint32_t)ga.wgEnd8[i] - (i ? (uint32_t)ga.wgEnd8[i - 1] : 0u)) * 8u != align_up(g.tiles * g.slices, 8)) return hipErrorInvalidValue;
+        if (chain && (g.slices != 8u || g.slots * 2u < (uint32_t)Fmt<FMT>::kAcc * E * 64u * 4u)) return hipErrorInvalidValue;
+    }
+    if (chain) {
+        uint32_t tiles[kMaxGroup];
+        uint16_t end8[kMaxGroup];
+        for (uint32_t i = 0; i < ga.count; i++) tiles[i] = ga.geom[ga.call[i].geom].tiles;
+        if (chain_ranges(tiles, ga.count, end8) != ga.totalItems || memcmp(end8, ga.wgEnd8, ga.count * sizeof(uint16_t)) != 0) return hipErrorInvalidValue;
     }
     if (ga.totalItems != (uint32_t)ga.wgEnd8[ga.count - 1] * 8u) return hipErrorInvalidValue;
-    uint32_t grid = ga.totalItems;
+    uint32_t grid = launch_grid(ga.numCU, ga.persistent, ga.totalItems, ga.cutJobs, chain);
     if (ga.persistent) {
         const uint32_t R = ga.persistent;
-        grid = ga.numCU * R;
         const uint32_t force = (160u * 1024u) / (R + 1u) + 512u;
         if (lds < force && force <= (160u * 1024u) / R) lds = force;
     }
-    bool fusedAny = false;
-    for (uint32_t i = 0; i < ga.count; i++) fusedAny = fusedAny || ga.call[i].pre || ga.call[i].resid;
     for (uint32_t i = 0; FMT != kFp16 && i < ga.count; i++)
         if (ga.call[i].pre && ga.call[i].ol.blockPtr && ga.geom[ga.call[i].geom].inDim > kOlLdsFloats) return hipErrorInvalidValue;
     if (lds > kMaxLdsBytes) return hipErrorInvalidValue;
@@ -1171,7 +1222,7 @@
     const hipError_t err = each_variant<FMT, E, W>([&](auto kernel, bool fu, bool co, bool pe) -> hipError_t {
         if (launched || fu != fusedAny || co != compact || pe == lean) return hipSuccess;
         launched = true;
-        if (ran) *ran = LaunchedVariant{(uint32_t)W, (uint32_t)E, fu, co, !pe, ga.persistent, grid, ga.totalItems};
+        if (ran) *ran = LaunchedVariant{(uint32_t)W, (uint32_t)E, fu, co, !pe, ga.persistent, grid, ga.totalItems, chain ? 1u : 0u};
         hipLaunchKernelGGL(kernel, gd, bd, lds, st, ga);
         return hipGetLastError();
     });
diff --git a/effort_amd/csrc/ctx.hip b/effort_amd/csrc/ctx.hip
--- a/effort_amd/csrc/ctx.hip
+++ b/effort_amd/csrc/ctx.hip
@@ -215,6 +215,11 @@
     c->env.persistent = wgPerCU;
     return EFFORT_OK;
 }
+extern "C" int effort_set_slice_pairs(effort_ctx* c, int policy) {
+    if (!c || policy < -1 || policy > 1) return EFFORT_ERR_ARG;
+    c->env.chain = policy;
+    return EFFORT_OK;
+}
 extern "C" int effort_set_row_reuse(effort_ctx* c, int reuse) {
     if (!c) return EFFORT_ERR_ARG;
     c->rowReuse = reuse != 0;
diff --git a/effort_amd/csrc/effort_internal.h b/effort_amd/csrc/effort_internal.h
--- a/effort_amd/csrc/effort_internal.h
+++ b/effort_amd/csrc/effort_internal.h
@@ -91,6 +91,24 @@
 };
 static_assert(sizeof(CallDesc) == 112 && sizeof(GroupKArgs) <= 4000, "the launch descriptor must fit the kernel-argument segment");
 
+struct ChainSlot { uint32_t ci, pair, k; };
+__host__ __device__ inline ChainSlot chain_locate(const uint16_t* wgEnd8, uint32_t count, uint32_t item) {
+    uint32_t c0 = 0;
+    for (uint32_t i = 0; i + 1 < count; i++) if ((item >> 3) >= (uint32_t)wgEnd8[i]) c0 = i + 1;
+    const uint32_t b = item - (c0 ? (uint32_t)wgEnd8[c0 - 1] * 8u : 0u), x = ((b & 7u) + (c0 >> 1)) & 7u;
+    return ChainSlot{c0 + (x >> 2), x & 3u, b >> 3};
+}
+inline uint32_t chain_ranges(const uint32_t* tiles, uint32_t count, uint16_t* wgEnd8) {
+    uint32_t end = 0;
+    for (uint32_t i = 0; i < count; i += 2) {
+        const uint32_t t1 = i + 1 < count ? tiles[i + 1] : 0u;
+        end += tiles[i] > t1 ? tiles[i] : t1;
+        wgEnd8[i] = (uint16_t)end;
+        if (i + 1 < count) wgEnd8[i + 1] = (uint16_t)end;
+    }
+    return end * 8u;
+}
+
 __device__ __forceinline__ float half_bits_to_float(uint16_t h) { return __half2float(__ushort_as_half(h)); }
 
 __device__ __forceinline__ float bf16_round(float f) {
@@ -171,7 +189,11 @@
 hipError_t launch_find_cutoff(const float* v, const uint16_t* probes, const uint32_t* expNo, uint32_t q,
                               float* cutoff, uint32_t* dispatchCount, unsigned long long* tstamp, hipStream_t st);
 
-struct LaunchedVariant { uint32_t W, E, fused, compact, lean, persistent, grid, totalItems; };
+inline uint32_t launch_grid(uint32_t numCU, uint32_t R, uint32_t totalItems, uint32_t cutJobs, bool chain) {
+    if (!R) return totalItems;
+    return chain && totalItems + cutJobs < numCU * R ? totalItems + cutJobs : numCU * R;
+}
+struct LaunchedVariant { uint32_t W, E, fused, compact, lean, persistent, grid, totalItems, chain; };
 hipError_t launch_bucket_mul(Format fmt, int wavesPerGroup, int elemsPerLane, const GroupKArgs& ga, hipStream_t st, LaunchedVariant* ran = nullptr);
 int bucket_mul_variants(Format fmt, int* rows, int maxRows);
 hipError_t bucket_mul_prepare_device();
diff --git a/effort_amd/csrc/mul.hip b/effort_amd/csrc/mul.hip
--- a/effort_amd/csrc/mul.hip
+++ b/effort_amd/csrc/mul.hip
@@ -65,7 +65,7 @@
         ga.slabs = L.d_slabs; ga.counters = L.d_counters; ga.sliceCounts = L.d_sliceCounts; ga.cutoff = L.d_cutoff + lp.first;
         ga.tstamp = env.clock ? c->d_tstamp : nullptr;
         ga.ablate = env.ablate; ga.trace = (env.clock && c->trace) ? 1u : 0u;
-        ga.split = (env.splitCutoff ? 1u : 0u) | (lp.compact ? 4u : 0u) | (c->rowReuse ? 8u : 0u);
+        ga.split = (env.splitCutoff ? 1u : 0u) | (lp.compact ? 4u : 0u) | (c->rowReuse ? 8u : 0u) | (lp.chain ? 16u : 0u);
         ga.numCU = (uint32_t)env.numCU; ga.queue = L.d_queue;
         ga.count = lp.count; ga.totalTiles = lp.totalTiles; ga.totalItems = lp.totalItems;
         ga.persistent = lp.persistent; ga.cutJobs = lp.cutJobs; ga.staggerSleeps = lp.staggerSleeps;
@@ -165,15 +165,12 @@
     HIP_TRY(c, hipStreamSynchronize(c->stream));
     return (int)n;
 }
-extern "C" int effort_debug_plan(int q4, int numCU, int lanes, int n, const int* inDim, const int* outDim, const int* percentLoad,
-                                 const int* prologue, const int* hasResid, const double* effort, int persistent, int tuneW, int tuneE, int tuneS,
-                                 int* we, int* slices, int* tiles, int* sliceRows, int* launchOf,
-                                 int* launchPersistent, int* launchCutJobs, int* launchCompact, int* launchStagger) {
-    if (numCU < 1 || lanes < 1 || lanes > kMaxLanes || n < 1 || n > kMaxGroup || !inDim || !outDim || !effort || !we || !slices || !tiles ||
-        !sliceRows || !launchOf || !launchPersistent || !launchCutJobs || !launchCompact || !launchStagger) return EFFORT_ERR_ARG;
+static int debug_plan(int q4, int numCU, int lanes, int n, const int* inDim, const int* outDim, const int* percentLoad, const int* prologue,
+                      const int* hasResid, const double* effort, int persistent, int tuneW, int tuneE, int tuneS, int pairs, GroupPlan& plan) {
+    if (numCU < 1 || lanes < 1 || lanes > kMaxLanes || n < 1 || n > kMaxGroup || !inDim || !outDim || !effort || pairs < -1 || pairs > 1) return EFFORT_ERR_ARG;
     const Format fmt = q4 ? kQ4 : kFp16;
     PlanEnv env = effort_ctx::scratch_env();
-    env.numCU = numCU; env.nLanes = lanes; env.persistent = persistent; env.tuneW = tuneW; env.tuneE = tuneE; env.tuneS = tuneS;
+    env.numCU = numCU; env.nLanes = lanes; env.persistent = persistent; env.tuneW = tuneW; env.tuneE = tuneE; env.tuneS = tuneS; env.chain = pairs;
     PlanCall pc[kMaxGroup];
     for (int i = 0; i < n; i++) {
         const int load = q4 ? 8 : (percentLoad ? percentLoad[i] : 16);
@@ -182,8 +179,15 @@
         const uint32_t cols = (uint32_t)outDim[i] / (q4 ? 32u : 16u);
         pc[i] = PlanCall{(uint32_t)inDim[i], (uint32_t)outDim[i], cols, (uint32_t)load, cols * 2u, 1u, !q4, (uint16_t)(prologue ? prologue[i] : 0), hasResid && hasResid[i]};
     }
+    return plan_group(fmt, call_env(env, lanes > 1, thin_effort(n, effort)), n, pc, &plan);
+}
+extern "C" int effort_debug_plan(int q4, int numCU, int lanes, int n, const int* inDim, const int* outDim, const int* percentLoad,
+                                 const int* prologue, const int* hasResid, const double* effort, int persistent, int tuneW, int tuneE, int tuneS,
+                                 int* we, int* slices, int* tiles, int* sliceRows, int* launchOf,
+                                 int* launchPersistent, int* launchCutJobs, int* launchCompact, int* launchStagger) {
+    if (!we || !slices || !tiles || !sliceRows || !launchOf || !launchPersistent || !launchCutJobs || !launchCompact || !launchStagger) return EFFORT_ERR_ARG;
     GroupPlan plan;
-    const int rc = plan_group(fmt, call_env(env, lanes > 1, thin_effort(n, effort)), n, pc, &plan);
+    const int rc = debug_plan(q4, numCU, lanes, n, inDim, outDim, percentLoad, prologue, hasResid, effort, persistent, tuneW, tuneE, tuneS, -1, plan);
     if (rc != EFFORT_OK) return rc;
     we[0] = plan.W; we[1] = plan.E;
     for (int i = 0; i < n; i++) {
@@ -195,6 +199,33 @@
         launchPersistent[l] = (int)lp.persistent; launchCutJobs[l] = (int)lp.cutJobs; launchCompact[l] = lp.compact ? 1 : 0; launchStagger[l] = (int)lp.staggerSleeps;
     }
     return (int)plan.nLaunches;
+}
+extern "C" int effort_debug_plan_pairs(int q4, int numCU, int lanes, int n, const int* inDim, const int* outDim, const int* percentLoad,
+                                       const int* prologue, const int* hasResid, const double* effort, int persistent, int tuneW, int tuneE, int tuneS,
+                                       int pairs, int* launchPaired, int* launchItems, int* launchGrid) {
+    if (!launchPaired || !launchItems || !launchGrid) return EFFORT_ERR_ARG;
+    GroupPlan plan;
+    const int rc = debug_plan(q4, numCU, lanes, n, inDim, outDim, percentLoad, prologue, hasResid, effort, persistent, tuneW, tuneE, tuneS, pairs, plan);
+    if (rc != EFFORT_OK) return rc;
+    for (uint32_t l = 0; l < plan.nLaunches; l++) {
+        const LaunchPlan& lp = plan.launch[l];
+        launchPaired[l] = lp.chain ? 1 : 0; launchItems[l] = (int)lp.totalItems;
+        launchGrid[l] = (int)launch_grid((uint32_t)numCU, lp.persistent, lp.totalItems, lp.cutJobs, lp.chain);
+    }
+    return (int)plan.nLaunches;
+}
+extern "C" int effort_debug_pair_items(int n, const int* tiles, int* items, int maxItems) {
+    if (n < 1 || n > kMaxGroup || !tiles || maxItems < 0 || (maxItems > 0 && !items)) return EFFORT_ERR_ARG;
+    uint32_t t[kMaxGroup];
+    uint16_t end8[kMaxGroup];
+    for (int i = 0; i < n; i++) { if (tiles[i] < 1 || tiles[i] > 1024) return EFFORT_ERR_ARG; t[i] = (uint32_t)tiles[i]; }
+    const uint32_t total = chain_ranges(t, (uint32_t)n, end8);
+    for (uint32_t b = 0; b < total && b < (uint32_t)maxItems; b++) {
+        const ChainSlot cs = chain_locate(end8, (uint32_t)n, b);
+        const bool real = cs.ci < (uint32_t)n && cs.k < t[cs.ci < (uint32_t)n ? cs.ci : 0];
+        items[3 * b] = real ? (int)cs.ci : -1; items[3 * b + 1] = (int)cs.k; items[3 * b + 2] = (int)cs.pair;
+    }
+    return (int)total;
 }
 extern "C" int effort_debug_variants(int q4, int* rows, int maxRows) {
     if (maxRows < 0 || (maxRows > 0 && !rows)) return EFFORT_ERR_ARG;
@@ -211,6 +242,13 @@
     const LaunchedVariant& v = L.lastVariant[launch];
     const uint32_t w[8] = {v.W, v.E, v.fused, v.compact, v.lean, v.persistent, v.grid, v.totalItems};
     for (int i = 0; i < 8; i++) out8[i] = (int)w[i];
+    return EFFORT_OK;
+}
+extern "C" int effort_debug_last_pairs(effort_ctx* c, int launch, int* paired) {
+    if (!c || !paired || launch < 0) return EFFORT_ERR_ARG;
+    const Lane& L = c->lane[c->lastLane];
+    if ((uint32_t)launch >= L.lastLaunches) return EFFORT_ERR_ARG;
+    *paired = (int)L.lastVariant[launch].chain;
     return EFFORT_OK;
 }
 extern "C" int effort_group_cutoff(effort_ctx* c, int idx, float* host_out) {
diff --git a/effort_amd/csrc/plan.h b/effort_amd/csrc/plan.h
--- a/effort_amd/csrc/plan.h
+++ b/effort_amd/csrc/plan.h
@@ -9,6 +9,7 @@
     int numCU = 256, nLanes = 1;
     bool laned = false;
     int persistent = -1;
+    int chain = -1;
     int tuneW = 0, tuneE = 0, tuneS = 0;
     bool splitCutoff = false, clock = false;
     uint32_t ablate = 0;
@@ -35,6 +36,7 @@
     uint32_t first, count;
     uint32_t persistent, cutJobs, staggerSleeps;
     bool compact;
+    bool chain;
     uint32_t totalItems, totalTiles, realItems;
 };
 struct GroupPlan {
diff --git a/effort_amd/csrc/plan.hip b/effort_amd/csrc/plan.hip
--- a/effort_amd/csrc/plan.hip
+++ b/effort_amd/csrc/plan.hip
@@ -185,7 +185,7 @@
     return k;
 }
 
-static void finish_launch(Format fmt, const PlanEnv& env, int W, const PlanCall* ws, const GroupPlan* P, LaunchPlan* lp) {
+static void finish_launch(Format fmt, const PlanEnv& env, int W, const PlanCall* ws, GroupPlan* P, LaunchPlan* lp) {
     const uint32_t R = env.persistent < 0 ? 2u : (uint32_t)env.persistent;
     const uint32_t perCU = (env.persistent < 0 && fmt == kFp16 && !env.laned) ? 6u : R;
     lp->persistent = (R && lp->realItems > (uint32_t)env.numCU * perCU) ? R : 0u;
@@ -201,6 +201,19 @@
     }
     lp->compact = compact;
     lp->staggerSleeps = (lp->persistent && fmt == kQ4 && !env.laned) ? 11u : 0u;
+    bool chain = fmt == kFp16 && lp->persistent != 0u && lp->compact && plain && (env.chain > 0 || (env.chain < 0 && env.laned));
+    for (uint32_t i = 0; chain && i < lp->count; i++) {
+        const MulGeom& g = P->call[lp->first + i].g;
+        chain = !ws[lp->first + i].hasResid && g.slices == 8u && (size_t)g.slots * 2u >= (size_t)tile_floats(fmt, P->E) * 4u;
+    }
+    lp->chain = chain;
+    if (chain) {
+        uint32_t tiles[kMaxGroup];
+        uint16_t end8[kMaxGroup];
+        for (uint32_t i = 0; i < lp->count; i++) tiles[i] = P->call[lp->first + i].g.tiles;
+        lp->totalItems = chain_ranges(tiles, lp->count, end8);
+        for (uint32_t i = 0; i < lp->count; i++) P->call[lp->first + i].itemEnd8 = end8[i];
+    }
 }
 
 int plan_group(Format fmt, const PlanEnv& env, int n, const PlanCall* ws, GroupPlan* P) {
diff --git a/effort_amd/runtime.py b/effort_amd/runtime.py
--- a/effort_amd/runtime.py
+++ b/effort_amd/runtime.py
@@ -110,6 +110,14 @@
     def set_persistent(self, wg_per_cu: int = -1):
         self.check(self._lib.effort_set_persistent(self.ctx, int(wg_per_cu)), "set_persistent")
 
+    def set_slice_pairs(self, policy: int = -1):
+        self.check(self._lib.effort_set_slice_pairs(self.ctx, int(policy)), "set_slice_pairs")
+
+    def last_pairs(self, launch: int = 0) -> bool:
+        n = C.c_int(0)
+        self.check(self._lib.effort_debug_last_pairs(self.ctx, int(launch), C.byref(n)), "last_pairs")
+        return bool(n.value)
+
     def set_dense_backend(self, rocblas: bool = False):
         self.check(self._lib.effort_set_dense_backend(self.ctx, int(bool(rocblas))), "set_dense_backend")
         self.dense_rocblas = bool(rocblas)
@@ -182,6 +190,29 @@
     res.update({name: list(a[:n]) for name, a in zip(("slices", "tiles", "sliceRows", "launch"), per_call)})
     res.update({name: list(a[:k]) for name, a in zip(("persistent", "cutJobs", "compact", "stagger"), per_launch)})
     return res
+
+
+def plan_pairs(calls, *, pairs: int = -1, q4: bool = False, numCU: int = 256, lanes: int = 1, persistent: int = -1, waves: int = 0, elems: int = 0,
+               slices: int = 0) -> dict:
+    n = len(calls)
+    rows = [tuple(c) + (16, 0, 0)[len(c) - 3:] for c in calls]
+    ints = lambda k: (C.c_int * n)(*[int(r[k]) for r in rows])
+    out = [(C.c_int * max(n, 2))() for _ in range(3)]
+    k = _lib.lib().effort_debug_plan_pairs(int(q4), numCU, lanes, n, ints(0), ints(1), ints(3), ints(4), ints(5), (C.c_double * n)(*[float(r[2]) for r in rows]),
+                                           persistent, waves, elems, slices, int(pairs), *out)
+    if k < 0:
+        raise _lib.EffortError(k, "plan_pairs")
+    return {"paired": [bool(x) for x in out[0][:k]], "items": list(out[1][:k]), "grid": list(out[2][:k])}
+
+
+def pair_items(tiles) -> list[tuple]:
+    n = len(tiles)
+    total = _lib.lib().effort_debug_pair_items(n, (C.c_int * n)(*[int(t) for t in tiles]), None, 0)
+    if total < 0:
+        raise _lib.EffortError(total, "pair_items")
+    buf = (C.c_int * (3 * max(total, 1)))()
+    _lib.lib().effort_debug_pair_items(n, (C.c_int * n)(*[int(t) for t in tiles]), buf, total)
+    return [(buf[3 * b], buf[3 * b + 1], buf[3 * b + 2]) for b in range(total)]
 
 
 def variants(q4: bool = False) -> list[tuple]:
diff --git a/include/effort_hip_debug.h b/include/effort_hip_debug.h
--- a/include/effort_hip_debug.h
+++ b/include/effort_hip_debug.h
@@ -11,6 +11,8 @@
 EFFORT_API int effort_set_split_cutoff(effort_ctx* ctx, int split);
 
 EFFORT_API int effort_set_persistent(effort_ctx* ctx, int wgPerCU);
+
+EFFORT_API int effort_set_slice_pairs(effort_ctx* ctx, int policy);
 
 EFFORT_API int effort_debug_hook_lane(effort_ctx* ctx, int lane);
 
@@ -26,6 +28,11 @@
                       const int* prologue, const int* hasResid, const double* effort, int persistent, int tuneW, int tuneE, int tuneS,
                       int* we, int* slices, int* tiles, int* sliceRows, int* launchOf,
                       int* launchPersistent, int* launchCutJobs, int* launchCompact, int* launchStagger);
+EFFORT_API int effort_debug_plan_pairs(int q4, int numCU, int lanes, int n, const int* inDim, const int* outDim, const int* percentLoad,
+                      const int* prologue, const int* hasResid, const double* effort, int persistent, int tuneW, int tuneE, int tuneS,
+                      int pairs, int* launchPaired, int* launchItems, int* launchGrid);
+EFFORT_API int effort_debug_pair_items(int n, const int* tiles, int* items, int maxItems);
+EFFORT_API int effort_debug_last_pairs(effort_ctx* ctx, int launch, int* paired);
 EFFORT_API int effort_debug_check_bundle(int q4, int inDim, int outDim, int percentLoad, int numExperts, int rowPitchBytes);
 EFFORT_API int effort_debug_variants(int q4, int* rows, int maxRows);
 EFFORT_API int effort_debug_last_variant(effort_ctx* ctx, int launch, int* out8);
```

Result: slower. 20780 (-3.4%).
